# vaenyr/stable-diffusion-on-device

Hardware: AMD Instinct MI355X
Metric: images/sec + per-UNet-step ms, SD v1.4 512x512 20-step PLMS, 1/2/4/8 MI355X (higher is better)
Workload: dtype f16; 1 GPU; SD v1.4 txt2img 512x512, 20-step PLMS (21 UNet evals, batch 2 = cond+uncond per image), CLIP encode + VAE decode + uint8, guidance 7.5; images_per_gpu=1, global_batch=1, parallelism=dp1 (image shards, 1 RCCL broadcast), hip_graph=True, trajectory_graph=True, decode_overlaps_next_sampling=False

## Files before the change

### include/sdod_hip.h

```cpp
#ifndef SDOD_HIP_H
#define SDOD_HIP_H

#include <stddef.h>
#include <stdint.h>

#ifndef SDOD_API
#define SDOD_API
#endif

#ifdef __cplusplus
extern "C" {
#endif

enum sdod_act { SDOD_ACT_NONE = 0, SDOD_ACT_SILU = 1, SDOD_ACT_GELU = 2, SDOD_ACT_QUICK_GELU = 3 };
enum sdod_dtype { SDOD_F16 = 0, SDOD_F32 = 1, SDOD_U8Q = 2, SDOD_BF16 = 3  };
enum sdod_a_mode { SDOD_A_ROWS = 0, SDOD_A_CONV3X3 = 1  };

typedef struct sdod_gemm_desc {
    const void* a;
    const void* a2;
    const void* w;
    const void* bias;
    const void* row_bias;
    const void* residual;
    void* out;
    void* workspace;
    size_t workspace_bytes;
    int M, N, K;
    int lda, ldw, ldo, ldr;
    int a_mode;
    int n_img, h_in, w_in, c0, c1;
    int stride;
    int upsample;
    int ksize;
    int rows_per_img;
    int ld_row_bias;
    int act;
    float alpha;
    int bias_on_m;
    int split_k;
    int tile;
    int geglu;
    int k_tail;
    const void* t0;
    const void* t1;
    int tc0, tc1;
    const void* bias2;
    int ln;
    const void* ln_s;
    float ln_eps;
    int phase;
    int wq;
    const void* w_scale;
    const void* w_off;
    void* fix_counters;
    int xcd_panels;
    int w_img_stride;
    int vec_img_stride;
    int softmax_cols;
    int pad_mode;
} sdod_gemm_desc;

SDOD_API int sdod_gemm_f16(const sdod_gemm_desc* d, void* stream);
SDOD_API int sdod_gemm_fixup(const sdod_gemm_desc* d);
SDOD_API size_t sdod_gemm_fixup_counters(void);
SDOD_API size_t sdod_gemm_workspace_bytes(const sdod_gemm_desc* d);
SDOD_API int sdod_gemm_plan(const sdod_gemm_desc* d, int* tile, int* splits);
SDOD_API int sdod_gemm_halo_ok(const sdod_gemm_desc* d, int tile);
SDOD_API int sdod_gemm_panel_ok(const sdod_gemm_desc* d, int tile);
SDOD_API int sdod_gemm_xcd_panels(const sdod_gemm_desc* d);
SDOD_API int sdod_gemm_num_tiles(void);
SDOD_API int sdod_gemm_tile_shape(int tile, int* bm, int* bn, int* lds_dma);
SDOD_API int sdod_gemm_tile_info(int tile, int out[7]);
SDOD_API int sdod_gemm_time(const sdod_gemm_desc* d, void* stream, int iters, float* ms_avg);
SDOD_API int sdod_gemm_time_cold(const sdod_gemm_desc* d, void* stream, int iters, void* scratch, size_t scratch_bytes, float* ms_avg,
                                float* ms_min );

SDOD_API size_t sdod_group_norm_workspace_bytes(int n, int groups);
SDOD_API int sdod_group_norm_layout(int n, int groups, size_t* sync_off, size_t* partial_off, size_t* stats_off, size_t* shift_off,
                                    size_t* end_off);
SDOD_API int sdod_group_norm_status(void);
SDOD_API int sdod_group_norm_clear_error(void);
SDOD_API int sdod_group_norm_launches(int hw, int c, int groups, int dtype);
SDOD_API int sdod_group_norm_path(int n, int hw, int c0, int c1, int groups, int dtype);
SDOD_API int sdod_group_norm_nhwc(const void* x, const void* x2, void* y, const float* weight, const float* bias,
                                  int n, int hw, int c0, int c1, int groups, float eps, int silu, int dtype,
                                  void* workspace, void* stream);

SDOD_API size_t sdod_group_norm_nchw_workspace_bytes(int n, int groups);
SDOD_API int sdod_group_norm_nchw(const void* x, void* y, const float* weight, const float* bias, int n, int c, long long spatial,
                                  int groups, float eps, int silu, int dtype, void* workspace, void* stream);

typedef struct sdod_gn_reduce {
    const void* partial;
    int splits;
    size_t slab_floats;
    const void* bias;
    const void* bias2;
    const void* row_bias;
    int ld_row_bias;
    const void* residual;
    int ldr;
    void* x_out;
    float alpha;
    int act;
    int M, N;
} sdod_gn_reduce;
SDOD_API int sdod_gemm_reduce_info(const sdod_gemm_desc* d, sdod_gn_reduce* out);
SDOD_API int sdod_group_norm_reduce_ok(int hw, int c0, int c1, int groups);
SDOD_API int sdod_group_norm_reduce_nhwc(const sdod_gn_reduce* red, const void* x2, void* y, const float* weight,
                                         const float* bias, int n, int hw, int c0, int c1, int groups, float eps, int silu,
                                         void* stream);

SDOD_API int sdod_ln_fold_f16(void* w, int n, int k, int ldw, const float* gamma, const float* beta, const float* bias_in,
                              float* s_out, float* t_out, void* stream);
SDOD_API int sdod_compose_linear_f16(const void* p, int ldp, const void* w, int ldw, void* c, int ldc, int n_out, int n_mid, int k,
                                     const float* bias_w, const float* bias_p, float* bias_out, void* stream);
SDOD_API int sdod_layer_norm_f16(const void* x, void* y, const float* weight, const float* bias, int m, int c,
                                 float eps, void* stream);

SDOD_API int sdod_attention_f16(const void* q, const void* k, const void* v, void* out, int batch, int heads,
                                int lq, int lk, int d, int ldq, int ldk, int ldv, int ldo, float scale, int causal,
                                void* stream);

SDOD_API int sdod_xattn_fold_f16(const void* kv, int ld_kv, int k_off, int v_off, int n_img, int L, const void* wq, int ldq,
                                 const void* sq, const void* tq, const void* wo, int ldwo, int heads, int d, float scale, void* w1,
                                 void* s1, void* t1, void* w2, void* stream);

SDOD_API int sdod_softmax_rows_f16(const void* x, void* y, int m, int n, void* stream);

SDOD_API int sdod_geglu_f16(const void* x, void* y, int m, int c, void* stream);
SDOD_API int sdod_act_f16(const void* x, void* y, size_t n, int act, void* stream);
SDOD_API int sdod_add_f16(const void* a, const void* b, void* y, size_t n, void* stream);
SDOD_API int sdod_concat_channels_f16(const void* a, const void* b, void* y, size_t rows, int c0, int c1, void* stream);
SDOD_API int sdod_im2col3x3_small_f16(const void* x, void* y, int n_img, int h, int w, int c, int kpad, void* stream);
SDOD_API int sdod_latent_im2col_f16(const float* x, void* y, int n_img, int h, int w, int c, int kpad, float scale, void* stream);

SDOD_API int sdod_conv_in_f16(const float* x, const void* w, const float* bias, void* y, int n_img, int h, int wd, int c, int cout,
                              float scale, void* stream);
SDOD_API int sdod_image_conv_in_f16(const uint8_t* img, const void* w, const float* bias, void* y, int n_img, int h, int wd, int cout,
                                    void* stream);
SDOD_API int sdod_conv_in_cat_f16(const float* x, const float* cond, const void* w, const float* bias, void* y, int n_img, int h, int wd,
                                  int c, int c_cond, int cout, void* stream);
SDOD_API int sdod_masked_image_conv_in_f16(const uint8_t* img, const uint8_t* mask, const void* w, const float* bias, void* y, int n_img,
                                           int h, int wd, int cout, void* stream);
SDOD_API int sdod_inpaint_cond_f32(const float* moments, const uint8_t* mask_u8, const float* n1, float* cond, int n, int c, int h_lat,
                                   int w_lat, int factor, int reps, uint64_t seed, uint64_t image_index0, void* stream);
SDOD_API int sdod_encode_latent_f32(const float* moments, const float* n1, const float* n2, float* x, float* z0, int n, int c, int hw,
                                    float sqrt_at, float sqrt_one_minus_at, uint64_t seed, uint64_t image_index0, void* stream);
SDOD_API int sdod_nchw_f32_to_nhwc_f16(const float* x, void* y, int n, int c, int hw, float scale, void* stream);
SDOD_API int sdod_latent_prep_f16(const float* x, const float* w, const float* b, void* y, int n, int c, int hw,
                                  float scale, void* stream);
SDOD_API int sdod_nhwc_f16_to_nchw_f32(const void* x, float* y, int n, int c, int hw, void* stream);
SDOD_API int sdod_embedding_f16(const int32_t* ids, const void* table, const void* pos, void* y, int rows, int seq,
                                int c, void* stream);
SDOD_API int sdod_timestep_features_f16(const float* t, void* y, int n, int dim, void* stream);

SDOD_API int sdod_stage_unet_inputs(const float* x, float* x_dst, size_t lat_count, int reps, const void* temb_row,
                                    void* temb_dst, size_t temb_width, int temb_reps, void* stream);
SDOD_API int sdod_randn_f32(float* out, uint32_t* words_out, size_t count, uint64_t seed, uint64_t stream_id, void* stream);

SDOD_API int sdod_cfg_combine(const void* eps_nhwc, float* e_out, int n, int c, int hw, float guidance,
                              int uncond_first, int mode, void* stream);
SDOD_API int sdod_dpm_update(float* x, const float* eps, float* y_prev, size_t count, int order, float sigma_s,
                             float alpha_s, float sigma_ratio, float c_prev, float c_cur, void* stream);
SDOD_API int sdod_ddim_step_f32(float* x, const float* e, size_t count, float sqrt_one_minus_at, float sqrt_at,
                                float sqrt_a_prev, float dir_coef, void* stream);
SDOD_API int sdod_lincomb4_f32(float* out, const float* e0, const float* e1, const float* e2, const float* e3,
                               float c0, float c1, float c2, float c3, float div, size_t count, void* stream);

typedef struct sdod_plms_update_args {
    const void* eps_nhwc;
    float* e_out;
    float* x;
    const float* old1; const float* old2; const float* old3;
    float* x_stage;
    const void* temb_row;
    void* temb_dst;
    int n, c, hw, uncond_first, mode, v_pred, stage_reps, temb_width, temb_reps;
    float guidance, vc0, vc1, c0, c1, c2, c3, div, sqrt_one_minus_at, sqrt_at, sqrt_a_prev, dir_coef;
} sdod_plms_update_args;
SDOD_API int sdod_plms_update(const sdod_plms_update_args* a, void* stream);

typedef struct sdod_dpm_step_args {
    const void* eps_nhwc;
    float* e_out;
    float* x;
    float* y_prev;
    float* x_stage;
    const void* temb_row;
    void* temb_dst;
    int n, c, hw, uncond_first, mode, order, stage_reps, temb_width, temb_reps;
    float guidance, sigma_s, alpha_s, sigma_ratio, c_prev, c_cur;
} sdod_dpm_step_args;
SDOD_API int sdod_dpm_step(const sdod_dpm_step_args* a, void* stream);

typedef struct sdod_ddim_inpaint_step_args {
    const void* eps_nhwc;
    float* x;
    const float* z0;
    const float* keep;
    const float* noise;
    float* x_stage;
    const void* temb_row;
    void* temb_dst;
    uint64_t seed, image_index0;
    int n, c, hw, uncond_first, mode, v_pred, last, noise_level, stage_reps, temb_width, temb_reps;
    float guidance, vc0, vc1, sqrt_one_minus_at, sqrt_at, sqrt_a_prev, dir_coef, known_sa, known_s1a;
} sdod_ddim_inpaint_step_args;
SDOD_API int sdod_ddim_inpaint_step(const sdod_ddim_inpaint_step_args* a, void* stream);

typedef struct sdod_k_step_args {
    const void* eps_nhwc;
    float* x;
    float* den_prev;
    const float* noise;
    float* x_stage;
    const void* temb_row;
    void* temb_dst;
    uint64_t seed, image_index0;
    int n, c, hw, uncond_first, mode, noise_level, stage_reps, temb_width, temb_reps;
    float guidance, d0, d1, a, b, cprev, u, stage_scale;
} sdod_k_step_args;
SDOD_API int sdod_k_step(const sdod_k_step_args* a, void* stream);
SDOD_API int sdod_mask_to_latent_f32(const uint8_t* mask_u8, float* keep, int n, int h_lat, int w_lat, int factor, void* stream);
SDOD_API int sdod_image_composite_u8(const void* img, const uint8_t* init_u8, const uint8_t* mask_u8, uint8_t* out_u8, int n, size_t hw,
                                     float a, float b, int mode, void* stream);
SDOD_API int sdod_image_to_u8(const void* img, uint8_t* out, size_t count, float a, float b, int mode, void* stream);

SDOD_API const char* sdod_hip_last_error(void);
SDOD_API int sdod_hip_device_info(int* cu_count, size_t* hbm_bytes, char* arch, int arch_len);

SDOD_API int sdod_l2_prefetch(const void* ptr, size_t bytes, void* stream);

#ifdef __cplusplus
}
#endif
#endif
```

### stable-diffusion-on-device_amd/csrc/attention.hip

```cpp
#include "common.h"
#include "sdod_hip.h"
#include "host_util.h"

#include <climits>
#include <cmath>
#include <cstdlib>
#include <type_traits>

namespace {

struct AttnP {
    const f16* q;
    const f16* k;
    const f16* v;
    f16* out;
    int B, H, Lq, Lk;
    int ldq, ldk, ldv, ldo;
    float scale_log2;
    int causal;
};

typedef short short4v __attribute__((__vector_size__(4 * sizeof(short))));
typedef __attribute__((address_space(3))) short4v* lds_short4_ptr;

constexpr int odd16(int dv) {
    int s = (dv + 15) / 16;
    if ((s & 1) == 0) s += 1;
    return s * 16;
}

template <int D, int QT>
constexpr int attn_min_waves() { return (D == 40 || (D == 80 && QT == 1)) ? 3 : 1; }

template <int N, int I = 0, class F>
SDOD_DEVICE void static_for(F&& f) {
    if constexpr (I < N) {
        f(std::integral_constant<int, I>{});
        static_for<N, I + 1>(f);
    }
}

template <int D, int QT, bool TR, int KVS = 1>
__global__ __launch_bounds__(256 * KVS, (attn_min_waves<D, QT>())) void attn_kernel(const AttnP p) {
    constexpr int DP = ((D + 31) / 32) * 32;
    constexpr int KSTEPS = DP / 32;
    constexpr int DV = ((D + 15) / 16) * 16;
    constexpr int NDT = DV / 16;
    constexpr int KSTR = DP + 8;
    constexpr int VSTR = odd16(DV);
    constexpr int KT = 64;
    constexpr int DC = D / 8;
    constexpr int LD_IT = (KT * DC + 255) / 256;
    constexpr int STAGE = KT * (KSTR + VSTR);
    constexpr bool SUM_BY_MFMA = DV > D;
    constexpr bool DEFER = DP > D;
    constexpr int KS_M = D / 32, G_M = (D % 32) / 8;
    constexpr float THR = 8.0f;
    static_assert(D % 8 == 0, "head dim must be a multiple of 8");

    extern __shared__ __attribute__((aligned(16))) char smem_raw[];
    const int grp = KVS > 1 ? (int)(threadIdx.x >> 8) : 0;
    f16* smem = reinterpret_cast<f16*>(smem_raw) + (size_t)grp * 2 * STAGE;

    const int tid = threadIdx.x & 255;
    const int lane = tid & 63;
    const int wave = tid >> 6;
    const int g = lane >> 4;
    const int li = lane & 15;
    const int nqb = (p.Lq + 64 * QT - 1) / (64 * QT);
    const int lid = xcd_remap(blockIdx.x, nqb * p.H * p.B);
    const int bh = lid / nqb;
    const int b = bh / p.H, h = bh - b * p.H;
    const int q_block = (lid - bh * nqb) * (64 * QT);

    const f16* kbase = p.k + (size_t)b * p.Lk * p.ldk + h * D;
    const f16* vbase = p.v + (size_t)b * p.Lk * p.ldv + h * D;

    {
        constexpr int KPADC = (DP - D) / 8, VPADC = (DV - D) / 8;
        for (int st = 0; st < 2; ++st) {
            f16* sK = smem + st * STAGE;
            f16* sV = sK + KT * KSTR;
            if (KPADC > 0)
                for (int idx = tid; idx < KT * KPADC; idx += 256) {
                    const int row = idx / (KPADC > 0 ? KPADC : 1), ch = idx - row * KPADC;
                    f16x8 pad = zero8();
                    if (DEFER && ch == 0) pad[0] = (f16)-1.0f;
                    *reinterpret_cast<f16x8*>(sK + row * KSTR + D + ch * 8) = pad;
                }
            if (VPADC > 0)
                for (int idx = tid; idx < KT * VPADC; idx += 256) {
                    const int row = idx / (VPADC > 0 ? VPADC : 1), ch = idx - row * VPADC;
                    f16x8 pad = zero8();
                    if (ch == 0) pad[0] = (f16)1.0f;
                    *reinterpret_cast<f16x8*>(sV + row * VSTR + D + ch * 8) = pad;
                }
        }
    }

    f16x8 qf[QT][KSTEPS];
    int qrow[QT];
#pragma unroll
    for (int t = 0; t < QT; ++t) {
        qrow[t] = q_block + wave * (16 * QT) + t * 16 + li;
        const f16* qp = p.q + ((size_t)b * p.Lq + qrow[t]) * p.ldq + h * D;
#pragma unroll
        for (int ks = 0; ks < KSTEPS; ++ks) {
            const int d0 = ks * 32 + g * 8;
            qf[t][ks] = (qrow[t] < p.Lq && d0 + 8 <= D) ? ldg8(qp + d0) : zero8();
            if (DEFER)
#pragma unroll
                for (int e = 0; e < 8; ++e) qf[t][ks][e] = (f16)((float)qf[t][ks][e] * p.scale_log2);
        }
    }

    int kend = p.Lk;
    if (p.causal) kend = min(p.Lk, q_block + 64 * QT);
    const int NT = (kend + KT - 1) / KT;

    f16x8 rk[LD_IT], rv[LD_IT];
    const f16* kptr0[LD_IT];
    const f16* vptr0[LD_IT];
#pragma unroll
    for (int i = 0; i < LD_IT; ++i) {
        const int idx = tid + 256 * i;
        const int row = idx / DC, ch = idx - row * DC;
        kptr0[i] = kbase + (size_t)row * p.ldk + ch * 8;
        vptr0[i] = vbase + (size_t)row * p.ldv + ch * 8;
    }
    auto load_tile = [&](int t) {
        if (t * KT + KT <= p.Lk) {
            const size_t ko = (size_t)t * KT * p.ldk, vo = (size_t)t * KT * p.ldv;
#pragma unroll
            for (int i = 0; i < LD_IT; ++i) {
                if (tid + 256 * i < KT * DC) {
                    rk[i] = ldg8(kptr0[i] + ko);
                    rv[i] = ldg8(vptr0[i] + vo);
                }
            }
            return;
        }
#pragma unroll
        for (int i = 0; i < LD_IT; ++i) {
            const int idx = tid + 256 * i;
            const int row = idx / DC, ch = idx - row * DC;
            const int key = t * KT + row;
            const bool ok = (idx < KT * DC) && (key < p.Lk);
            rk[i] = ok ? ldg8(kbase + (size_t)key * p.ldk + ch * 8) : zero8();
            rv[i] = ok ? ldg8(vbase + (size_t)key * p.ldv + ch * 8) : zero8();
        }
    };
    auto store_tile = [&](int st) {
        f16* sK = smem + st * STAGE;
        f16* sV = sK + KT * KSTR;
#pragma unroll
        for (int i = 0; i < LD_IT; ++i) {
            const int idx = tid + 256 * i;
            const int row = idx / DC, ch = idx - row * DC;
            if (idx < KT * DC) {
                *reinterpret_cast<f16x8*>(sK + row * KSTR + ch * 8) = rk[i];
                *reinterpret_cast<f16x8*>(sV + row * VSTR + ch * 8) = rv[i];
            }
        }
    };

    f32x4 o[QT][NDT];
    float m_run[QT], l_run[QT];
#pragma unroll
    for (int t = 0; t < QT; ++t) {
        m_run[t] = DEFER ? 0.f : -1e30f;
        l_run[t] = 0.f;
#pragma unroll
        for (int dt = 0; dt < NDT; ++dt) o[t][dt] = f32x4{0.f, 0.f, 0.f, 0.f};
    }

#ifdef SDOD_ATTN_ABLATE
    constexpr int abl = SDOD_ATTN_ABLATE;
#else
    constexpr int abl = 0;
#endif
    constexpr bool HOLD = D <= 80;
    auto read_vt = [&](const f16* sV, int u, int dt) -> f16x8 {
        const f16* a0 = sV + (32 * u + 4 * g + (li >> 2)) * VSTR + dt * 16 + 4 * (li & 3);
        const short4v lo = __builtin_amdgcn_ds_read_tr16_b64_v4i16((lds_short4_ptr)(a0));
        const short4v hi = __builtin_amdgcn_ds_read_tr16_b64_v4i16((lds_short4_ptr)(a0 + 16 * VSTR));
        typedef short short8v __attribute__((__vector_size__(8 * sizeof(short))));
        const short8v both = __builtin_shufflevector(lo, hi, 0, 1, 2, 3, 4, 5, 6, 7);
        return __builtin_bit_cast(f16x8, both);
    };
    auto softmax_pv = [&](auto a_c, int t, int thr, f32x4 (&s_a)[4], const f16x8 (&vfr)[HOLD ? 2 : 1][HOLD ? NDT : 1],
                          const f16* sV) {
        constexpr int a = decltype(a_c)::value;
        const bool need_mask = (t * KT + KT > p.Lk) || (p.causal && (t * KT + KT - 1 > q_block + wave * (16 * QT)));
        if (need_mask) {
            int key0 = t * KT + g * 4;
            asm volatile("" : "+v"(key0));
#pragma unroll
            for (int c = 0; c < 4; ++c)
#pragma unroll
                for (int r = 0; r < 4; ++r) {
                    const int key = key0 + c * 16 + r;
                    const bool masked = (key >= p.Lk) | (p.causal & (key > qrow[a]));
                    s_a[c][r] = masked ? -1e30f : s_a[c][r];
                }
        }
        auto lane_max = [&]() {
            const float t0 = fmaxf(fmaxf(s_a[0][0], s_a[0][1]), s_a[0][2]);
            const float t1 = fmaxf(fmaxf(s_a[0][3], s_a[1][0]), s_a[1][1]);
            const float t2 = fmaxf(fmaxf(s_a[1][2], s_a[1][3]), s_a[2][0]);
            const float t3 = fmaxf(fmaxf(s_a[2][1], s_a[2][2]), s_a[2][3]);
            const float t4 = fmaxf(fmaxf(s_a[3][0], s_a[3][1]), s_a[3][2]);
            const float u0 = fmaxf(fmaxf(t0, t1), t2);
            const float u1 = fmaxf(fmaxf(t3, t4), s_a[3][3]);
            return fmaxf(u0, u1);
        };
        float rs[4] = {0.f, 0.f, 0.f, 0.f};
        if constexpr (DEFER) {
            auto bi = [](float x) { return __builtin_bit_cast(int, x); };
            auto mx3 = [](int x, int y, int z) { return max(max(x, y), z); };
            const int t0 = mx3(bi(s_a[0][0]), bi(s_a[0][1]), bi(s_a[0][2]));
            const int t1 = mx3(bi(s_a[0][3]), bi(s_a[1][0]), bi(s_a[1][1]));
            const int t2 = mx3(bi(s_a[1][2]), bi(s_a[1][3]), bi(s_a[2][0]));
            const int t3 = mx3(bi(s_a[2][1]), bi(s_a[2][2]), bi(s_a[2][3]));
            const int t4 = mx3(bi(s_a[3][0]), bi(s_a[3][1]), bi(s_a[3][2]));
            const int mi = max(mx3(t0, t1, t2), mx3(t3, t4, bi(s_a[3][3])));
            if (__builtin_amdgcn_ballot_w64(mi > thr) != 0) {
                const bool first = thr == INT_MIN;
                const float mx = quad_rows_max(lane_max());
                const float m_old = m_run[a];
                float m_new = m_old;
                if (first || mx > 0.f) m_new = (float)(f16)fminf(fmaxf(m_old + mx, -65504.f), 65504.f);
                const float delta = m_new - m_old;
                if (!first) {
                    const float alpha = __builtin_amdgcn_exp2f(-delta);
#pragma unroll
                    for (int dt = 0; dt < NDT; ++dt)
#pragma unroll
                        for (int r = 0; r < 4; ++r) o[a][dt][r] *= alpha;
                    if (!SUM_BY_MFMA) l_run[a] *= alpha;
                }
                m_run[a] = m_new;
                if (g == G_M) qf[a][KS_M][0] = (f16)m_new;
#pragma unroll
                for (int c = 0; c < 4; ++c)
#pragma unroll
                    for (int r = 0; r < 4; ++r) s_a[c][r] -= delta;
            }
#pragma unroll
            for (int c = 0; c < 4; ++c) {
#pragma unroll
                for (int r = 0; r < 4; ++r) {
                    float v = s_a[c][r];
                    if (!(abl & 2)) v = __builtin_amdgcn_exp2f(v);
                    if (!SUM_BY_MFMA) rs[r] += v;
                    s_a[c][r] = v;
                }
            }
            if (!SUM_BY_MFMA) l_run[a] += (rs[0] + rs[1]) + (rs[2] + rs[3]);
        } else {
            const float mx = quad_rows_max(lane_max());
            const float m_new = fmaxf(m_run[a], mx * p.scale_log2);
            const bool rescale = __builtin_amdgcn_ballot_w64(m_new != m_run[a]) != 0;
            const float alpha = rescale ? __builtin_amdgcn_exp2f(m_run[a] - m_new) : 1.0f;
            m_run[a] = m_new;
            const float sc = p.scale_log2, nm = -m_new;
#pragma unroll
            for (int c = 0; c < 4; ++c) {
#pragma unroll
                for (int r = 0; r < 4; ++r) {
                    float v = __builtin_fmaf(s_a[c][r], sc, nm);
                    if (!(abl & 2)) v = __builtin_amdgcn_exp2f(v);
                    if (!SUM_BY_MFMA) rs[r] += v;
                    s_a[c][r] = v;
                }
            }
            if (!SUM_BY_MFMA) l_run[a] = __builtin_fmaf(l_run[a], alpha, (rs[0] + rs[1]) + (rs[2] + rs[3]));
            if (rescale) {
#pragma unroll
                for (int dt = 0; dt < NDT; ++dt)
#pragma unroll
                    for (int r = 0; r < 4; ++r) o[a][dt][r] *= alpha;
            }
        }
        f16x8 pf[2];
#pragma unroll
        for (int u = 0; u < 2; ++u) {
            f16x8 f;
#pragma unroll
            for (int r = 0; r < 4; ++r) {
                f[r] = (f16)s_a[2 * u][r];
                f[4 + r] = (f16)s_a[2 * u + 1][r];
            }
            pf[u] = f;
        }
#pragma unroll
        for (int u = 0; u < 2; ++u) {
#pragma unroll
            for (int dt = 0; dt < NDT; ++dt) {
                f16x8 vf;
                if (TR) {
                    vf = HOLD ? vfr[u][dt] : read_vt(sV, u, dt);
                } else {
#pragma unroll
                    for (int e = 0; e < 8; ++e) vf[e] = sV[(32 * u + 16 * (e >> 2) + 4 * g + (e & 3)) * VSTR + dt * 16 + li];
                }
                o[a][dt] = mfma16(vf, pf[u], o[a][dt]);
            }
        }
    };
    auto read_k = [&](const f16* sK, f16x8 (&kf)[HOLD ? KSTEPS : 1][4]) {
        if constexpr (HOLD) {
#pragma unroll
            for (int ks = 0; ks < KSTEPS; ++ks)
#pragma unroll
                for (int c = 0; c < 4; ++c) kf[ks][c] = *reinterpret_cast<const f16x8*>(sK + (c * 16 + li) * KSTR + ks * 32 + g * 8);
        }
    };
    auto read_v = [&](const f16* sV, f16x8 (&vfr)[HOLD ? 2 : 1][HOLD ? NDT : 1]) {
        if constexpr (TR && HOLD) {
#pragma unroll
            for (int u = 0; u < 2; ++u)
#pragma unroll
                for (int dt = 0; dt < NDT; ++dt) vfr[u][dt] = read_vt(sV, u, dt);
        }
    };
    auto qk = [&](const f16* sK, const f16x8 (&kf)[HOLD ? KSTEPS : 1][4], f32x4 (&s)[QT][4]) {
#pragma unroll
        for (int a = 0; a < QT; ++a) {
#pragma unroll
            for (int c = 0; c < 4; ++c) s[a][c] = f32x4{0.f, 0.f, 0.f, 0.f};
#pragma unroll
            for (int ks = 0; ks < KSTEPS; ++ks)
#pragma unroll
                for (int c = 0; c < 4; ++c) {
                    const f16x8 k8 = HOLD ? kf[ks][c] : *reinterpret_cast<const f16x8*>(sK + (c * 16 + li) * KSTR + ks * 32 + g * 8);
                    s[a][c] = mfma16(k8, qf[a][ks], s[a][c]);
                }
        }
    };

    if (grp < NT) {
        load_tile(grp);
        store_tile(0);
    }
    __syncthreads();
    const int NTG = (NT + KVS - 1) / KVS;
    int thr = INT_MIN;
    for (int it = 0; it < NTG; ++it) {
        const int t = it * KVS + grp;
        const int cur = it & 1;
        const bool has_next = t + KVS < NT;
        const f16* sK = smem + cur * STAGE;
        const f16* sV = sK + KT * KSTR;
        if (t >= NT) {
            __syncthreads();
            continue;
        }
        f16x8 kf[HOLD ? KSTEPS : 1][4];
        f16x8 vfr[HOLD ? 2 : 1][HOLD ? NDT : 1];
        read_k(sK, kf);
        read_v(sV, vfr);
        f32x4 s[QT][4];
        qk(sK, kf, s);
        if (has_next && !(abl & 1)) load_tile(t + KVS);
        static_for<QT>([&](auto a_c) { softmax_pv(a_c, t, thr, s[decltype(a_c)::value], vfr, sV); });
        thr = __builtin_bit_cast(int, THR);
        asm volatile("" : "+s"(thr));
        if (has_next) store_tile(cur ^ 1);
        __syncthreads();
    }

    if constexpr (KVS > 1) {
        static_assert(KVS == 2, "the merge below handles two groups");
        float* mrg = reinterpret_cast<float*>(smem_raw);
        constexpr int NV = QT * (2 + NDT * 4);
        static_assert((size_t)NV * 256 * sizeof(float) <= (size_t)KVS * 2 * STAGE * sizeof(f16), "merge buffer fits the staging LDS");
        if (grp == 1) {
#pragma unroll
            for (int a = 0; a < QT; ++a) {
                mrg[(a * (2 + NDT * 4) + 0) * 256 + tid] = m_run[a];
                mrg[(a * (2 + NDT * 4) + 1) * 256 + tid] = l_run[a];
#pragma unroll
                for (int dt = 0; dt < NDT; ++dt)
#pragma unroll
                    for (int r = 0; r < 4; ++r) mrg[(a * (2 + NDT * 4) + 2 + dt * 4 + r) * 256 + tid] = o[a][dt][r];
            }
        }
        __syncthreads();
        if (grp == 1) return;
#pragma unroll
        for (int a = 0; a < QT; ++a) {
            const float m1 = mrg[(a * (2 + NDT * 4) + 0) * 256 + tid], l1 = mrg[(a * (2 + NDT * 4) + 1) * 256 + tid];
            const float m = fmaxf(m_run[a], m1);
            const float a0 = __builtin_amdgcn_exp2f(m_run[a] - m), a1 = __builtin_amdgcn_exp2f(m1 - m);
            l_run[a] = l_run[a] * a0 + l1 * a1;
#pragma unroll
            for (int dt = 0; dt < NDT; ++dt)
#pragma unroll
                for (int r = 0; r < 4; ++r) o[a][dt][r] = o[a][dt][r] * a0 + mrg[(a * (2 + NDT * 4) + 2 + dt * 4 + r) * 256 + tid] * a1;
            m_run[a] = m;
        }
    }
#pragma unroll
    for (int a = 0; a < QT; ++a) {
        float l;
        if (SUM_BY_MFMA) {
            l = __shfl(o[a][D / 16][D % 4], ((D % 16) / 4) * 16 + li);
        } else {
            l = quad_rows_sum(l_run[a]);
        }
        const float inv = l > 0.f ? 1.0f / l : 0.f;
        if (qrow[a] < p.Lq) {
            f16* op = p.out + ((size_t)b * p.Lq + qrow[a]) * p.ldo + h * D;
#pragma unroll
            for (int dt = 0; dt < NDT; ++dt) {
                const int dv0 = dt * 16 + g * 4;
                if (dv0 < D) {
                    f16x4 hv;
#pragma unroll
                    for (int r = 0; r < 4; ++r) hv[r] = (f16)(o[a][dt][r] * inv);
                    *reinterpret_cast<f16x4*>(op + dv0) = hv;
                }
            }
        }
    }
}

template <int D, int QT, bool TR, int KVS = 1>
hipError_t attn_launch(const AttnP& p, hipStream_t st) {
    constexpr int DP = ((D + 31) / 32) * 32;
    constexpr int DV = ((D + 15) / 16) * 16;
    constexpr size_t smem = (size_t)KVS * 2 * 64 * (DP + 8 + odd16(DV)) * sizeof(f16);
    static_assert(smem <= 160 * 1024, "LDS");
    static std::atomic<unsigned long long> attr_devs{0};
    if (sdod::first_use_on_device(attr_devs)) {
        hipError_t e = hipFuncSetAttribute(reinterpret_cast<const void*>(&attn_kernel<D, QT, TR, KVS>),
                                           hipFuncAttributeMaxDynamicSharedMemorySize, (int)smem);
        if (e != hipSuccess) return e;
    }
    dim3 grid(((p.Lq + 64 * QT - 1) / (64 * QT)) * p.H * p.B);
    SDOD_LAUNCH((attn_kernel<D, QT, TR, KVS>), grid, dim3(256 * KVS), smem, st, p);
    return hipGetLastError();
}

template <int D>
hipError_t attn_dispatch(const AttnP& p, bool big, bool tr, hipStream_t st) {
    if (tr) return big ? attn_launch<D, 2, true>(p, st) : attn_launch<D, 1, true>(p, st);
    return big ? attn_launch<D, 2, false>(p, st) : attn_launch<D, 1, false>(p, st);
}

struct FoldP {
    const f16* kv; int ld_kv, k_off, v_off, L, n_img;
    const f16* wq; int ldq;
    const float* sq; const float* tq;
    const f16* wo; int ldwo;
    int heads, d, C;
    float alpha;
    f16* w1; float* s1; float* t1; f16* w2;
    int tiles_c;
    int n_w;
};
constexpr int kFoldKMax = 160;
__global__ __launch_bounds__(256) void xattn_fold_kernel(const FoldP p) {
    __shared__ __attribute__((aligned(16))) f16 sa[80][kFoldKMax + 8], sb[80][kFoldKMax + 8];
    const int tid = threadIdx.x, lane = tid & 63, wave = tid >> 6;
    const int NK = p.heads * 80, d = p.d;
    int item = blockIdx.x;
    if (item >= 2 * p.n_w) {
        const int idx = (item - 2 * p.n_w) * 256 + tid;
        if (idx >= p.n_img * NK) return;
        const int j = idx % 80, bh = idx / 80, h = bh % p.heads, img = bh / p.heads;
        if (j >= p.L) {
            p.s1[idx] = 0.f;
            p.t1[idx] = -30000.f;
            return;
        }
        const f16* kr = p.kv + ((long long)img * p.L + j) * p.ld_kv + p.k_off + h * d;
        float a = 0.f, b = 0.f;
        for (int dd = 0; dd < d; ++dd) {
            const float kval = (float)kr[dd];
            a = fmaf(kval, p.sq[h * d + dd], a);
            b = fmaf(kval, p.tq[h * d + dd], b);
        }
        p.s1[idx] = p.alpha * a;
        p.t1[idx] = p.alpha * b;
        return;
    }
    const bool second = item >= p.n_w;
    if (second) item -= p.n_w;
    const int tc = item % p.tiles_c, bh = item / p.tiles_c, h = bh % p.heads, img = bh / p.heads;
    const int KP = (d + 31) & ~31, kc = KP / 8;
    auto stage_rows = [&](f16 (*dst)[kFoldKMax + 8], const f16* base, long long row_stride, int valid_rows) {
        for (int idx = tid; idx < 80 * kc; idx += 256) {
            const int r = idx / kc, ch = idx - r * kc;
            const f16x8 v = (r < valid_rows && ch * 8 < d) ? ldg8(base + (long long)r * row_stride + ch * 8) : zero8();
            *reinterpret_cast<f16x8*>(&dst[r][ch * 8]) = v;
        }
    };
    if (!second) {
        stage_rows(sa, p.kv + (long long)img * p.L * p.ld_kv + p.k_off + h * d, p.ld_kv, p.L);
        for (int idx = tid; idx < KP * 10; idx += 256) {
            const int k = idx / 10, ch = idx - k * 10;
            const f16x8 v = k < d ? ldg8(p.wq + (long long)(h * d + k) * p.ldq + tc * 80 + ch * 8) : zero8();
#pragma unroll
            for (int e = 0; e < 8; ++e) sb[ch * 8 + e][k] = v[e];
        }
    } else {
        stage_rows(sa, p.wo + (long long)(tc * 80) * p.ldwo + h * d, p.ldwo, 80);
        stage_rows(sb, p.kv + (long long)img * p.L * p.ld_kv + p.v_off + h * d, p.ld_kv, p.L);
    }
    __syncthreads();
    const int fr = lane & 15, fg = lane >> 4;
    for (int rb = wave; rb < 5; rb += 4) {
        f32x4 acc[5];
#pragma unroll
        for (int j = 0; j < 5; ++j) acc[j] = f32x4{0.f, 0.f, 0.f, 0.f};
        for (int ks = 0; ks < KP / 32; ++ks) {
            const f16x8 fa = *reinterpret_cast<const f16x8*>(&sa[rb * 16 + fr][ks * 32 + fg * 8]);
#pragma unroll
            for (int j = 0; j < 5; ++j) {
                const f16x8 fb = *reinterpret_cast<const f16x8*>(&sb[j * 16 + fr][ks * 32 + fg * 8]);
                acc[j] = mfma16(fb, fa, acc[j]);
            }
        }
        const int m = rb * 16 + fr;
        f16* row = second ? p.w2 + ((long long)img * p.C + tc * 80 + m) * NK + h * 80
                          : p.w1 + ((long long)(img * p.heads + h) * 80 + m) * p.C + tc * 80;
        const float al = second ? 1.0f : p.alpha;
#pragma unroll
        for (int j = 0; j < 5; ++j) {
            f16x4 o;
#pragma unroll
            for (int r = 0; r < 4; ++r) o[r] = (f16)(al * acc[j][r]);
            *reinterpret_cast<f16x4*>(row + j * 16 + fg * 4) = o;
        }
    }
}

}

extern "C" int sdod_attention_f16(const void* q, const void* k, const void* v, void* out, int batch, int heads, int lq,
                                  int lk, int d, int ldq, int ldk, int ldv, int ldo, float scale, int causal,
                                  void* stream) {
    SDOD_TRY
    SDOD_REQUIRE(q && k && v && out, "null pointer");
    SDOD_REQUIRE(batch > 0 && heads > 0 && lq > 0 && lk > 0, "bad shape");
    SDOD_REQUIRE(d == 40 || d == 64 || d == 80 || d == 160, "head dim must be one of 40, 64, 80, 160");
    SDOD_REQUIRE(ldq % 8 == 0 && ldk % 8 == 0 && ldv % 8 == 0 && ldo % 4 == 0, "row strides must keep 16-byte alignment");
    SDOD_REQUIRE(ldq >= heads * d && ldk >= heads * d && ldv >= heads * d && ldo >= heads * d, "row stride < heads*d");
    SDOD_REQUIRE((((uintptr_t)q | (uintptr_t)k | (uintptr_t)v) & 15) == 0 && ((uintptr_t)out & 7) == 0, "misaligned pointer");
    SDOD_REQUIRE(std::isfinite(scale) && scale > 0.f, "scale must be finite and > 0");
    AttnP p{};
    p.q = (const f16*)q; p.k = (const f16*)k; p.v = (const f16*)v; p.out = (f16*)out;
    p.B = batch; p.H = heads; p.Lq = lq; p.Lk = lk;
    p.ldq = ldq; p.ldk = ldk; p.ldv = ldv; p.ldo = ldo;
    p.scale_log2 = scale * 1.4426950408889634f;
    p.causal = causal;
    const bool no_tr = std::getenv("SDOD_ATTN_NO_TR") != nullptr;
    const bool tr = !no_tr;
    bool big = lq >= 2048 && d != 160;
    if (const char* e = std::getenv("SDOD_ATTN_QT")) big = e[0] == '2' && d != 160;
    hipStream_t st = (hipStream_t)stream;
    hipError_t e;
    switch (d) {
    case 40: e = attn_dispatch<40>(p, big, tr, st); break;
    case 64: e = attn_dispatch<64>(p, big, tr, st); break;
    case 80: {
        static const bool kvs_off = [] { const char* e2 = std::getenv("SDOD_ATTN_KVS"); return e2 && e2[0] == '0'; }();
        const long long wgs = (long long)((lq + 63) / 64) * heads * batch;
        if (!big && tr && !kvs_off && !causal && wgs <= 512 && lk >= 256) e = attn_launch<80, 1, true, 2>(p, st);
        else e = attn_dispatch<80>(p, big, tr, st);
        break;
    }
    default: e = attn_dispatch<160>(p, false, tr, st); break;
    }
    SDOD_HIP_CHECK(e);
    return 0;
    SDOD_CATCH
}

extern "C" int sdod_xattn_fold_f16(const void* kv, int ld_kv, int k_off, int v_off, int n_img, int L, const void* wq, int ldq,
                                   const void* sq, const void* tq, const void* wo, int ldwo, int heads, int d, float scale, void* w1,
                                   void* s1, void* t1, void* w2, void* stream) {
    SDOD_TRY
    SDOD_REQUIRE(kv && wq && sq && tq && wo && w1 && s1 && t1 && w2, "null pointer");
    SDOD_REQUIRE(n_img > 0 && heads > 0 && d > 0 && d <= kFoldKMax && d % 8 == 0 && L > 0 && L <= 80, "bad shape (d <= 160, d % 8 == 0, L <= 80)");
    const int C = heads * d, NK = heads * 80;
    SDOD_REQUIRE(C % 80 == 0 && ldq >= C && ldwo >= C && ld_kv >= C, "heads * d must be a multiple of 80; row strides >= heads * d");
    SDOD_REQUIRE(ld_kv % 8 == 0 && k_off % 8 == 0 && v_off % 8 == 0 && ldq % 8 == 0 && ldwo % 8 == 0 &&
                     (((uintptr_t)kv | (uintptr_t)wq | (uintptr_t)wo | (uintptr_t)w1 | (uintptr_t)w2) & 15) == 0,
                 "operands must keep 16-byte alignment");
    FoldP p{};
    p.kv = (const f16*)kv; p.ld_kv = ld_kv; p.k_off = k_off; p.v_off = v_off; p.L = L; p.n_img = n_img;
    p.wq = (const f16*)wq; p.ldq = ldq; p.sq = (const float*)sq; p.tq = (const float*)tq;
    p.wo = (const f16*)wo; p.ldwo = ldwo;
    p.heads = heads; p.d = d; p.C = C;
    p.alpha = scale * 1.4426950408889634f;
    p.w1 = (f16*)w1; p.s1 = (float*)s1; p.t1 = (float*)t1; p.w2 = (f16*)w2;
    p.tiles_c = C / 80;
    p.n_w = n_img * heads * p.tiles_c;
    const int blocks = 2 * p.n_w + (n_img * NK + 255) / 256;
    SDOD_LAUNCH(xattn_fold_kernel, dim3(blocks), dim3(256), 0, (hipStream_t)stream, p);
    SDOD_HIP_CHECK(hipGetLastError());
    return 0;
    SDOD_CATCH
}
```

### stable-diffusion-on-device_amd/csrc/engine.h

```cpp
#pragma once
#include <hip/hip_runtime.h>

#include <cstdint>
#include <functional>
#include <map>
#include <string>
#include <unordered_map>
#include <vector>

#include "host_util.h"
#include "sdod_engine.h"
#include "sdod_hip.h"

namespace sdod {

typedef _Float16 f16;

enum ParamKind {
    PK_CONV3,
    PK_CONV3_SMALL,
    PK_CONV1,
    PK_LINEAR,
    PK_EMBED,
    PK_VEC,
    PK_MAT_F32,
    PK_LINEAR_GEGLU,
    PK_VEC_GEGLU,
};

inline int small_k(int64_t cin) { return 9 * cin <= 64 ? 64 : 128; }

struct Param {
    std::string name;
    std::vector<int64_t> shape;
    ParamKind kind;
    int group = -1;
    int ld = 0;
    int col_off = 0;
    int owner = -1;
    size_t dev_bytes = 0;
    char* dev = nullptr;
    bool set = false;
    bool quant = false;
    size_t qrow = 0;
};

struct Act {
    f16* p = nullptr;
    int n = 0, h = 0, w = 0, c = 0;
    int rows() const { return n * h * w; }
    size_t numel() const { return (size_t)rows() * c; }
};

struct IoSlot {
    void* ptr = nullptr;
    size_t bytes = 0;
};

class Graph {
public:
    Graph(int kind, const sdod_model_config& cfg, int batch);
    ~Graph();
    Graph(const Graph&) = delete;

    int num_params() const { return (int)params_.size(); }
    const Param& param(int i) const { return params_.at(i); }
    void set_param(const std::string& name, const void* data, int dtype, const int64_t* shape, int ndim);
    void load_file(const std::string& path, const std::string& prefix);
    void finalize();
    void execute(hipStream_t st, bool use_hip_graph, bool skip_static = false);
    void check_health() const;
    IoSlot io(bool output, int index) const;
    void stats(size_t* wbytes, size_t* abytes, int* launches, double* flops) const;

private:
    enum Mode { DECLARE, DRY, REAL };
    int kind_;
    sdod_model_config cfg_;
    int batch_;
    Mode mode_ = DECLARE;
    bool finalized_ = false;

    std::vector<Param> params_;
    std::unordered_map<std::string, int> pindex_;
    std::vector<std::vector<int>> groups_;
    std::unordered_map<std::string, int> gindex_;
    char* weight_base_ = nullptr;
    size_t weight_bytes_ = 0;
    float* qscale_ = nullptr;
    float* qoff_ = nullptr;
    size_t qrows_ = 0;
    bool quant_mode() const { return cfg_.weight_quant != 0 && (kind_ == SDOD_GRAPH_UNET || kind_ == SDOD_GRAPH_TEMB); }
    static constexpr int kQuantAutoMaxRows = 128;
    bool quant_decl_ = false;
    void quant_rows(int rows) { quant_decl_ = quant_mode() && (cfg_.weight_quant == 1 || rows <= kQuantAutoMaxRows); }
    void quant_global() { quant_decl_ = quant_mode(); }
    const float* qscale_of(int w) const { return params_[w].quant ? qscale_ + params_[w].qrow : nullptr; }
    const float* qoff_of(int w) const { return params_[w].quant ? qoff_ + params_[w].qrow : nullptr; }
    int P(const std::string& name, std::vector<int64_t> shape, ParamKind kind, const std::string& group = "");
    int Pc(const std::string& name, std::vector<int64_t> shape, ParamKind kind, int ld, int col_off, int owner);
    template <typename T>
    const T* W(int idx) const { return reinterpret_cast<const T*>(params_[idx].dev); }
    void allocate_weights();

    char* arena_base_ = nullptr;
    size_t arena_cap_ = 0, arena_high_ = 0;
    std::map<size_t, size_t> free_;
    std::map<size_t, size_t> used_;
    void arena_reset();
    f16* alloc(size_t halves);
    void release(const void* p);
    Act act(int n, int h, int w, int c);
    void release(const Act& a) { release(a.p); }

    char* ws_ = nullptr;
    size_t ws_bytes_ = 0, ws_need_ = 0;
    char* gn_ws_ = nullptr;
    size_t gn_ws_bytes_ = 0, gn_ws_need_ = 0;

    std::vector<IoSlot> inputs_, outputs_;
    void* io_alloc(std::vector<IoSlot>& v, size_t bytes);

    struct Op {
        std::function<void(hipStream_t)> fn;
        std::string label;
        double flops = 0;
        double bytes = 0;
        std::string detail;
        const void* pf_ptr = nullptr;
        size_t pf_bytes = 0;
    };
    std::vector<Op> ops_;
    std::vector<Op> static_ops_;
    bool to_static_ = false;
    double flops_ = 0;
    hipGraphExec_t graph_exec_ = nullptr;
    hipGraph_t hip_graph_ = nullptr;
    hipStream_t capture_stream_ = nullptr;
    unsigned* fix_counters_ = nullptr;
    hipStream_t side_stream_ = nullptr;
    std::vector<hipEvent_t> pf_events_;
    void run_ops(hipStream_t st);
    int eager_runs_ = 0;
    int tune_hits_ = 0, tune_misses_ = 0;

    void build();
    void build_unet();
    void build_vae();
    void build_vae_encoder(bool masked);
    void build_clip();
    void build_temb();

    struct GemmOpt {
        int bias = -1;
        const float* bias_raw = nullptr;
        f16* out = nullptr;
        const f16* row_bias = nullptr;
        int ld_row_bias = 0, rows_per_img = 0;
        const f16* residual = nullptr;
        int act = 0;
        float alpha = 1.0f;
        bool bias_on_m = false;
        int lda = 0, ldo = 0;
        int ldr = 0;
        bool geglu = false;
        const Act* tail0 = nullptr;
        const Act* tail1 = nullptr;
        int bias2 = -1;
        int ln_w = -1, ln_b = -1;
        const float* wq_scale = nullptr;
        const float* wq_off = nullptr;
        const float* ln_s_raw = nullptr;
        int w_img_stride = 0, vec_img_stride = 0;
        int softmax_cols = 0;
        int pad_mode = 0;
    };
    struct LnVecs { float* s; float* t; };
    LnVecs ln_fold_vectors(f16* w, int N, int K, int ldw, int ln_w, int ln_b, const float* bias);
    struct FoldJob {
        f16* w; int n, k, ldw;
        const float *gamma, *beta, *bias_in;
        float *s, *t;
    };
    std::vector<FoldJob> fold_jobs_;
    struct ComposeJob {
        f16* c; const f16* p; int ld, n_out, n_mid, k;
        const float *bias_w, *bias_p;
        float* bias_out;
    };
    std::vector<ComposeJob> compose_jobs_;
    std::vector<void*> derived_;
    void emit_gemm(sdod_gemm_desc d);
    void linear(const f16* x, int rows, int K, int w, int N, f16* out, const GemmOpt& o);
    void linear_raw(const f16* x, int rows, int K, const f16* w, int ldw, int N, f16* out, const GemmOpt& o);
    Act conv(const Act& x, const Act* x2, int w, int cout, int ksize, int stride, bool upsample, const GemmOpt& o);
    Act group_norm(const Act& x, const Act* x2, int gw, int gb, float eps, bool silu);
    Act layer_norm(const Act& x, int lw, int lb, float eps);
    void attention(const f16* q, const f16* k, const f16* v, f16* out, int B, int heads, int lq, int lk, int d, int ldq,
                   int ldk, int ldv, int ldo, bool causal);

    Act res_block(const std::string& pfx, const Act& x, const Act* x2, int cout, const f16* emb_all, int emb_ld, int& emb_off);
    std::vector<Op>& sink() { return to_static_ ? static_ops_ : ops_; }
    struct PendingReduce {
        bool active = false;
        sdod_gemm_desc d{};
        double bytes = 0;
        std::string detail;
    } pending_;
    void flush_pending();
    std::vector<const void*> parked_;
    void release_after_consumer(const Act& a) { parked_.push_back(a.p); }
    void drain_parked() {
        for (const void* p : parked_) release(p);
        parked_.clear();
    }
    void settle() {
        flush_pending();
        drain_parked();
    }
    Act spatial_transformer(const std::string& pfx, const Act& x, const Act& ctx);
    Act vae_res_block(const std::string& pfx, const Act& x, int cout);
    Act vae_attn_block(const std::string& pfx, const Act& x);
    int emb_total_ = 0;
    int kv_total_ = 0;
    f16* kv_all_ = nullptr;
    int kv_off_ = 0;
    std::vector<std::pair<std::string, int>> unet_res_blocks() const;
    const char* group_base(const std::string& group) const;
    int group_first(const std::string& group) const;
    void emit(std::function<void(hipStream_t)> fn, const char* label = "elementwise", double flops = 0, double bytes = 0) {
        settle();
        if (mode_ == REAL) sink().push_back(Op{std::move(fn), label, flops, bytes, ""});
    }

public:
    int tune_hits() const { return tune_hits_; }
    int tune_misses() const { return tune_misses_; }
    int num_ops() const { return (int)ops_.size(); }
    const Op& op(int i) const { return ops_.at(i); }
    void profile(hipStream_t st, int iters, float* ms, int n);
};

}
```

### stable-diffusion-on-device_amd/csrc/engine.hip

```cpp
#include "engine.h"

#include <cstdio>

#include <dlfcn.h>
#include <fcntl.h>
#include <sys/mman.h>
#include <sys/stat.h>
#include <unistd.h>

#include <algorithm>
#include <cstdlib>
#include <cstring>
#include <map>
#include <mutex>
#include <thread>

namespace sdod {

static inline size_t align_up(size_t v, size_t a) { return (v + a - 1) / a * a; }

static void check_rc(int rc) {
    if (rc != 0) throw Error(rc, get_last_error());
}

template <typename F>
static void parallel_for(int64_t n, F&& fn) {
    int nt = (int)std::min<int64_t>(n, std::max(1u, std::min(16u, std::thread::hardware_concurrency())));
    if (nt <= 1) {
        fn(0, n);
        return;
    }
    std::vector<std::thread> th;
    const int64_t per = (n + nt - 1) / nt;
    for (int t = 0; t < nt; ++t) {
        const int64_t b = t * per, e = std::min(n, b + per);
        if (b < e) th.emplace_back([=, &fn]() { fn(b, e); });
    }
    for (auto& t : th) t.join();
}

Graph::Graph(int kind, const sdod_model_config& cfg, int batch) : kind_(kind), cfg_(cfg), batch_(batch) {
    SDOD_REQUIRE(kind >= SDOD_GRAPH_UNET && kind <= SDOD_GRAPH_VAE_ENCODER_MASKED, "unknown graph kind");
    SDOD_REQUIRE(batch > 0 && batch <= 64, "batch must be in [1, 64]");
    SDOD_REQUIRE(cfg.model_channels > 0 && cfg.model_channels % 64 == 0, "model_channels must be a multiple of 64");
    SDOD_REQUIRE(cfg.context_dim % 64 == 0, "context_dim must be a multiple of 64");
    SDOD_REQUIRE(cfg.concat_channels >= 0, "concat_channels must not be negative");
    mode_ = DECLARE;
    arena_reset();
    build();
}

Graph::~Graph() {
    if (graph_exec_) (void)hipGraphExecDestroy(graph_exec_);
    if (capture_stream_) (void)hipStreamDestroy(capture_stream_);
    if (side_stream_) (void)hipStreamDestroy(side_stream_);
    (void)hipFree(fix_counters_);
    for (hipEvent_t e : pf_events_) (void)hipEventDestroy(e);
    if (hip_graph_) (void)hipGraphDestroy(hip_graph_);
    for (auto& s : inputs_) (void)hipFree(s.ptr);
    for (auto& s : outputs_) (void)hipFree(s.ptr);
    (void)hipFree(weight_base_);
    (void)hipFree(qscale_);
    (void)hipFree(qoff_);
    (void)hipFree(arena_base_);
    (void)hipFree(ws_);
    (void)hipFree(gn_ws_);
    (void)hipFree(kv_all_);
    for (void* d : derived_) (void)hipFree(d);
}

static size_t param_dev_bytes(const Param& p) {
    const auto& s = p.shape;
    if (p.quant) return (size_t)s[0] * s[1] * (p.kind == PK_CONV3 ? 9 : 1);
    switch (p.kind) {
    case PK_CONV3: return (size_t)s[0] * s[1] * 9 * sizeof(f16);
    case PK_CONV3_SMALL: return (size_t)s[0] * small_k(s[1]) * sizeof(f16);
    case PK_CONV1:
    case PK_LINEAR:
    case PK_LINEAR_GEGLU:
    case PK_EMBED: return (size_t)s[0] * s[1] * sizeof(f16);
    case PK_VEC:
    case PK_VEC_GEGLU: return (size_t)s[0] * sizeof(float);
    case PK_MAT_F32: {
        size_t n = 1;
        for (auto d : s) n *= (size_t)d;
        return n * sizeof(float);
    }
    }
    return 0;
}

int Graph::P(const std::string& name, std::vector<int64_t> shape, ParamKind kind, const std::string& group) {
    if (mode_ != DECLARE) {
        auto it = pindex_.find(name);
        if (it == pindex_.end()) throw Error(INTERNAL_ERROR, "parameter not declared: " + name);
        return it->second;
    }
    if (pindex_.count(name)) throw Error(INTERNAL_ERROR, "duplicate parameter: " + name);
    Param p;
    p.name = name;
    p.shape = std::move(shape);
    p.kind = kind;
    p.quant = quant_decl_ && (kind == PK_CONV3 || kind == PK_CONV1 || kind == PK_LINEAR || kind == PK_LINEAR_GEGLU);
    p.dev_bytes = param_dev_bytes(p);
    if (!group.empty()) {
        auto it = gindex_.find(group);
        if (it == gindex_.end()) {
            gindex_[group] = (int)groups_.size();
            groups_.emplace_back();
            it = gindex_.find(group);
        }
        p.group = it->second;
        groups_[p.group].push_back((int)params_.size());
    }
    pindex_[name] = (int)params_.size();
    params_.push_back(std::move(p));
    return (int)params_.size() - 1;
}

int Graph::Pc(const std::string& name, std::vector<int64_t> shape, ParamKind kind, int ld, int col_off, int owner) {
    const int idx = P(name, std::move(shape), kind);
    if (mode_ == DECLARE) {
        Param& p = params_[idx];
        p.ld = ld;
        p.col_off = col_off;
        p.owner = owner;
        p.dev_bytes = owner < 0 ? (size_t)p.shape[0] * ld * sizeof(f16) : 0;
    }
    return idx;
}

void Graph::allocate_weights() {
    if (weight_base_) return;
    size_t off = 0;
    std::vector<size_t> offs(params_.size(), 0);
    for (auto& g : groups_) {
        off = align_up(off, 256);
        for (int idx : g) {
            if (params_[idx].dev_bytes % 16) throw Error(INTERNAL_ERROR, "grouped parameter size must be a multiple of 16: " + params_[idx].name);
            offs[idx] = off;
            off += params_[idx].dev_bytes;
        }
    }
    for (size_t i = 0; i < params_.size(); ++i) {
        if (params_[i].group >= 0) continue;
        off = align_up(off, 256);
        offs[i] = off;
        off += params_[i].dev_bytes;
    }
    weight_bytes_ = align_up(off, 256);
    SDOD_HIP_CHECK(hipMalloc((void**)&weight_base_, weight_bytes_));
    SDOD_HIP_CHECK(hipMemset(weight_base_, 0, weight_bytes_));
    for (size_t i = 0; i < params_.size(); ++i) params_[i].dev = weight_base_ + offs[i];
    {
        std::vector<size_t> order;
        for (size_t i = 0; i < params_.size(); ++i)
            if (params_[i].quant) order.push_back(i);
        std::sort(order.begin(), order.end(), [&](size_t a, size_t b) { return offs[a] < offs[b]; });
        qrows_ = 0;
        for (size_t i : order) {
            params_[i].qrow = qrows_;
            qrows_ += (size_t)params_[i].shape[0];
        }
        if (qrows_) {
            SDOD_HIP_CHECK(hipMalloc((void**)&qscale_, qrows_ * sizeof(float)));
            SDOD_HIP_CHECK(hipMalloc((void**)&qoff_, qrows_ * sizeof(float)));
        }
    }
    for (auto& p : params_)
        if (p.owner >= 0) p.dev = params_[p.owner].dev + (size_t)p.col_off * sizeof(f16);
}

template <typename S>
static void pack_param_host(const Param& p, const S* src, char* dst_raw) {
    const auto& s = p.shape;
    switch (p.kind) {
    case PK_CONV3:
    case PK_CONV3_SMALL: {
        const int64_t co = s[0], ci = s[1];
        const int64_t kd = p.kind == PK_CONV3 ? 9 * ci : small_k(ci);
        f16* dst = reinterpret_cast<f16*>(dst_raw);
        parallel_for(co, [&](int64_t b, int64_t e) {
            for (int64_t o = b; o < e; ++o) {
                f16* drow = dst + o * kd;
                if (p.kind == PK_CONV3_SMALL) std::memset(drow, 0, kd * sizeof(f16));
                const S* srow = src + o * ci * 9;
                for (int64_t c = 0; c < ci; ++c)
                    for (int t = 0; t < 9; ++t) drow[t * ci + c] = (f16)(float)srow[c * 9 + t];
            }
        });
        break;
    }
    case PK_CONV1:
    case PK_LINEAR:
    case PK_EMBED: {
        const int64_t n = s[0] * s[1];
        f16* dst = reinterpret_cast<f16*>(dst_raw);
        parallel_for(n, [&](int64_t b, int64_t e) {
            for (int64_t i = b; i < e; ++i) dst[i] = (f16)(float)src[i];
        });
        break;
    }
    case PK_LINEAR_GEGLU: {
        const int64_t rows = s[0], k = s[1], H = rows / 2;
        f16* dst = reinterpret_cast<f16*>(dst_raw);
        parallel_for(rows, [&](int64_t b, int64_t e) {
            for (int64_t r = b; r < e; ++r) {
                const int64_t j = r < H ? r : r - H;
                const int64_t nr = (j / 16) * 32 + (r < H ? 0 : 16) + j % 16;
                for (int64_t c = 0; c < k; ++c) dst[nr * k + c] = (f16)(float)src[r * k + c];
            }
        });
        break;
    }
    case PK_VEC_GEGLU: {
        const int64_t rows = s[0], H = rows / 2;
        float* dst = reinterpret_cast<float*>(dst_raw);
        for (int64_t r = 0; r < rows; ++r) {
            const int64_t j = r < H ? r : r - H;
            dst[(j / 16) * 32 + (r < H ? 0 : 16) + j % 16] = (float)src[r];
        }
        break;
    }
    case PK_VEC:
    case PK_MAT_F32: {
        int64_t n = 1;
        for (auto d : s) n *= d;
        float* dst = reinterpret_cast<float*>(dst_raw);
        for (int64_t i = 0; i < n; ++i) dst[i] = (float)src[i];
        break;
    }
    }
}

void Graph::set_param(const std::string& name, const void* data, int dtype, const int64_t* shape, int ndim) {
    allocate_weights();
    SDOD_REQUIRE(!finalized_, "parameters cannot change after finalize() (weights are repacked / folded in place)");
    auto it = pindex_.find(name);
    SDOD_REQUIRE(it != pindex_.end(), "unknown parameter '" + name + "'");
    SDOD_REQUIRE(data != nullptr, "null data for '" + name + "'");
    SDOD_REQUIRE(dtype == SDOD_F32 || dtype == SDOD_F16 || dtype == SDOD_U8Q, "dtype must be SDOD_F32, SDOD_F16 or SDOD_U8Q");
    Param& p = params_[it->second];
    int64_t want = 1, got = 1;
    for (auto d : p.shape) want *= d;
    for (int i = 0; i < ndim; ++i) got *= shape[i];
    if (p.quant) {
        SDOD_REQUIRE(dtype == SDOD_U8Q, "graph was created with weight_quant != 0: '" + name + "' must be given as SDOD_U8Q");
        bool same = (int)p.shape.size() == ndim;
        for (int i = 0; same && i < ndim; ++i) same = p.shape[i] == shape[i];
        if (!same && want == got && (p.kind == PK_CONV1 || p.kind == PK_LINEAR) && ndim >= 2 && shape[0] == p.shape[0]) same = true;
        SDOD_REQUIRE(same, "shape mismatch for '" + name + "'");
        float scale;
        int32_t offset;
        std::memcpy(&scale, data, 4);
        std::memcpy(&offset, static_cast<const char*>(data) + 4, 4);
        SDOD_REQUIRE(offset >= -1024 && offset <= 0, "'" + name + "': uint8 encoding offset must be in [-1024, 0] (QNN: -zero_point of a uint8 tensor)");
        const uint8_t* q = static_cast<const uint8_t*>(data) + 8;
        const int64_t rows = p.shape[0], kd = got / rows;
        std::vector<uint8_t> staging((size_t)got);
        uint8_t* dst = staging.data();
        if (p.kind == PK_CONV3) {
            const int64_t ci = p.shape[1];
            parallel_for(rows, [&](int64_t b, int64_t e) {
                for (int64_t o = b; o < e; ++o)
                    for (int64_t c = 0; c < ci; ++c)
                        for (int t = 0; t < 9; ++t) dst[o * kd + t * ci + c] = q[(o * ci + c) * 9 + t];
            });
        } else if (p.kind == PK_LINEAR_GEGLU) {
            const int64_t H = rows / 2;
            parallel_for(rows, [&](int64_t b, int64_t e) {
                for (int64_t r = b; r < e; ++r) {
                    const int64_t j = r < H ? r : r - H;
                    const int64_t nr = (j / 16) * 32 + (r < H ? 0 : 16) + j % 16;
                    std::memcpy(dst + nr * kd, q + r * kd, (size_t)kd);
                }
            });
        } else {
            std::memcpy(dst, q, (size_t)got);
        }
        SDOD_REQUIRE(p.ld == 0, "column-block parameters are not used with uint8 weights");
        SDOD_HIP_CHECK(hipMemcpy(p.dev, staging.data(), (size_t)got, hipMemcpyHostToDevice));
        std::vector<float> sv((size_t)rows, scale), ov((size_t)rows, (float)(offset + 128));
        SDOD_HIP_CHECK(hipMemcpy(qscale_ + p.qrow, sv.data(), sv.size() * sizeof(float), hipMemcpyHostToDevice));
        SDOD_HIP_CHECK(hipMemcpy(qoff_ + p.qrow, ov.data(), ov.size() * sizeof(float), hipMemcpyHostToDevice));
        p.set = true;
        return;
    }
    std::vector<float> deq;
    if (dtype == SDOD_U8Q) {
        float scale;
        int32_t offset;
        std::memcpy(&scale, data, 4);
        std::memcpy(&offset, static_cast<const char*>(data) + 4, 4);
        const uint8_t* q = static_cast<const uint8_t*>(data) + 8;
        deq.resize((size_t)got);
        float* dst = deq.data();
        parallel_for(got, [&](int64_t b, int64_t e) {
            for (int64_t i = b; i < e; ++i) dst[i] = (float)((double)((int32_t)q[i] + offset) * (double)scale);
        });
        data = deq.data();
        dtype = SDOD_F32;
    }
    bool same = (int)p.shape.size() == ndim;
    for (int i = 0; same && i < ndim; ++i) same = p.shape[i] == shape[i];
    if (!same && want == got && (p.kind == PK_CONV1 || p.kind == PK_LINEAR) && ndim >= 2 && shape[0] == p.shape[0]) same = true;
    if (!same) {
        std::string m = "shape mismatch for '" + name + "': expected [";
        for (auto d : p.shape) m += std::to_string(d) + ",";
        m += "] got [";
        for (int i = 0; i < ndim; ++i) m += std::to_string(shape[i]) + ",";
        throw Error(INVALID_ARGUMENT, m + "]");
    }
    Param dense = p;
    dense.ld = 0;
    const size_t dense_bytes = param_dev_bytes(dense);
    std::vector<char> staging(dense_bytes);
    if (dtype == SDOD_F32) pack_param_host(dense, reinterpret_cast<const float*>(data), staging.data());
    else pack_param_host(dense, reinterpret_cast<const f16*>(data), staging.data());
    if (p.ld > 0) {
        const size_t row_bytes = dense_bytes / (size_t)p.shape[0];
        SDOD_HIP_CHECK(hipMemcpy2D(p.dev, (size_t)p.ld * sizeof(f16), staging.data(), row_bytes, row_bytes, (size_t)p.shape[0],
                                   hipMemcpyHostToDevice));
    } else {
        SDOD_HIP_CHECK(hipMemcpy(p.dev, staging.data(), dense_bytes, hipMemcpyHostToDevice));
    }
    p.set = true;
}

void Graph::load_file(const std::string& path, const std::string& prefix) {
    int fd = ::open(path.c_str(), O_RDONLY);
    SDOD_REQUIRE(fd >= 0, "cannot open weight file " + path);
    struct stat stt;
    if (fstat(fd, &stt) != 0) {
        ::close(fd);
        throw Error(INVALID_ARGUMENT, "cannot stat " + path);
    }
    const size_t fsize = (size_t)stt.st_size;
    void* map = mmap(nullptr, fsize, PROT_READ, MAP_PRIVATE, fd, 0);
    ::close(fd);
    SDOD_REQUIRE(map != MAP_FAILED, "mmap failed for " + path);
    struct Unmap {
        void* p;
        size_t n;
        ~Unmap() { munmap(p, n); }
    } guard{map, fsize};
    const char* base = static_cast<const char*>(map);
    size_t pos = 0;
    auto need = [&](size_t n) { SDOD_REQUIRE(pos + n <= fsize, "truncated weight file " + path); };
    need(16);
    SDOD_REQUIRE(std::memcmp(base, "SDODW001", 8) == 0, "bad magic in " + path);
    uint64_t count;
    std::memcpy(&count, base + 8, 8);
    pos = 16;
    for (uint64_t t = 0; t < count; ++t) {
        uint32_t nl, dt, nd;
        need(4); std::memcpy(&nl, base + pos, 4); pos += 4;
        need(nl); std::string name(base + pos, nl); pos += nl;
        need(8); std::memcpy(&dt, base + pos, 4); std::memcpy(&nd, base + pos + 4, 4); pos += 8;
        SDOD_REQUIRE(nd <= 8, "bad ndim in " + path);
        int64_t dims[8];
        need(8 * nd + 16);
        for (uint32_t i = 0; i < nd; ++i) { uint64_t d; std::memcpy(&d, base + pos, 8); pos += 8; dims[i] = (int64_t)d; }
        uint64_t off, nb;
        std::memcpy(&off, base + pos, 8); std::memcpy(&nb, base + pos + 8, 8); pos += 16;
        SDOD_REQUIRE(off <= fsize && nb <= fsize - off, "tensor payload out of range in " + path);
        SDOD_REQUIRE(dt == SDOD_F16 || dt == SDOD_F32 || dt == SDOD_U8Q, "bad dtype for '" + name + "' in " + path);
        uint64_t numel = 1;
        for (uint32_t i = 0; i < nd; ++i) {
            SDOD_REQUIRE(dims[i] > 0 && (uint64_t)dims[i] <= (uint64_t(1) << 40) / numel, "bad dims for '" + name + "' in " + path);
            numel *= (uint64_t)dims[i];
        }
        const uint64_t want = dt == SDOD_U8Q ? 8 + numel : numel * (dt == SDOD_F16 ? 2 : 4);
        SDOD_REQUIRE(nb == want, "payload size of '" + name + "' does not match its dims in " + path);
        if (name.compare(0, prefix.size(), prefix) != 0) continue;
        const std::string local = name.substr(prefix.size());
        if (!pindex_.count(local)) continue;
        set_param(local, base + off, (int)dt, dims, (int)nd);
    }
}

static char* const kFakeBase = reinterpret_cast<char*>(uintptr_t(1) << 40);

void Graph::arena_reset() {
    free_.clear();
    used_.clear();
    if (mode_ == REAL) {
        free_[0] = arena_cap_;
    } else {
        free_[0] = size_t(1) << 39;
        arena_high_ = 0;
    }
}

f16* Graph::alloc(size_t halves) {
    const size_t bytes = align_up(std::max<size_t>(halves * sizeof(f16), 256), 256);
    for (auto it = free_.begin(); it != free_.end(); ++it) {
        if (it->second >= bytes) {
            const size_t off = it->first, sz = it->second;
            free_.erase(it);
            if (sz > bytes) free_[off + bytes] = sz - bytes;
            used_[off] = bytes;
            arena_high_ = std::max(arena_high_, off + bytes);
            char* base = mode_ == REAL ? arena_base_ : kFakeBase;
            return reinterpret_cast<f16*>(base + off);
        }
    }
    throw Error(INTERNAL_ERROR, "activation arena exhausted");
}

void Graph::release(const void* p) {
    if (!p) return;
    if (pending_.active && pending_.d.residual == p) flush_pending();
    char* base = mode_ == REAL ? arena_base_ : kFakeBase;
    const size_t off = (size_t)(reinterpret_cast<const char*>(p) - base);
    auto it = used_.find(off);
    if (it == used_.end()) throw Error(INTERNAL_ERROR, "arena release of unknown block");
    size_t sz = it->second;
    used_.erase(it);
    size_t start = off;
    auto nxt = free_.lower_bound(off);
    if (nxt != free_.end() && nxt->first == off + sz) {
        sz += nxt->second;
        nxt = free_.erase(nxt);
    }
    if (nxt != free_.begin()) {
        auto prv = std::prev(nxt);
        if (prv->first + prv->second == off) {
            start = prv->first;
            sz += prv->second;
            free_.erase(prv);
        }
    }
    free_[start] = sz;
}

Act Graph::act(int n, int h, int w, int c) {
    Act a;
    a.n = n; a.h = h; a.w = w; a.c = c;
    a.p = alloc(a.numel());
    return a;
}

void* Graph::io_alloc(std::vector<IoSlot>& v, size_t bytes) {
    IoSlot s;
    s.bytes = bytes;
    if (mode_ == REAL) {
        SDOD_HIP_CHECK(hipMalloc(&s.ptr, align_up(bytes, 256)));
        SDOD_HIP_CHECK(hipMemset(s.ptr, 0, align_up(bytes, 256)));
        v.push_back(s);
        return s.ptr;
    }
    return kFakeBase + (size_t(1) << 39) + v.size() * 4096;
}

IoSlot Graph::io(bool output, int index) const {
    const auto& v = output ? outputs_ : inputs_;
    SDOD_REQUIRE(finalized_, "graph not finalized");
    SDOD_REQUIRE(index >= 0 && index < (int)v.size(), "io index out of range");
    return v[index];
}

namespace {
constexpr size_t kPrefetchMinBytes = (size_t)12 << 20;
const std::vector<int> kCandidates = [] {
    std::vector<int> v((size_t)gemm_tuner_tiles(nullptr, 0));
    gemm_tuner_tiles(v.data(), (int)v.size());
    return v;
}();

struct ShapeKey {
    static constexpr int kFields = 14;
    int v[kFields];
    bool operator<(const ShapeKey& o) const { return std::lexicographical_compare(v, v + kFields, o.v, o.v + kFields); }
};
const char* tune_cache_path() {
    const char* e = std::getenv("SDOD_TUNE_CACHE");
    return (e && e[0]) ? e : nullptr;
}
std::string shipped_tune_path() {
    const char* e = std::getenv("SDOD_TUNE_DEFAULT");
    if (e && e[0] == '0') return "";
    Dl_info info;
    if (!dladdr(reinterpret_cast<const void*>(&sdod_model_config_sd14), &info) || !info.dli_fname) return "";
    std::string lib = info.dli_fname;
    const size_t a = lib.rfind('/');
    if (a == std::string::npos) return "";
    const size_t b = lib.rfind('/', a - 1);
    if (b == std::string::npos) return "";
    return lib.substr(0, b) + "/tune/gfx950.tune";
}
struct TuneEntry {
    int v;
    bool from_file;
};
struct TuneCache {
    std::mutex mu;
    std::map<ShapeKey, TuneEntry> map;
    bool loaded = false;
};
void tune_cache_read(const char* path, std::map<ShapeKey, TuneEntry>& c) {
    FILE* f = std::fopen(path, "r");
    if (!f) return;
    char line[512];
    while (std::fgets(line, sizeof line, f)) {
        long val[ShapeKey::kFields + 2];
        int n = 0;
        char* cur = line;
        while (n < ShapeKey::kFields + 2) {
            char* endp = nullptr;
            const long x = std::strtol(cur, &endp, 10);
            if (endp == cur) break;
            val[n++] = x;
            cur = endp;
        }
        ShapeKey k{};
        int v;
        if (n == ShapeKey::kFields + 1) {
            for (int i = 0; i < ShapeKey::kFields; ++i) k.v[i] = (int)val[i];
            v = (int)val[ShapeKey::kFields];
        } else if (n == 13) {
            for (int i = 0; i < 12; ++i) k.v[i] = (int)val[i];
            k.v[12] = k.v[13] = 0;
            if (k.v[0] == SDOD_A_CONV3X3 && k.v[9] > 0) {
                const int ups = k.v[7] ? 1 : 0, stride = k.v[6] > 0 ? k.v[6] : 1;
                const int ho = (k.v[9] << ups) / stride;
                k.v[12] = k.v[9];
                k.v[13] = ho > 0 ? k.v[1] / (ho * ho) : 0;
            }
            v = (int)val[12];
        } else {
            continue;
        }
        const int tile = v % 1000, split = v / 1000;
        if (tile >= 1 && tile <= sdod_gemm_num_tiles() && split >= 1 && split <= 64) c[k] = TuneEntry{v, true};
    }
    std::fclose(f);
}
TuneCache& tune_cache() {
    static TuneCache c;
    std::lock_guard<std::mutex> lk(c.mu);
    if (!c.loaded) {
        c.loaded = true;
        const std::string shipped = shipped_tune_path();
        if (!shipped.empty()) tune_cache_read(shipped.c_str(), c.map);
        if (const char* path = tune_cache_path()) tune_cache_read(path, c.map);
    }
    return c;
}
void tune_cache_append(const ShapeKey& k, int v) {
    const char* path = tune_cache_path();
    if (!path) return;
    if (FILE* f = std::fopen(path, "a")) {
        for (int i = 0; i < ShapeKey::kFields; ++i) std::fprintf(f, "%d ", k.v[i]);
        std::fprintf(f, "%d\n", v);
        std::fclose(f);
    }
}
bool autotune_enabled() {
    const char* e = std::getenv("SDOD_AUTOTUNE");
    return !(e && e[0] == '0');
}
bool autotune_cold() {
    const char* e = std::getenv("SDOD_AUTOTUNE");
    return !(e && e[0] == 'h');
}
constexpr size_t kSweepBytes = (size_t)384 << 20;
void*& tune_scratch() {
    static void* p = nullptr;
    return p;
}
ShapeKey key_of(const sdod_gemm_desc& d) {
    return ShapeKey{{d.a_mode, d.M, d.N, d.K, d.c0, d.c1, d.stride, d.upsample, d.ksize, d.h_in,
                     (d.residual ? 1 : 0) + (d.geglu ? 2 : 0) + 4 * d.tc0 + 16384 * d.tc1 + (d.ln ? (1 << 30) : 0) + (d.wq ? (1 << 29) : 0) + (d.softmax_cols ? (1 << 28) : 0) + (d.w_img_stride ? (1 << 27) : 0) +
                         (d.pad_mode ? (1 << 26) : 0) , d.lda,
                     d.a_mode == SDOD_A_CONV3X3 ? d.w_in : 0, d.a_mode == SDOD_A_CONV3X3 ? d.n_img : 0}};
}
bool pick_runs(const sdod_gemm_desc& d, int v) {
    sdod_gemm_desc c = d;
    c.tile = v % 1000;
    c.split_k = v / 1000;
    int info[7] = {0};
    if (sdod_gemm_tile_info(c.tile, info) != 0) return false;
    if (info[5] == 2) return sdod_gemm_halo_ok(&c, c.tile) != 0;
    if (info[5] == 3) return sdod_gemm_panel_ok(&c, c.tile) != 0;
    return true;
}
}

void Graph::flush_pending() {
    if (!pending_.active) return;
    pending_.active = false;
    const sdod_gemm_desc d2 = pending_.d;
    sink().push_back(Op{[d2](hipStream_t st) { check_rc(sdod_gemm_f16(&d2, st)); }, "splitk_reduce", 0.0, pending_.bytes, pending_.detail});
}

void Graph::emit_gemm(sdod_gemm_desc d) {
    settle();
    if (mode_ == DECLARE) return;
    const bool tune = autotune_enabled() && (d.N > 16 || (d.a_mode == SDOD_A_CONV3X3 && d.ksize != 1 && d.N % 4 == 0));
    if (tune) {
        for (int t : kCandidates) {
            sdod_gemm_desc c = d;
            c.tile = t;
            c.split_k = 0;
            int tt = 0, sp = 1;
            (void)sdod_gemm_plan(&c, &tt, &sp);
            c.split_k = sp > 1 ? std::min(64, sp * 2) : 1;
            if (c.split_k > 1 && d.N % 4 == 0) ws_need_ = std::max(ws_need_, sdod_gemm_workspace_bytes(&c));
        }
    }
    ws_need_ = std::max(ws_need_, sdod_gemm_workspace_bytes(&d));
    if (mode_ != REAL) return;
    if (tune) {
        d.workspace = ws_;
        d.workspace_bytes = ws_bytes_;
        d.fix_counters = std::getenv("SDOD_GEMM_FIXUP") && std::getenv("SDOD_GEMM_FIXUP")[0] == '1' ? fix_counters_ : nullptr;
        const ShapeKey key = key_of(d);
        TuneCache& tc = tune_cache();
        int pick = 0;
        bool from_file = false;
        {
            std::lock_guard<std::mutex> lk(tc.mu);
            auto it = tc.map.find(key);
            if (it != tc.map.end() && pick_runs(d, it->second.v)) {
                pick = it->second.v;
                from_file = it->second.from_file;
            }
        }
        if (pick && from_file) ++tune_hits_;
        else ++tune_misses_;
        if (!pick) {
            int best = 0;
            float best_ms = 1e30f;
            const int KT = d.K / 64;
            for (int t : kCandidates) {
                sdod_gemm_desc h = d;
                h.tile = t;
                h.split_k = 0;
                int tt = 0, sp = 1;
                (void)sdod_gemm_plan(&h, &tt, &sp);
                if (tt != t) continue;
                int tried[4] = {sp, 1, sp / 2, sp > 1 ? sp * 2 : 0};
                for (int k = 0; k < 4; ++k) {
                    const int want = tried[k];
                    bool dup = want < 1 || want > 64 || (want > 1 && KT / want < 2) || (want > 1 && d.N % 4 != 0);
                    for (int j = 0; j < k && !dup; ++j) dup = tried[j] == want;
                    if (dup) continue;
                    sdod_gemm_desc c = d;
                    c.tile = t;
                    c.split_k = want;
                    if (sdod_gemm_workspace_bytes(&c) > ws_bytes_) continue;
                    float ms = 0.f;
                    if (autotune_cold()) {
                        if (!tune_scratch()) {
                            SDOD_HIP_CHECK(hipMalloc(&tune_scratch(), kSweepBytes));
                            SDOD_HIP_CHECK(hipMemset(tune_scratch(), 0, kSweepBytes));
                        }
                        float avg = 0.f;
                        if (sdod_gemm_time_cold(&c, nullptr, 4, tune_scratch(), kSweepBytes, &avg, &ms) != 0) continue;
                    } else if (sdod_gemm_time(&c, nullptr, 4, &ms) != 0) {
                        continue;
                    }
                    if (ms < best_ms) {
                        best_ms = ms;
                        best = t + 1000 * want;
                    }
                }
            }
            {
                std::lock_guard<std::mutex> lk(tc.mu);
                tc.map[key] = TuneEntry{best, false};
                tune_cache_append(key, best);
            }
            pick = best;
        }
        d.tile = pick % 1000;
        d.split_k = pick / 1000;
    }
    const double fl = 2.0 * d.M * d.N * d.K;
    flops_ += fl;
    d.workspace = ws_;
    d.workspace_bytes = ws_bytes_;
    d.fix_counters = fix_counters_;
    int tile = 0, splits = 1;
    (void)sdod_gemm_plan(&d, &tile, &splits);
    std::string label = "gemm_t" + std::to_string(tile);
    double a_bytes = d.a_mode == SDOD_A_ROWS ? (double)d.M * d.K * 2
                                             : (double)d.n_img * d.h_in * d.w_in * (d.c0 + d.c1) * 2;
    double by = a_bytes + (double)d.N * d.K * 2 + (double)d.M * d.N * 2 * (d.residual ? 2 : 1);
    std::string detail = (d.a_mode == SDOD_A_ROWS ? std::string("rows") : "conv" + std::to_string(d.ksize) + (d.upsample ? "u" : "") +
                                                                          (d.stride == 2 ? "s2" : "") + (d.c1 ? "+cat" : "")) +
                         " M" + std::to_string(d.M) + " N" + std::to_string(d.N) + " K" + std::to_string(d.K) + " x" + std::to_string(splits);
    static const bool fixup_on = [] { const char* e = std::getenv("SDOD_GEMM_FIXUP"); return e && e[0] == '1'; }();
    if (!fixup_on) d.fix_counters = nullptr;
    static const bool fuse_reduce_gn = [] { const char* e = std::getenv("SDOD_GN_REDUCE"); return e && e[0] == '1'; }();
    if (splits > 1 && !fuse_reduce_gn && sdod_gemm_fixup(&d)) {
        const double part = (double)splits * d.M * d.N * 4;
        sink().push_back(Op{[d](hipStream_t st) { check_rc(sdod_gemm_f16(&d, st)); }, label, fl, by + part, detail});
        return;
    }
    if (splits > 1) {
        sdod_gemm_desc d1 = d, d2 = d;
        d1.phase = 1;
        d2.phase = 2;
        const double part = (double)splits * d.M * d.N * 4;
        sink().push_back(Op{[d1](hipStream_t st) { check_rc(sdod_gemm_f16(&d1, st)); }, label, fl, by + part, detail});
        if ((size_t)d.N * d.ldw * (d.wq ? 1 : 2) >= kPrefetchMinBytes) {
            sink().back().pf_ptr = d.w;
            sink().back().pf_bytes = (size_t)d.N * d.ldw * (d.wq ? 1 : 2);
        }
        pending_.active = true;
        pending_.d = d2;
        pending_.bytes = part + (double)d.M * d.N * 2 * (d.residual ? 2 : 1);
        pending_.detail = detail;
        static const bool fuse_reduce = [] { const char* e = std::getenv("SDOD_GN_REDUCE"); return e && e[0] == '1'; }();
        if (to_static_ || !fuse_reduce) flush_pending();
        return;
    }
    sink().push_back(Op{[d](hipStream_t st) { check_rc(sdod_gemm_f16(&d, st)); }, label, fl, by, detail});
    if ((size_t)d.N * d.ldw * (d.wq ? 1 : 2) >= kPrefetchMinBytes) {
        sink().back().pf_ptr = d.w;
        sink().back().pf_bytes = (size_t)d.N * d.ldw * (d.wq ? 1 : 2);
    }
}

void Graph::linear_raw(const f16* x, int rows, int K, const f16* w, int ldw, int N, f16* out, const GemmOpt& o) {
    sdod_gemm_desc d{};
    d.a = x; d.w = w; d.out = out;
    d.M = rows; d.N = N; d.K = K;
    d.lda = o.lda ? o.lda : K;
    d.ldw = ldw;
    d.ldo = o.ldo ? o.ldo : N;
    d.a_mode = SDOD_A_ROWS;
    if (o.bias >= 0) d.bias = params_[o.bias].dev;
    if (o.bias_raw) d.bias = o.bias_raw;
    d.bias_on_m = o.bias_on_m ? 1 : 0;
    d.row_bias = o.row_bias; d.ld_row_bias = o.ld_row_bias; d.rows_per_img = o.rows_per_img;
    d.residual = o.residual; d.ldr = o.ldr ? o.ldr : d.ldo;
    d.act = o.act; d.alpha = o.alpha;
    if (o.geglu) {
        d.geglu = 1;
        if (!o.ldo) d.ldo = N / 2;
        d.ldr = d.ldo;
    }
    if (o.wq_scale) {
        d.wq = 1;
        d.w_scale = o.wq_scale;
        d.w_off = o.wq_off;
    }
    if (o.ln_w >= 0) {
        if (d.wq) throw Error(INTERNAL_ERROR, "LayerNorm fold with uint8 weights");
        d.ln = 1;
        d.ln_eps = 1e-5f;
        if (mode_ == REAL) {
            const LnVecs v = ln_fold_vectors(const_cast<f16*>(w), N, K, ldw, o.ln_w, o.ln_b, reinterpret_cast<const float*>(d.bias));
            d.ln_s = v.s;
            d.bias = v.t;
        } else {
            d.ln_s = d.w;
            d.bias = d.w;
        }
    }
    if (o.ln_s_raw) {
        d.ln = 1;
        d.ln_eps = 1e-5f;
        d.ln_s = o.ln_s_raw;
    }
    d.w_img_stride = o.w_img_stride; d.vec_img_stride = o.vec_img_stride; d.softmax_cols = o.softmax_cols;
    emit_gemm(d);
}

Graph::LnVecs Graph::ln_fold_vectors(f16* w, int N, int K, int ldw, int ln_w, int ln_b, const float* bias) {
    float *sv = nullptr, *tv = nullptr;
    SDOD_HIP_CHECK(hipMalloc((void**)&sv, (size_t)N * sizeof(float)));
    SDOD_HIP_CHECK(hipMalloc((void**)&tv, (size_t)N * sizeof(float)));
    derived_.push_back(sv);
    derived_.push_back(tv);
    fold_jobs_.push_back(FoldJob{w, N, K, ldw, W<float>(ln_w), W<float>(ln_b), bias, sv, tv});
    return LnVecs{sv, tv};
}

void Graph::linear(const f16* x, int rows, int K, int w, int N, f16* out, const GemmOpt& o) {
    const Param& p = params_[w];
    const int ldw = p.ld > 0 ? p.ld : p.kind == PK_CONV3_SMALL ? small_k(p.shape[1]) : (int)(p.kind == PK_CONV3 ? p.shape[1] * 9 : p.shape[1]);
    if (p.quant) {
        GemmOpt oq = o;
        oq.wq_scale = qscale_of(w);
        oq.wq_off = qoff_of(w);
        linear_raw(x, rows, K, reinterpret_cast<const f16*>(p.dev), ldw, N, out, oq);
        return;
    }
    linear_raw(x, rows, K, reinterpret_cast<const f16*>(p.dev), ldw, N, out, o);
}

Act Graph::conv(const Act& x, const Act* x2, int w, int cout, int ksize, int stride, bool upsample, const GemmOpt& o) {
    const int ups = upsample ? 1 : 0;
    const int hup = x.h << ups, wup = x.w << ups;
    const int pad_sum = o.pad_mode ? 1 : 2 * (ksize / 2);
    const int ho = (hup + pad_sum - ksize) / stride + 1, wo = (wup + pad_sum - ksize) / stride + 1;
    Act y;
    y.n = x.n; y.h = ho; y.w = wo; y.c = cout;
    y.p = o.out ? o.out : alloc(y.numel());
    sdod_gemm_desc d{};
    d.a = x.p; d.a2 = x2 ? x2->p : nullptr;
    d.w = params_[w].dev; d.out = y.p;
    const int cin = x.c + (x2 ? x2->c : 0);
    d.M = y.rows(); d.N = cout; d.K = ksize * ksize * cin;
    if (o.tail0) {
        d.k_tail = d.K;
        d.t0 = o.tail0->p; d.tc0 = o.tail0->c;
        d.t1 = o.tail1 ? o.tail1->p : nullptr; d.tc1 = o.tail1 ? o.tail1->c : 0;
        d.K += d.tc0 + d.tc1;
        if (o.bias2 >= 0) d.bias2 = params_[o.bias2].dev;
    }
    d.ldw = params_[w].ld > 0 ? params_[w].ld : d.K; d.ldo = cout;
    d.a_mode = SDOD_A_CONV3X3;
    d.n_img = x.n; d.h_in = x.h; d.w_in = x.w; d.c0 = x.c; d.c1 = x2 ? x2->c : 0;
    d.stride = stride; d.upsample = ups; d.ksize = ksize; d.pad_mode = o.pad_mode;
    if (o.bias >= 0) d.bias = params_[o.bias].dev;
    else if (o.bias_raw) d.bias = o.bias_raw;
    d.row_bias = o.row_bias; d.ld_row_bias = o.ld_row_bias; d.rows_per_img = o.rows_per_img;
    d.residual = o.residual; d.ldr = cout;
    d.act = o.act; d.alpha = o.alpha;
    if (params_[w].quant) {
        if (o.tail0) throw Error(INTERNAL_ERROR, "tail segment with uint8 weights");
        d.wq = 1;
        d.w_scale = qscale_of(w);
        d.w_off = qoff_of(w);
    }
    emit_gemm(d);
    return y;
}

Act Graph::group_norm(const Act& x, const Act* x2, int gw, int gb, float eps, bool silu) {
    Act y = act(x.n, x.h, x.w, x.c + (x2 ? x2->c : 0));
    if (mode_ != DECLARE) gn_ws_need_ = std::max(gn_ws_need_, sdod_group_norm_workspace_bytes(x.n, 32));
    if (mode_ == REAL) {
        const void* xp = x.p; const void* x2p = x2 ? x2->p : nullptr; void* yp = y.p;
        const float* wp = W<float>(gw); const float* bp = W<float>(gb);
        const int n = x.n, hw = x.h * x.w, c0 = x.c, c1 = x2 ? x2->c : 0, si = silu ? 1 : 0;
        const std::string shape = "n" + std::to_string(n) + " hw" + std::to_string(hw) + " c" + std::to_string(c0 + c1);
        if (pending_.active && pending_.d.out == x.p && pending_.d.M == x.rows() && pending_.d.N == c0 &&
            (!pending_.d.row_bias || pending_.d.rows_per_img == hw) && sdod_group_norm_reduce_ok(hw, c0, c1, 32)) {
            sdod_gn_reduce red{};
            check_rc(sdod_gemm_reduce_info(&pending_.d, &red));
            pending_.active = false;
            ops_.push_back(Op{[=](hipStream_t st) {
                check_rc(sdod_group_norm_reduce_nhwc(&red, x2p, yp, wp, bp, n, hw, c0, c1, 32, eps, si, st));
            }, "gn_group_red", 0, pending_.bytes + 2.0 * n * hw * (c0 + c1) * 2, shape + " x" + std::to_string(red.splits)});
        } else {
            flush_pending();
            void* ws = gn_ws_;
            ops_.push_back(Op{[=](hipStream_t st) {
                check_rc(sdod_group_norm_nhwc(xp, x2p, yp, wp, bp, n, hw, c0, c1, 32, eps, si, SDOD_F16, ws, st));
            }, [&] {
                switch (sdod_group_norm_path(n, hw, c0, c1, 32, SDOD_F16)) {
                case 0: return "gn_grid";
                case 1: return "gn_group";
                case 2: return "gn_small";
                default: return "gn_stats_apply";
                }
            }(), 0, 2.0 * n * hw * (c0 + c1) * 2, shape});
        }
    }
    drain_parked();
    return y;
}

Act Graph::layer_norm(const Act& x, int lw, int lb, float eps) {
    Act y = act(x.n, x.h, x.w, x.c);
    settle();
    if (mode_ != REAL) return y;
    const void* xp = x.p; void* yp = y.p;
    const float* wp = W<float>(lw); const float* bp = W<float>(lb);
    const int m = x.rows(), c = x.c;
    ops_.push_back(Op{[=](hipStream_t st) { check_rc(sdod_layer_norm_f16(xp, yp, wp, bp, m, c, eps, st)); }, "layer_norm", 0,
                      2.0 * m * c * 2, "m" + std::to_string(m) + " c" + std::to_string(c)});
    return y;
}

void Graph::attention(const f16* q, const f16* k, const f16* v, f16* out, int B, int heads, int lq, int lk, int d, int ldq,
                      int ldk, int ldv, int ldo, bool causal) {
    settle();
    if (mode_ != REAL) return;
    const double fl = 4.0 * B * heads * (double)lq * lk * d;
    flops_ += fl;
    const float scale = 1.0f / sqrtf((float)d);
    const int ca = causal ? 1 : 0;
    ops_.push_back(Op{[=](hipStream_t st) {
        check_rc(sdod_attention_f16(q, k, v, out, B, heads, lq, lk, d, ldq, ldk, ldv, ldo, scale, ca, st));
    }, "attn_d" + std::to_string(d), fl, 2.0 * B * heads * d * (2.0 * lq + 2.0 * lk),
                      "B" + std::to_string(B) + " h" + std::to_string(heads) + " lq" + std::to_string(lq) + " lk" + std::to_string(lk)});
}

void Graph::build() {
    quant_global();
    switch (kind_) {
    case SDOD_GRAPH_UNET: build_unet(); break;
    case SDOD_GRAPH_VAE_DECODER: build_vae(); break;
    case SDOD_GRAPH_TEXT_ENCODER: build_clip(); break;
    case SDOD_GRAPH_VAE_ENCODER: build_vae_encoder(false); break;
    case SDOD_GRAPH_VAE_ENCODER_MASKED: build_vae_encoder(true); break;
    default: build_temb(); break;
    }
    settle();
}

void Graph::finalize() {
    allocate_weights();
    SDOD_REQUIRE(!finalized_, "graph already finalized");
    std::string missing;
    int nmiss = 0;
    for (auto& p : params_)
        if (!p.set) {
            if (nmiss < 5) missing += (nmiss ? ", " : "") + p.name;
            ++nmiss;
        }
    SDOD_REQUIRE(nmiss == 0, std::to_string(nmiss) + " parameter(s) not set: " + missing + (nmiss > 5 ? ", ..." : ""));
    mode_ = DRY;
    arena_reset();
    ws_need_ = gn_ws_need_ = 0;
    build();
    arena_cap_ = align_up(arena_high_, 256) + 256;
    ws_bytes_ = align_up(ws_need_, 256) + 256;
    gn_ws_bytes_ = align_up(gn_ws_need_, 256) + 256;
    SDOD_HIP_CHECK(hipMalloc((void**)&arena_base_, arena_cap_));
    SDOD_HIP_CHECK(hipMalloc((void**)&ws_, ws_bytes_));
    SDOD_HIP_CHECK(hipMalloc((void**)&gn_ws_, gn_ws_bytes_));
    SDOD_HIP_CHECK(hipMemset(gn_ws_, 0, gn_ws_bytes_));
    SDOD_HIP_CHECK(hipMalloc((void**)&fix_counters_, sdod_gemm_fixup_counters() * sizeof(unsigned)));
    SDOD_HIP_CHECK(hipMemset(fix_counters_, 0, sdod_gemm_fixup_counters() * sizeof(unsigned)));
    if (kind_ == SDOD_GRAPH_UNET && kv_total_ > 0)
        SDOD_HIP_CHECK(hipMalloc((void**)&kv_all_, (size_t)batch_ * cfg_.context_len * kv_total_ * sizeof(f16)));
    mode_ = REAL;
    arena_reset();
    ops_.clear();
    static_ops_.clear();
    fold_jobs_.clear();
    compose_jobs_.clear();
    flops_ = 0;
    build();
    for (const FoldJob& j : fold_jobs_)
        check_rc(sdod_ln_fold_f16(j.w, j.n, j.k, j.ldw, j.gamma, j.beta, j.bias_in, j.s, j.t, nullptr));
    for (const ComposeJob& j : compose_jobs_) {
        f16* tmp = nullptr;
        SDOD_HIP_CHECK(hipMalloc((void**)&tmp, (size_t)j.n_mid * j.k * sizeof(f16)));
        SDOD_HIP_CHECK(hipMemcpy2D(tmp, (size_t)j.k * sizeof(f16), j.c, (size_t)j.ld * sizeof(f16), (size_t)j.k * sizeof(f16), (size_t)j.n_mid,
                                   hipMemcpyDeviceToDevice));
        const int rc = sdod_compose_linear_f16(j.p, j.ld, tmp, j.k, j.c, j.ld, j.n_out, j.n_mid, j.k, j.bias_w, j.bias_p, j.bias_out, nullptr);
        SDOD_HIP_CHECK(hipDeviceSynchronize());
        (void)hipFree(tmp);
        check_rc(rc);
    }
    SDOD_HIP_CHECK(hipDeviceSynchronize());
    if (tune_scratch()) {
        (void)hipFree(tune_scratch());
        tune_scratch() = nullptr;
    }
    finalized_ = true;
}

namespace {
constexpr int kPrefetchLookahead = 3;
bool prefetch_enabled() {
    static const bool on = [] { const char* e = std::getenv("SDOD_PREFETCH"); return e && e[0] == '1'; }();
    return on;
}
}

void Graph::run_ops(hipStream_t st) {
    const bool pf = prefetch_enabled() && g_launch_timer == nullptr;
    size_t ev = 0;
    bool forked = false;
    auto next_event = [&]() {
        if (ev == pf_events_.size()) {
            hipEvent_t e = nullptr;
            SDOD_HIP_CHECK(hipEventCreateWithFlags(&e, hipEventDisableTiming));
            pf_events_.push_back(e);
        }
        return pf_events_[ev++];
    };
    for (size_t i = 0; i < ops_.size(); ++i) {
        const size_t j = i + kPrefetchLookahead;
        if (pf && j < ops_.size() && ops_[j].pf_bytes) {
            if (!side_stream_) SDOD_HIP_CHECK(hipStreamCreateWithFlags(&side_stream_, hipStreamNonBlocking));
            hipEvent_t fork = next_event();
            SDOD_HIP_CHECK(hipEventRecord(fork, st));
            SDOD_HIP_CHECK(hipStreamWaitEvent(side_stream_, fork, 0));
            check_rc(sdod_l2_prefetch(ops_[j].pf_ptr, ops_[j].pf_bytes, side_stream_));
            forked = true;
        }
        ops_[i].fn(st);
    }
    if (forked) {
        hipEvent_t join = next_event();
        SDOD_HIP_CHECK(hipEventRecord(join, side_stream_));
        SDOD_HIP_CHECK(hipStreamWaitEvent(st, join, 0));
    }
}

void Graph::check_health() const {
    if (sdod_group_norm_status() != 0)
        throw Error(RUNTIME_ERROR, "a GroupNorm grid barrier timed out on this device (workspace clobbered, or graphs sharing the device "
                                   "starved each other of CUs): results since then are invalid; sdod_group_norm_clear_error() after "
                                   "rebuilding the graph re-arms");
}

void Graph::execute(hipStream_t st, bool use_hip_graph, bool skip_static) {
    SDOD_REQUIRE(finalized_, "graph not finalized");
    check_health();
    if (!skip_static || eager_runs_ == 0)
        for (auto& op : static_ops_) op.fn(st);
    if (!use_hip_graph || eager_runs_ == 0) {
        run_ops(st);
        ++eager_runs_;
        return;
    }
    if (!graph_exec_) {
        if (!capture_stream_) SDOD_HIP_CHECK(hipStreamCreateWithFlags(&capture_stream_, hipStreamNonBlocking));
        SDOD_HIP_CHECK(hipStreamSynchronize(st));
        SDOD_HIP_CHECK(hipStreamBeginCapture(capture_stream_, hipStreamCaptureModeThreadLocal));
        try {
            run_ops(capture_stream_);
        } catch (...) {
            hipGraph_t g = nullptr;
            (void)hipStreamEndCapture(capture_stream_, &g);
            if (g) (void)hipGraphDestroy(g);
            throw;
        }
        SDOD_HIP_CHECK(hipStreamEndCapture(capture_stream_, &hip_graph_));
        SDOD_HIP_CHECK(hipGraphInstantiate(&graph_exec_, hip_graph_, nullptr, nullptr, 0));
    }
    SDOD_HIP_CHECK(hipGraphLaunch(graph_exec_, st));
}

void Graph::profile(hipStream_t st, int iters, float* ms, int n) {
    SDOD_REQUIRE(finalized_, "graph not finalized");
    SDOD_REQUIRE(ms != nullptr && n == (int)ops_.size() && iters > 0, "profile buffer must hold one float per op");
    constexpr int kMaxLaunches = 4;
    struct Events {
        std::vector<hipEvent_t> v;
        explicit Events(size_t n) : v(n, nullptr) {}
        ~Events() { for (auto e : v) if (e) (void)hipEventDestroy(e); }
        hipEvent_t& operator[](size_t i) { return v[i]; }
    } evs(ops_.size() * kMaxLaunches), eve(ops_.size() * kMaxLaunches);
    for (auto& e : evs.v) SDOD_HIP_CHECK(hipEventCreate(&e));
    for (auto& e : eve.v) SDOD_HIP_CHECK(hipEventCreate(&e));
    std::vector<int> used(ops_.size(), 0);
    std::vector<std::vector<float>> samples(ops_.size());
    for (int it = 0; it < iters + 1; ++it) {
        for (size_t i = 0; i < ops_.size(); ++i) {
            LaunchTimer lt{&evs[i * kMaxLaunches], &eve[i * kMaxLaunches], kMaxLaunches, 0};
            g_launch_timer = &lt;
            try {
                ops_[i].fn(st);
            } catch (...) {
                g_launch_timer = nullptr;
                throw;
            }
            g_launch_timer = nullptr;
            used[i] = lt.used;
        }
        SDOD_HIP_CHECK(hipStreamSynchronize(st));
        if (it == 0) continue;
        for (size_t i = 0; i < ops_.size(); ++i) {
            float tot = 0.f;
            for (int k = 0; k < used[i]; ++k) {
                float t = 0.f;
                SDOD_HIP_CHECK(hipEventElapsedTime(&t, evs[i * kMaxLaunches + k], eve[i * kMaxLaunches + k]));
                tot += t;
            }
            samples[i].push_back(tot);
        }
    }
    for (size_t i = 0; i < ops_.size(); ++i) {
        std::sort(samples[i].begin(), samples[i].end());
        const size_t k = samples[i].size();
        ms[i] = k == 0 ? 0.f : (k & 1) ? samples[i][k / 2] : 0.5f * (samples[i][k / 2 - 1] + samples[i][k / 2]);
    }
    ++eager_runs_;
}

void Graph::stats(size_t* wbytes, size_t* abytes, int* launches, double* flops) const {
    if (wbytes) *wbytes = weight_bytes_;
    if (abytes) *abytes = arena_cap_;
    if (launches) *launches = (int)ops_.size();
    if (flops) *flops = flops_;
}

}

using sdod::Graph;

extern "C" void sdod_model_config_sd14(sdod_model_config* cfg) {
    if (!cfg) return;
    cfg->latent_channels = 4;
    cfg->latent_h = 64;
    cfg->latent_w = 64;
    cfg->model_channels = 320;
    cfg->context_dim = 768;
    cfg->context_len = 77;
    cfg->num_heads = 8;
    cfg->head_dim = 0;
    cfg->vocab_size = 49408;
    cfg->text_layers = 12;
    cfg->text_heads = 12;
    cfg->vae_channels = 128;
    cfg->linear_proj = 0;
    cfg->text_arch = 0;
    cfg->concat_channels = 0;
}

extern "C" void sdod_model_config_sd21(sdod_model_config* cfg) {
    if (!cfg) return;
    sdod_model_config_sd14(cfg);
    cfg->latent_h = cfg->latent_w = 96;
    cfg->context_dim = 1024;
    cfg->num_heads = 0;
    cfg->head_dim = 64;
    cfg->linear_proj = 1;
    cfg->text_arch = 1;
    cfg->text_layers = 23;
    cfg->text_heads = 16;
}

extern "C" int sdod_graph_create(void** graph, int kind, const sdod_model_config* cfg, int batch) {
    SDOD_TRY
    SDOD_REQUIRE(graph != nullptr && cfg != nullptr, "null argument");
    *graph = nullptr;
    *graph = new Graph(kind, *cfg, batch);
    return 0;
    SDOD_CATCH
}

extern "C" int sdod_graph_destroy(void* graph) {
    SDOD_TRY
    delete static_cast<Graph*>(graph);
    return 0;
    SDOD_CATCH
}

extern "C" int sdod_graph_num_params(void* graph) { return graph ? static_cast<Graph*>(graph)->num_params() : 0; }

extern "C" int sdod_graph_param_info(void* graph, int index, const char** name, int* ndim, int64_t shape[4]) {
    SDOD_TRY
    SDOD_REQUIRE(graph != nullptr, "null graph");
    auto* g = static_cast<Graph*>(graph);
    SDOD_REQUIRE(index >= 0 && index < g->num_params(), "parameter index out of range");
    const sdod::Param& p = g->param(index);
    if (name) *name = p.name.c_str();
    if (ndim) *ndim = (int)p.shape.size();
    if (shape)
        for (size_t i = 0; i < 4; ++i) shape[i] = i < p.shape.size() ? p.shape[i] : 1;
    return 0;
    SDOD_CATCH
}

extern "C" int sdod_graph_set_param(void* graph, const char* name, const void* data, int dtype, const int64_t* shape, int ndim) {
    SDOD_TRY
    SDOD_REQUIRE(graph && name && shape, "null argument");
    static_cast<Graph*>(graph)->set_param(name, data, dtype, shape, ndim);
    return 0;
    SDOD_CATCH
}

extern "C" int sdod_graph_load_file(void* graph, const char* path, const char* prefix) {
    SDOD_TRY
    SDOD_REQUIRE(graph && path, "null argument");
    static_cast<Graph*>(graph)->load_file(path, prefix ? prefix : "");
    return 0;
    SDOD_CATCH
}

extern "C" int sdod_graph_finalize(void* graph) {
    SDOD_TRY
    SDOD_REQUIRE(graph != nullptr, "null graph");
    static_cast<Graph*>(graph)->finalize();
    return 0;
    SDOD_CATCH
}

extern "C" int sdod_graph_io(void* graph, int is_output, int index, void** device_ptr, size_t* bytes) {
    SDOD_TRY
    SDOD_REQUIRE(graph != nullptr, "null graph");
    const sdod::IoSlot s = static_cast<Graph*>(graph)->io(is_output != 0, index);
    if (device_ptr) *device_ptr = s.ptr;
    if (bytes) *bytes = s.bytes;
    return 0;
    SDOD_CATCH
}

extern "C" int sdod_graph_param_device(void* graph, const char* name, void** device_ptr, size_t* bytes) {
    SDOD_TRY
    SDOD_REQUIRE(graph != nullptr && name != nullptr, "null argument");
    Graph* g = static_cast<Graph*>(graph);
    for (int i = 0; i < g->num_params(); ++i) {
        const sdod::Param& p = g->param(i);
        if (p.name != name) continue;
        SDOD_REQUIRE(p.dev != nullptr && p.set, "parameter '" + p.name + "' has not been set");
        if (device_ptr) *device_ptr = p.dev;
        if (bytes) *bytes = p.dev_bytes;
        return 0;
    }
    SDOD_REQUIRE(false, std::string("unknown parameter '") + name + "'");
    return 0;
    SDOD_CATCH
}

extern "C" int sdod_graph_execute(void* graph, void* stream, int use_hip_graph) {
    SDOD_TRY
    SDOD_REQUIRE(graph != nullptr, "null graph");
    static_cast<Graph*>(graph)->execute((hipStream_t)stream, (use_hip_graph & 1) != 0, (use_hip_graph & 2) != 0);
    return 0;
    SDOD_CATCH
}

extern "C" int sdod_graph_check(void* graph) {
    SDOD_TRY
    SDOD_REQUIRE(graph != nullptr, "null graph");
    static_cast<Graph*>(graph)->check_health();
    return 0;
    SDOD_CATCH
}

extern "C" int sdod_graph_num_ops(void* graph) { return graph ? static_cast<Graph*>(graph)->num_ops() : 0; }

extern "C" int sdod_graph_op_detail(void* graph, int index, const char** detail) {
    SDOD_TRY
    SDOD_REQUIRE(graph != nullptr && detail != nullptr, "null argument");
    auto* g = static_cast<Graph*>(graph);
    SDOD_REQUIRE(index >= 0 && index < g->num_ops(), "op index out of range");
    *detail = g->op(index).detail.c_str();
    return 0;
    SDOD_CATCH
}

extern "C" int sdod_graph_op_info(void* graph, int index, const char** label, double* flops, double* bytes) {
    SDOD_TRY
    SDOD_REQUIRE(graph != nullptr, "null graph");
    auto* g = static_cast<Graph*>(graph);
    SDOD_REQUIRE(index >= 0 && index < g->num_ops(), "op index out of range");
    const auto& op = g->op(index);
    if (label) *label = op.label.c_str();
    if (flops) *flops = op.flops;
    if (bytes) *bytes = op.bytes;
    return 0;
    SDOD_CATCH
}

extern "C" int sdod_graph_profile(void* graph, void* stream, int iters, float* ms_out, int n) {
    SDOD_TRY
    SDOD_REQUIRE(graph != nullptr, "null graph");
    static_cast<Graph*>(graph)->profile((hipStream_t)stream, iters, ms_out, n);
    return 0;
    SDOD_CATCH
}

extern "C" int sdod_graph_tune_info(void* graph, int* from_table, int* tuned_in_process, char* table_path, int cap) {
    SDOD_TRY
    SDOD_REQUIRE(graph != nullptr, "null graph");
    auto* g = static_cast<Graph*>(graph);
    if (from_table) *from_table = g->tune_hits();
    if (tuned_in_process) *tuned_in_process = g->tune_misses();
    if (table_path && cap > 0) {
        std::string s = sdod::shipped_tune_path();
        if (const char* extra = sdod::tune_cache_path()) s += (s.empty() ? "" : " + ") + std::string(extra);
        std::snprintf(table_path, (size_t)cap, "%s", s.c_str());
    }
    return 0;
    SDOD_CATCH
}

extern "C" int sdod_graph_stats(void* graph, size_t* weight_bytes, size_t* arena_bytes, int* num_launches, double* flops) {
    SDOD_TRY
    SDOD_REQUIRE(graph != nullptr, "null graph");
    static_cast<Graph*>(graph)->stats(weight_bytes, arena_bytes, num_launches, flops);
    return 0;
    SDOD_CATCH
}
```

### stable-diffusion-on-device_amd/sdod/amd/_lib.py

```python
import ctypes
import os

_HERE = os.path.dirname(os.path.abspath(__file__))
LIB_DIR = os.path.normpath(os.path.join(_HERE, '..', '..', 'lib'))

_cache = {}


def load(name):
    if name in _cache:
        return _cache[name]
    path = os.path.join(LIB_DIR, os.environ.get('SDOD_LIBSDOD', name) if name == 'libsdod.so' else name)
    if not os.path.exists(path):
        raise ImportError(
            f'{path} not found: build the MI355X extension first '
            f'(python -c "import __graft_entry__ as g; g.build()" or make -C stable-diffusion-on-device_amd). '
            f'There is no CPU fallback for the HIP path.')
    lib = ctypes.CDLL(path, mode=ctypes.RTLD_GLOBAL)
    _cache[name] = lib
    return lib


class SdodError(RuntimeError):
    def __init__(self, code, msg):
        super().__init__(f'[libsdod status {code}] {msg}')
        self.code = code


def hip():
    lib = load('libsdod.so')
    if not getattr(lib, '_sdod_typed', False):
        _declare(lib)
        lib._sdod_typed = True
    return lib


c_void_p, c_int, c_float, c_size_t, c_char_p = ctypes.c_void_p, ctypes.c_int, ctypes.c_float, ctypes.c_size_t, ctypes.c_char_p


class PlmsUpdateArgs(ctypes.Structure):
    _fields_ = [('eps_nhwc', ctypes.c_void_p), ('e_out', ctypes.c_void_p), ('x', ctypes.c_void_p), ('old1', ctypes.c_void_p),
                ('old2', ctypes.c_void_p), ('old3', ctypes.c_void_p), ('x_stage', ctypes.c_void_p), ('temb_row', ctypes.c_void_p),
                ('temb_dst', ctypes.c_void_p)] + \
               [(k, ctypes.c_int) for k in ('n', 'c', 'hw', 'uncond_first', 'mode', 'v_pred', 'stage_reps', 'temb_width', 'temb_reps')] + \
               [(k, ctypes.c_float) for k in ('guidance', 'vc0', 'vc1', 'c0', 'c1', 'c2', 'c3', 'div', 'sqrt_one_minus_at', 'sqrt_at',
                                              'sqrt_a_prev', 'dir_coef')]


class DpmStepArgs(ctypes.Structure):
    _fields_ = [('eps_nhwc', ctypes.c_void_p), ('e_out', ctypes.c_void_p), ('x', ctypes.c_void_p), ('y_prev', ctypes.c_void_p),
                ('x_stage', ctypes.c_void_p), ('temb_row', ctypes.c_void_p), ('temb_dst', ctypes.c_void_p)] + \
               [(k, ctypes.c_int) for k in ('n', 'c', 'hw', 'uncond_first', 'mode', 'order', 'stage_reps', 'temb_width', 'temb_reps')] + \
               [(k, ctypes.c_float) for k in ('guidance', 'sigma_s', 'alpha_s', 'sigma_ratio', 'c_prev', 'c_cur')]


class DdimInpaintStepArgs(ctypes.Structure):
    _fields_ = [(k, ctypes.c_void_p) for k in ('eps_nhwc', 'x', 'z0', 'keep', 'noise', 'x_stage', 'temb_row', 'temb_dst')] + \
               [('seed', ctypes.c_uint64), ('image_index0', ctypes.c_uint64)] + \
               [(k, ctypes.c_int) for k in ('n', 'c', 'hw', 'uncond_first', 'mode', 'v_pred', 'last', 'noise_level', 'stage_reps',
                                            'temb_width', 'temb_reps')] + \
               [(k, ctypes.c_float) for k in ('guidance', 'vc0', 'vc1', 'sqrt_one_minus_at', 'sqrt_at', 'sqrt_a_prev', 'dir_coef',
                                              'known_sa', 'known_s1a')]


class KStepArgs(ctypes.Structure):
    _fields_ = [(k, ctypes.c_void_p) for k in ('eps_nhwc', 'x', 'den_prev', 'noise', 'x_stage', 'temb_row', 'temb_dst')] + \
               [('seed', ctypes.c_uint64), ('image_index0', ctypes.c_uint64)] + \
               [(k, ctypes.c_int) for k in ('n', 'c', 'hw', 'uncond_first', 'mode', 'noise_level', 'stage_reps', 'temb_width', 'temb_reps')] + \
               [(k, ctypes.c_float) for k in ('guidance', 'd0', 'd1', 'a', 'b', 'cprev', 'u', 'stage_scale')]


class GemmDesc(ctypes.Structure):
    _fields_ = [
        ('a', c_void_p), ('a2', c_void_p), ('w', c_void_p), ('bias', c_void_p), ('row_bias', c_void_p),
        ('residual', c_void_p), ('out', c_void_p), ('workspace', c_void_p), ('workspace_bytes', c_size_t),
        ('M', c_int), ('N', c_int), ('K', c_int),
        ('lda', c_int), ('ldw', c_int), ('ldo', c_int), ('ldr', c_int),
        ('a_mode', c_int),
        ('n_img', c_int), ('h_in', c_int), ('w_in', c_int), ('c0', c_int), ('c1', c_int),
        ('stride', c_int), ('upsample', c_int), ('ksize', c_int), ('rows_per_img', c_int), ('ld_row_bias', c_int),
        ('act', c_int), ('alpha', c_float), ('bias_on_m', c_int), ('split_k', c_int), ('tile', c_int),
        ('geglu', c_int), ('k_tail', c_int), ('t0', c_void_p), ('t1', c_void_p), ('tc0', c_int), ('tc1', c_int),
        ('bias2', c_void_p), ('ln', c_int), ('ln_s', c_void_p), ('ln_eps', c_float), ('phase', c_int),
        ('wq', c_int), ('w_scale', c_void_p), ('w_off', c_void_p), ('fix_counters', c_void_p), ('xcd_panels', c_int),
        ('w_img_stride', c_int), ('vec_img_stride', c_int), ('softmax_cols', c_int), ('pad_mode', c_int),
    ]


def _declare(lib):
    P = c_void_p
    sig = {
        'sdod_gemm_f16': (c_int, [ctypes.POINTER(GemmDesc), P]),
        'sdod_gemm_fixup': (c_int, [P]),
        'sdod_gemm_fixup_counters': (c_size_t, []),
        'sdod_gemm_workspace_bytes': (c_size_t, [ctypes.POINTER(GemmDesc)]),
        'sdod_gemm_plan': (c_int, [ctypes.POINTER(GemmDesc), ctypes.POINTER(c_int), ctypes.POINTER(c_int)]),
        'sdod_gemm_halo_ok': (c_int, [ctypes.POINTER(GemmDesc), c_int]),
        'sdod_gemm_panel_ok': (c_int, [ctypes.POINTER(GemmDesc), c_int]),
        'sdod_gemm_xcd_panels': (c_int, [ctypes.POINTER(GemmDesc)]),
        'sdod_gemm_time': (c_int, [ctypes.POINTER(GemmDesc), P, c_int, ctypes.POINTER(c_float)]),
        'sdod_gemm_time_cold': (c_int, [ctypes.POINTER(GemmDesc), P, c_int, P, c_size_t, ctypes.POINTER(c_float), ctypes.POINTER(c_float)]),
        'sdod_gemm_num_tiles': (c_int, []),
        'sdod_gemm_tile_info': (c_int, [c_int, ctypes.POINTER(c_int)]),
        'sdod_gemm_tile_shape': (c_int, [c_int, ctypes.POINTER(c_int), ctypes.POINTER(c_int), ctypes.POINTER(c_int)]),
        'sdod_gemm_reduce_info': (c_int, [ctypes.POINTER(GemmDesc), P]),
        'sdod_group_norm_reduce_ok': (c_int, [c_int, c_int, c_int, c_int]),
        'sdod_group_norm_reduce_nhwc': (c_int, [P, P, P, P, P, c_int, c_int, c_int, c_int, c_int, c_float, c_int, P]),
        'sdod_group_norm_launches': (c_int, [c_int, c_int, c_int, c_int]),
        'sdod_group_norm_workspace_bytes': (c_size_t, [c_int, c_int]),
        'sdod_group_norm_layout': (c_int, [c_int, c_int] + [ctypes.POINTER(c_size_t)] * 5),
        'sdod_group_norm_status': (c_int, []),
        'sdod_group_norm_clear_error': (c_int, []),
        'sdod_group_norm_path': (c_int, [c_int, c_int, c_int, c_int, c_int, c_int]),
        'sdod_group_norm_nchw_workspace_bytes': (c_size_t, [c_int, c_int]),
        'sdod_group_norm_nchw': (c_int, [P, P, P, P, c_int, c_int, ctypes.c_longlong, c_int, c_float, c_int, c_int, P, P]),
        'sdod_group_norm_nhwc': (c_int, [P, P, P, P, P, c_int, c_int, c_int, c_int, c_int, c_float, c_int, c_int, P, P]),
        'sdod_layer_norm_f16': (c_int, [P, P, P, P, c_int, c_int, c_float, P]),
        'sdod_ln_fold_f16': (c_int, [P, c_int, c_int, c_int, P, P, P, P, P, P]),
        'sdod_compose_linear_f16': (c_int, [P, c_int, P, c_int, P, c_int, c_int, c_int, c_int, P, P, P, P]),
        'sdod_attention_f16': (c_int, [P, P, P, P, c_int, c_int, c_int, c_int, c_int, c_int, c_int, c_int, c_int, c_float, c_int, P]),
        'sdod_xattn_fold_f16': (c_int, [P, c_int, c_int, c_int, c_int, c_int, P, c_int, P, P, P, c_int, c_int, c_int, c_float, P, P, P, P, P]),
        'sdod_softmax_rows_f16': (c_int, [P, P, c_int, c_int, P]),
        'sdod_geglu_f16': (c_int, [P, P, c_int, c_int, P]),
        'sdod_act_f16': (c_int, [P, P, c_size_t, c_int, P]),
        'sdod_add_f16': (c_int, [P, P, P, c_size_t, P]),
        'sdod_concat_channels_f16': (c_int, [P, P, P, c_size_t, c_int, c_int, P]),
        'sdod_im2col3x3_small_f16': (c_int, [P, P, c_int, c_int, c_int, c_int, c_int, P]),
        'sdod_latent_im2col_f16': (c_int, [P, P, c_int, c_int, c_int, c_int, c_int, c_float, P]),
        'sdod_conv_in_f16': (c_int, [P, P, P, P, c_int, c_int, c_int, c_int, c_int, c_float, P]),
        'sdod_image_conv_in_f16': (c_int, [P, P, P, P, c_int, c_int, c_int, c_int, P]),
        'sdod_conv_in_cat_f16': (c_int, [P, P, P, P, P, c_int, c_int, c_int, c_int, c_int, c_int, P]),
        'sdod_masked_image_conv_in_f16': (c_int, [P, P, P, P, P, c_int, c_int, c_int, c_int, P]),
        'sdod_inpaint_cond_f32': (c_int, [P, P, P, P, c_int, c_int, c_int, c_int, c_int, c_int, ctypes.c_uint64, ctypes.c_uint64, P]),
        'sdod_encode_latent_f32': (c_int, [P, P, P, P, P, c_int, c_int, c_int, c_float, c_float, ctypes.c_uint64, ctypes.c_uint64, P]),
        'sdod_plms_update': (c_int, [ctypes.POINTER(PlmsUpdateArgs), P]),
        'sdod_dpm_step': (c_int, [ctypes.POINTER(DpmStepArgs), P]),
        'sdod_ddim_inpaint_step': (c_int, [ctypes.POINTER(DdimInpaintStepArgs), P]),
        'sdod_k_step': (c_int, [ctypes.POINTER(KStepArgs), P]),
        'sdod_mask_to_latent_f32': (c_int, [P, P, c_int, c_int, c_int, c_int, P]),
        'sdod_image_composite_u8': (c_int, [P, P, P, P, c_int, c_size_t, c_float, c_float, c_int, P]),
        'sdod_nchw_f32_to_nhwc_f16': (c_int, [P, P, c_int, c_int, c_int, c_float, P]),
        'sdod_nhwc_f16_to_nchw_f32': (c_int, [P, P, c_int, c_int, c_int, P]),
        'sdod_latent_prep_f16': (c_int, [P, P, P, P, c_int, c_int, c_int, c_float, P]),
        'sdod_embedding_f16': (c_int, [P, P, P, P, c_int, c_int, c_int, P]),
        'sdod_timestep_features_f16': (c_int, [P, P, c_int, c_int, P]),
        'sdod_stage_unet_inputs': (c_int, [P, P, c_size_t, c_int, P, P, c_size_t, c_int, P]),
        'sdod_randn_f32': (c_int, [P, P, c_size_t, ctypes.c_uint64, ctypes.c_uint64, P]),
        'sdod_cfg_combine': (c_int, [P, P, c_int, c_int, c_int, c_float, c_int, c_int, P]),
        'sdod_dpm_update': (c_int, [P, P, P, c_size_t, c_int, c_float, c_float, c_float, c_float, c_float, P]),
        'sdod_ddim_step_f32': (c_int, [P, P, c_size_t, c_float, c_float, c_float, c_float, P]),
        'sdod_lincomb4_f32': (c_int, [P, P, P, P, P, c_float, c_float, c_float, c_float, c_float, c_size_t, P]),
        'sdod_image_to_u8': (c_int, [P, P, c_size_t, c_float, c_float, c_int, P]),
        'sdod_hip_last_error': (c_char_p, []),
        'sdod_hip_device_info': (c_int, [ctypes.POINTER(c_int), ctypes.POINTER(c_size_t), c_char_p, c_int]),
    }
    for name, (res, args) in sig.items():
        fn = getattr(lib, name)
        fn.restype = res
        fn.argtypes = args


HIP_SYMBOLS = [
    'sdod_gemm_f16', 'sdod_gemm_fixup', 'sdod_gemm_fixup_counters', 'sdod_gemm_workspace_bytes', 'sdod_gemm_plan', 'sdod_gemm_halo_ok', 'sdod_gemm_panel_ok', 'sdod_gemm_xcd_panels', 'sdod_gemm_num_tiles', 'sdod_gemm_tile_shape', 'sdod_gemm_tile_info', 'sdod_gemm_time', 'sdod_gemm_time_cold', 'sdod_group_norm_workspace_bytes', 'sdod_group_norm_layout', 'sdod_group_norm_status', 'sdod_group_norm_clear_error', 'sdod_l2_prefetch', 'sdod_group_norm_launches', 'sdod_group_norm_path', 'sdod_group_norm_nhwc', 'sdod_group_norm_nchw', 'sdod_group_norm_nchw_workspace_bytes', 'sdod_gemm_reduce_info', 'sdod_group_norm_reduce_ok', 'sdod_group_norm_reduce_nhwc',
    'sdod_layer_norm_f16', 'sdod_ln_fold_f16', 'sdod_compose_linear_f16', 'sdod_attention_f16', 'sdod_xattn_fold_f16', 'sdod_softmax_rows_f16', 'sdod_geglu_f16', 'sdod_act_f16',
    'sdod_add_f16', 'sdod_concat_channels_f16', 'sdod_im2col3x3_small_f16', 'sdod_latent_im2col_f16', 'sdod_conv_in_f16', 'sdod_image_conv_in_f16', 'sdod_conv_in_cat_f16', 'sdod_masked_image_conv_in_f16', 'sdod_inpaint_cond_f32', 'sdod_encode_latent_f32', 'sdod_plms_update', 'sdod_dpm_step', 'sdod_ddim_inpaint_step', 'sdod_k_step', 'sdod_mask_to_latent_f32', 'sdod_image_composite_u8', 'sdod_nchw_f32_to_nhwc_f16',
    'sdod_nhwc_f16_to_nchw_f32', 'sdod_latent_prep_f16', 'sdod_embedding_f16', 'sdod_timestep_features_f16', 'sdod_cfg_combine', 'sdod_stage_unet_inputs', 'sdod_randn_f32',
    'sdod_dpm_update', 'sdod_ddim_step_f32', 'sdod_lincomb4_f32', 'sdod_image_to_u8', 'sdod_hip_last_error',
    'sdod_hip_device_info',
]


def check(code):
    if code != 0:
        msg = hip().sdod_hip_last_error()
        raise SdodError(code, msg.decode() if msg else 'unknown error')
```

### stable-diffusion-on-device_amd/sdod/amd/ops.py

```python
import ctypes

import torch

from . import _lib
from ._lib import GemmDesc, check

ACT = {None: 0, 'none': 0, 'silu': 1, 'gelu': 2, 'quick_gelu': 3}


def _stream():
    return ctypes.c_void_p(torch.cuda.current_stream().cuda_stream)


def _p(t):
    return None if t is None else ctypes.c_void_p(t.data_ptr())


def _req(t, dtype=None, name='tensor'):
    if not t.is_cuda:
        raise ValueError(f'{name} must live on the GPU')
    if not t.is_contiguous():
        raise ValueError(f'{name} must be contiguous')
    if dtype is not None and t.dtype != dtype:
        raise ValueError(f'{name} must be {dtype}, got {t.dtype}')
    return t


def _affine(weight, bias, c, device):
    if weight is None and bias is None:
        return None, None
    weight = torch.ones(c, dtype=torch.float32, device=device) if weight is None else weight.detach().to(torch.float32).contiguous()
    bias = torch.zeros(c, dtype=torch.float32, device=device) if bias is None else bias.detach().to(torch.float32).contiguous()
    return weight, bias


_ws = {}


def workspace(nbytes, device, tag='default'):
    key = (device, tag)
    buf = _ws.get(key)
    if buf is None or buf.numel() * 4 < nbytes:
        buf = torch.zeros((max(nbytes, 1) + 3) // 4, dtype=torch.float32, device=device)
        _ws[key] = buf
    return buf


def gemm(a, w, bias=None, *, residual=None, row_bias=None, rows_per_img=0, act=None, alpha=1.0, out=None,
         conv=None, a2=None, bias_on_m=False, split_k=0, tile=0, time_iters=0, geglu=False, tail=None, bias2=None,
         ln_s=None, ln_eps=1e-5, cold_scratch=None, phase=0, return_desc=False, w_scale=None, w_off=None, fixup=False,
         xcd=0, softmax_cols=0):
    lib = _lib.hip()
    _req(a, torch.float16, 'a')
    d = GemmDesc()
    if w_scale is not None:
        _req(w, torch.uint8, 'w'); _req(w_scale, torch.float32, 'w_scale'); _req(w_off, torch.float32, 'w_off')
        d.wq = 1; d.w_scale = _p(w_scale); d.w_off = _p(w_off)
    else:
        _req(w, torch.float16, 'w')
    per_image = w.dim() == 3
    nout, k = w.shape[-2:]
    if per_image:
        assert conv is None and rows_per_img > 0 and w.is_contiguous()
        d.w_img_stride = nout * k
        d.rows_per_img = rows_per_img
        if (bias is not None and bias.dim() == 2) or (ln_s is not None and ln_s.dim() == 2):
            assert (bias is None or bias.dim() == 2) and (ln_s is None or ln_s.dim() == 2)
            d.vec_img_stride = nout
    d.softmax_cols = softmax_cols
    if conv is None:
        m = a.shape[0]
        assert a.shape[1] == k, (a.shape, w.shape)
        d.a_mode = 0
        d.lda = k
        out_shape = (m, nout)
    else:
        n_img, h, wd, c0 = a.shape
        c1 = 0
        if a2 is not None:
            _req(a2, torch.float16, 'a2')
            assert a2.shape[:3] == a.shape[:3]
            c1 = a2.shape[3]
        stride = int(conv.get('stride', 1)); ups = 1 if conv.get('upsample', False) else 0
        ks = int(conv.get('ksize', 3))
        pad_mode = int(conv.get('pad_mode', 0))
        pad_sum = 1 if pad_mode else 2 * (ks // 2)
        hup, wup = h << ups, wd << ups
        ho, wo = (hup + pad_sum - ks) // stride + 1, (wup + pad_sum - ks) // stride + 1
        d.ksize = ks
        d.pad_mode = pad_mode
        m = n_img * ho * wo
        d.a_mode = 1
        d.n_img, d.h_in, d.w_in, d.c0, d.c1 = n_img, h, wd, c0, c1
        d.stride, d.upsample = stride, ups
        d.a2 = _p(a2)
        out_shape = (n_img, ho, wo, nout)
    nvis = nout // 2 if geglu else nout
    if geglu:
        out_shape = out_shape[:-1] + (nvis,)
    if out is None:
        out = torch.empty(out_shape, dtype=torch.float16, device=a.device)
    else:
        _req(out, torch.float16, 'out')
        assert out.numel() == m * nvis
    d.a, d.w, d.out = _p(a), _p(w), _p(out)
    d.M, d.N, d.K = m, nout, k
    d.ldw, d.ldo = k, nvis
    d.geglu = 1 if geglu else 0
    if tail is not None:
        t0, t1 = tail
        d.t0 = _p(t0); d.tc0 = t0.shape[-1]
        d.t1 = _p(t1); d.tc1 = t1.shape[-1] if t1 is not None else 0
        d.k_tail = k - d.tc0 - d.tc1
    if bias2 is not None:
        _req(bias2, torch.float32, 'bias2'); d.bias2 = _p(bias2)
    if ln_s is not None:
        _req(ln_s, torch.float32, 'ln_s'); d.ln = 1; d.ln_s = _p(ln_s); d.ln_eps = ln_eps
    if bias is not None:
        _req(bias, torch.float32, 'bias'); d.bias = _p(bias)
    if row_bias is not None:
        _req(row_bias, torch.float16, 'row_bias'); d.row_bias = _p(row_bias); d.rows_per_img = rows_per_img
        d.ld_row_bias = row_bias.shape[-1]
    if residual is not None:
        _req(residual, torch.float16, 'residual'); assert residual.numel() == m * nout
        d.residual = _p(residual); d.ldr = nout
    d.act = ACT[act]
    d.alpha = alpha
    d.bias_on_m = 1 if bias_on_m else 0
    d.split_k = split_k
    d.tile = tile
    d.xcd_panels = xcd
    need = lib.sdod_gemm_workspace_bytes(ctypes.byref(d))
    if need:
        ws = workspace(need, a.device, 'gemm')
        d.workspace = _p(ws); d.workspace_bytes = ws.numel() * 4
        if fixup:
            d.fix_counters = _p(workspace(lib.sdod_gemm_fixup_counters() * 4, a.device, 'gemm_fixup'))
    if time_iters:
        ms = ctypes.c_float()
        if cold_scratch is not None:
            check(lib.sdod_gemm_time_cold(ctypes.byref(d), _stream(), min(time_iters, 16), _p(cold_scratch),
                                          cold_scratch.numel() * cold_scratch.element_size(), ctypes.byref(ms), None))
        else:
            check(lib.sdod_gemm_time(ctypes.byref(d), _stream(), time_iters, ctypes.byref(ms)))
        return ms.value
    d.phase = phase
    check(lib.sdod_gemm_f16(ctypes.byref(d), _stream()))
    if return_desc:
        d._keep = (a, w, bias, residual, row_bias, out, a2, bias2)
        return out, d
    return out


class GnReduce(ctypes.Structure):
    _fields_ = [('partial', ctypes.c_void_p), ('splits', ctypes.c_int), ('slab_floats', ctypes.c_size_t), ('bias', ctypes.c_void_p),
                ('bias2', ctypes.c_void_p), ('row_bias', ctypes.c_void_p), ('ld_row_bias', ctypes.c_int), ('residual', ctypes.c_void_p),
                ('ldr', ctypes.c_int), ('x_out', ctypes.c_void_p), ('alpha', ctypes.c_float), ('act', ctypes.c_int),
                ('M', ctypes.c_int), ('N', ctypes.c_int)]


def group_norm_reduce(desc, n, hw, groups, weight=None, bias=None, eps=1e-5, silu=False, x2=None):
    lib = _lib.hip()
    red = GnReduce()
    check(lib.sdod_gemm_reduce_info(ctypes.byref(desc), ctypes.byref(red)))
    c0 = desc.N
    c1 = x2.shape[-1] if x2 is not None else 0
    dev = desc._keep[0].device
    y = torch.empty((n, hw, c0 + c1), dtype=torch.float16, device=dev)
    weight, bias = _affine(weight, bias, c0 + c1, dev)
    check(lib.sdod_group_norm_reduce_nhwc(ctypes.byref(red), _p(x2), _p(y), _p(weight), _p(bias), n, hw, c0, c1, groups, eps,
                                          1 if silu else 0, _stream()))
    return y


def group_norm_nhwc(x, groups, weight=None, bias=None, eps=1e-5, silu=False, x2=None, out=None):
    lib = _lib.hip()
    _req(x, None, 'x')
    assert x.dtype in (torch.float16, torch.float32)
    n, c0 = x.shape[0], x.shape[-1]
    hw = x.numel() // (n * c0)
    c1 = 0
    if x2 is not None:
        _req(x2, x.dtype, 'x2'); c1 = x2.shape[-1]
    if out is None:
        out = torch.empty(x.shape[:-1] + (c0 + c1,), dtype=x.dtype, device=x.device)
    weight, bias = _affine(weight, bias, c0 + c1, x.device)
    ws = workspace(lib.sdod_group_norm_workspace_bytes(n, groups), x.device, 'gn')
    check(lib.sdod_group_norm_nhwc(_p(x), _p(x2), _p(out), _p(weight), _p(bias), n, hw, c0, c1, groups, eps,
                                   1 if silu else 0, 0 if x.dtype == torch.float16 else 1, _p(ws), _stream()))
    return out


_NCHW_DTYPES = {torch.float16: 0, torch.float32: 1, torch.bfloat16: 3}


def group_norm_nchw(x, groups, weight=None, bias=None, eps=1e-5, silu=False, out=None):
    if x.dtype not in _NCHW_DTYPES:
        raise TypeError('EfficientGN HIP kernels support float16, bfloat16 and float32')
    n, c = x.shape[0], x.shape[1]
    x = x.detach()
    lib = _lib.hip()
    if (x.dim() == 4 and c % 8 == 0 and x.dtype != torch.bfloat16 and not x.is_contiguous()
            and x.is_contiguous(memory_format=torch.channels_last)):
        hw = x.shape[2] * x.shape[3]
        if lib.sdod_group_norm_path(n, hw, c, 0, groups, 0 if x.dtype == torch.float16 else 1) >= 0:
            o = None
            if out is not None:
                if not (out.shape == x.shape and out.dtype == x.dtype and out.is_contiguous(memory_format=torch.channels_last)):
                    raise ValueError('out must match x in shape, dtype and memory format')
                o = out.permute(0, 2, 3, 1)
            y = group_norm_nhwc(x.permute(0, 2, 3, 1), groups, weight, bias, eps, silu, out=o)
            return y.permute(0, 3, 1, 2)
    back_to_cl = False
    if not x.is_contiguous():
        back_to_cl = x.dim() == 4 and x.is_contiguous(memory_format=torch.channels_last)
        x = x.contiguous()
    _req(x, None, 'x')
    dst = torch.empty_like(x)
    if out is not None:
        if out.shape != x.shape or out.dtype != x.dtype:
            raise ValueError('out must match x in shape and dtype')
        if out.is_contiguous():
            dst = out
        elif not (back_to_cl and out.is_contiguous(memory_format=torch.channels_last)):
            raise ValueError('out must have the memory format of x')
    weight, bias = _affine(weight, bias, c, x.device)
    spatial = x.numel() // (n * c)
    ws = workspace(lib.sdod_group_norm_nchw_workspace_bytes(n, groups), x.device, 'gn_nchw')
    check(lib.sdod_group_norm_nchw(_p(x), _p(dst), _p(weight), _p(bias), n, c, spatial, groups, eps, 1 if silu else 0,
                                   _NCHW_DTYPES[x.dtype], _p(ws), _stream()))
    if back_to_cl:
        if out is not None and dst is not out:
            return out.copy_(dst)
        return dst.contiguous(memory_format=torch.channels_last)
    return dst


def ln_fold(w, gamma, beta, bias=None):
    lib = _lib.hip()
    _req(w, torch.float16, 'w'); _req(gamma, torch.float32, 'gamma'); _req(beta, torch.float32, 'beta')
    n, k = w.shape
    s = torch.empty(n, dtype=torch.float32, device=w.device); t = torch.empty_like(s)
    check(lib.sdod_ln_fold_f16(_p(w), n, k, k, _p(gamma), _p(beta), _p(bias), _p(s), _p(t), _stream()))
    return w, s, t


def layer_norm(x, weight, bias, eps=1e-5, out=None):
    lib = _lib.hip()
    _req(x, torch.float16, 'x')
    c = x.shape[-1]; m = x.numel() // c
    if out is None:
        out = torch.empty_like(x)
    check(lib.sdod_layer_norm_f16(_p(x), _p(out), _p(weight), _p(bias), m, c, eps, _stream()))
    return out


def attention(q, k, v, heads, scale=None, causal=False, out=None):
    lib = _lib.hip()
    for t, nme in ((q, 'q'), (k, 'k'), (v, 'v')):
        _req(t, torch.float16, nme)
    b, lq, c = q.shape
    lk = k.shape[1]
    d = c // heads
    if scale is None:
        scale = d ** -0.5
    if out is None:
        out = torch.empty_like(q)
    check(lib.sdod_attention_f16(_p(q), _p(k), _p(v), _p(out), b, heads, lq, lk, d, q.shape[2], k.shape[2], v.shape[2],
                                 out.shape[2], scale, 1 if causal else 0, _stream()))
    return out


def xattn_fold(kv, k_off, v_off, n_img, L, wq, sq, tq, wo, heads, scale=None):
    lib = _lib.hip()
    _req(kv, torch.float16, 'kv'); _req(wq, torch.float16, 'wq'); _req(wo, torch.float16, 'wo')
    _req(sq, torch.float32, 'sq'); _req(tq, torch.float32, 'tq')
    c = wq.shape[0]; d = c // heads
    if scale is None:
        scale = d ** -0.5
    w1 = torch.empty(n_img, heads * 80, c, dtype=torch.float16, device=kv.device)
    w2 = torch.empty(n_img, c, heads * 80, dtype=torch.float16, device=kv.device)
    s1 = torch.empty(n_img, heads * 80, dtype=torch.float32, device=kv.device); t1 = torch.empty_like(s1)
    check(lib.sdod_xattn_fold_f16(_p(kv), kv.shape[-1], k_off, v_off, n_img, L, _p(wq), wq.shape[1], _p(sq), _p(tq), _p(wo), wo.shape[1],
                                  heads, d, scale, _p(w1), _p(s1), _p(t1), _p(w2), _stream()))
    return w1, s1, t1, w2


def attention_strided(q, k, v, out, batch, heads, lq, lk, d, ldq, ldk, ldv, ldo, scale, causal=False):
    lib = _lib.hip()
    check(lib.sdod_attention_f16(q, k, v, out, batch, heads, lq, lk, d, ldq, ldk, ldv, ldo, scale, 1 if causal else 0,
                                 _stream()))


def softmax_rows(x, out=None):
    lib = _lib.hip()
    _req(x, torch.float16, 'x')
    n = x.shape[-1]; m = x.numel() // n
    if out is None:
        out = torch.empty_like(x)
    check(lib.sdod_softmax_rows_f16(_p(x), _p(out), m, n, _stream()))
    return out


def geglu(x, out=None):
    lib = _lib.hip()
    _req(x, torch.float16, 'x')
    c = x.shape[-1] // 2; m = x.numel() // (2 * c)
    if out is None:
        out = torch.empty(x.shape[:-1] + (c,), dtype=torch.float16, device=x.device)
    check(lib.sdod_geglu_f16(_p(x), _p(out), m, c, _stream()))
    return out


def activation(x, act, out=None):
    lib = _lib.hip()
    _req(x, torch.float16, 'x')
    if out is None:
        out = torch.empty_like(x)
    check(lib.sdod_act_f16(_p(x), _p(out), x.numel(), ACT[act], _stream()))
    return out


def add(a, b, out=None):
    lib = _lib.hip()
    _req(a, torch.float16, 'a'); _req(b, torch.float16, 'b')
    if out is None:
        out = torch.empty_like(a)
    check(lib.sdod_add_f16(_p(a), _p(b), _p(out), a.numel(), _stream()))
    return out


def concat_channels(a, b):
    lib = _lib.hip()
    _req(a, torch.float16, 'a'); _req(b, torch.float16, 'b')
    c0, c1 = a.shape[-1], b.shape[-1]
    rows = a.numel() // c0
    out = torch.empty(a.shape[:-1] + (c0 + c1,), dtype=torch.float16, device=a.device)
    check(lib.sdod_concat_channels_f16(_p(a), _p(b), _p(out), rows, c0, c1, _stream()))
    return out


def im2col3x3_small(x, kpad=64):
    lib = _lib.hip()
    _req(x, torch.float16, 'x')
    n, h, w, c = x.shape
    out = torch.empty((n * h * w, kpad), dtype=torch.float16, device=x.device)
    check(lib.sdod_im2col3x3_small_f16(_p(x), _p(out), n, h, w, c, kpad, _stream()))
    return out


def latent_im2col(x, kpad=64, scale=1.0):
    lib = _lib.hip()
    _req(x, torch.float32, 'x')
    n, c, h, w = x.shape
    out = torch.empty((n * h * w, kpad), dtype=torch.float16, device=x.device)
    check(lib.sdod_latent_im2col_f16(_p(x), _p(out), n, h, w, c, kpad, scale, _stream()))
    return out


def conv_in(x, w, bias, scale=1.0):
    lib = _lib.hip()
    _req(x, torch.float32, 'x'); _req(w, torch.float16, 'w'); _req(bias, torch.float32, 'bias')
    n, c, h, wd = x.shape
    cout = w.shape[0]
    assert w.shape[1] == 64
    out = torch.empty((n, h, wd, cout), dtype=torch.float16, device=x.device)
    check(lib.sdod_conv_in_f16(_p(x), _p(w), _p(bias), _p(out), n, h, wd, c, cout, scale, _stream()))
    return out


def image_conv_in(img_u8, w, bias):
    lib = _lib.hip()
    _req(img_u8, torch.uint8, 'img'); _req(w, torch.float16, 'w'); _req(bias, torch.float32, 'bias')
    n, h, wd, c = img_u8.shape
    assert c == 3 and w.shape[1] == 64
    cout = w.shape[0]
    out = torch.empty((n, h, wd, cout), dtype=torch.float16, device=img_u8.device)
    check(lib.sdod_image_conv_in_f16(_p(img_u8), _p(w), _p(bias), _p(out), n, h, wd, cout, _stream()))
    return out


def conv_in_cat(x, cond, w, bias):
    lib = _lib.hip()
    _req(x, torch.float32, 'x'); _req(cond, torch.float32, 'cond'); _req(w, torch.float16, 'w'); _req(bias, torch.float32, 'bias')
    n, c, h, wd = x.shape
    assert cond.shape[0] == n and tuple(cond.shape[2:]) == (h, wd) and w.shape[1] == 128, (x.shape, cond.shape, w.shape)
    cout = w.shape[0]
    out = torch.empty((n, h, wd, cout), dtype=torch.float16, device=x.device)
    check(lib.sdod_conv_in_cat_f16(_p(x), _p(cond), _p(w), _p(bias), _p(out), n, h, wd, c, cond.shape[1], cout, _stream()))
    return out


def masked_image_conv_in(img_u8, mask_u8, w, bias):
    lib = _lib.hip()
    _req(img_u8, torch.uint8, 'img'); _req(mask_u8, torch.uint8, 'mask'); _req(w, torch.float16, 'w'); _req(bias, torch.float32, 'bias')
    n, h, wd, c = img_u8.shape
    assert c == 3 and w.shape[1] == 64 and tuple(mask_u8.shape) == (n, h, wd)
    cout = w.shape[0]
    out = torch.empty((n, h, wd, cout), dtype=torch.float16, device=img_u8.device)
    check(lib.sdod_masked_image_conv_in_f16(_p(img_u8), _p(mask_u8), _p(w), _p(bias), _p(out), n, h, wd, cout, _stream()))
    return out


def inpaint_cond(moments, mask_u8, seed=0, image_index=0, n1=None, out=None, reps=1, factor=8):
    lib = _lib.hip()
    _req(moments, torch.float32, 'moments'); _req(mask_u8, torch.uint8, 'mask')
    n, c2, h, w = moments.shape
    c = c2 // 2
    assert tuple(mask_u8.shape) == (n, factor * h, factor * w), (mask_u8.shape, moments.shape)
    if n1 is not None:
        _req(n1, torch.float32, 'n1')
        assert tuple(n1.shape) == (n, c, h, w), n1.shape
    if out is None:
        out = torch.empty((reps * n, 1 + c, h, w), dtype=torch.float32, device=moments.device)
    else:
        _req(out, torch.float32, 'out')
        assert out.numel() == reps * n * (1 + c) * h * w, (out.shape, reps, n, c, h, w)
    check(lib.sdod_inpaint_cond_f32(_p(moments), _p(mask_u8), _p(n1), _p(out), n, c, h, w, factor, reps, int(seed) & (2 ** 64 - 1),
                                    int(image_index) & (2 ** 64 - 1), _stream()))
    return out


def encode_latent(moments, sqrt_at, sqrt_one_minus_at, seed=0, image_index=0, n1=None, n2=None, z0=None):
    lib = _lib.hip()
    _req(moments, torch.float32, 'moments')
    n, c2, h, w = moments.shape
    c = c2 // 2
    shape = (n, c, h, w)
    for t, name in ((n1, 'n1'), (n2, 'n2'), (z0, 'z0')):
        if t is not None:
            _req(t, torch.float32, name)
            assert tuple(t.shape) == shape, (name, t.shape, shape)
    x = torch.empty(shape, dtype=torch.float32, device=moments.device)
    check(lib.sdod_encode_latent_f32(_p(moments), _p(n1), _p(n2), _p(x), _p(z0), n, c, h * w, float(sqrt_at), float(sqrt_one_minus_at),
                                     int(seed), int(image_index), _stream()))
    return x


def nchw_f32_to_nhwc_f16(x, scale=1.0):
    lib = _lib.hip()
    _req(x, torch.float32, 'x')
    n, c = x.shape[0], x.shape[1]
    hw = x.numel() // (n * c)
    out = torch.empty((n,) + tuple(x.shape[2:]) + (c,), dtype=torch.float16, device=x.device)
    check(lib.sdod_nchw_f32_to_nhwc_f16(_p(x), _p(out), n, c, hw, scale, _stream()))
    return out


def nhwc_f16_to_nchw_f32(x):
    lib = _lib.hip()
    _req(x, torch.float16, 'x')
    n, c = x.shape[0], x.shape[-1]
    hw = x.numel() // (n * c)
    out = torch.empty((n, c) + tuple(x.shape[1:-1]), dtype=torch.float32, device=x.device)
    check(lib.sdod_nhwc_f16_to_nchw_f32(_p(x), _p(out), n, c, hw, _stream()))
    return out


def embedding(ids, table, pos):
    lib = _lib.hip()
    _req(ids, torch.int32, 'ids'); _req(table, torch.float16, 'table'); _req(pos, torch.float16, 'pos')
    rows = ids.numel(); seq = pos.shape[0]; c = table.shape[1]
    out = torch.empty(tuple(ids.shape) + (c,), dtype=torch.float16, device=ids.device)
    check(lib.sdod_embedding_f16(_p(ids), _p(table), _p(pos), _p(out), rows, seq, c, _stream()))
    return out


def timestep_features(t, dim=320):
    lib = _lib.hip()
    _req(t, torch.float32, 't')
    out = torch.empty((t.numel(), dim), dtype=torch.float16, device=t.device)
    check(lib.sdod_timestep_features_f16(_p(t), _p(out), t.numel(), dim, _stream()))
    return out


def cfg_combine(eps_nhwc, guidance, uncond_first=True, mode=1):
    lib = _lib.hip()
    _req(eps_nhwc, torch.float16, 'eps')
    n2, c = eps_nhwc.shape[0], eps_nhwc.shape[-1]
    n = n2 // 2
    spatial = tuple(eps_nhwc.shape[1:-1])
    hw = eps_nhwc.numel() // (n2 * c)
    out = torch.empty((n, c) + spatial, dtype=torch.float32, device=eps_nhwc.device)
    check(lib.sdod_cfg_combine(_p(eps_nhwc), _p(out), n, c, hw, guidance, 1 if uncond_first else 0, mode, _stream()))
    return out


def _guided_dims(eps_nhwc, x):
    _req(eps_nhwc, torch.float16, 'eps'); _req(x, torch.float32, 'x')
    n2, c = eps_nhwc.shape[0], eps_nhwc.shape[-1]
    n = n2 // 2
    hw = eps_nhwc.numel() // (n2 * c)
    assert x.numel() == n * c * hw
    return n, c, hw


def _fill_ddim(a, ddim):
    a.sqrt_one_minus_at, a.sqrt_at, a.sqrt_a_prev, a.dir_coef = ddim['sqrt_one_minus_at'], ddim['sqrt_at'], ddim['sqrt_a_prev'], ddim['dir_coef']


def _fill_v_pred(a, v_coef):
    if v_coef is not None:
        a.v_pred, a.vc0, a.vc1 = 1, v_coef[0], v_coef[1]


def _fill_stage(a, x, stage):
    if stage is None:
        return
    x_dst, temb_row, temb_dst = stage
    _req(x_dst, torch.float32, 'x_dst'); _req(temb_row, torch.float16, 'temb_row'); _req(temb_dst, torch.float16, 'temb_dst')
    a.x_stage, a.stage_reps = _p(x_dst), x_dst.numel() // x.numel()
    assert a.stage_reps * x.numel() == x_dst.numel() and temb_dst.numel() % temb_row.numel() == 0
    a.temb_row, a.temb_dst, a.temb_width, a.temb_reps = _p(temb_row), _p(temb_dst), temb_row.numel(), temb_dst.numel() // temb_row.numel()


def plms_update(eps_nhwc, x, old, coefs, div, ddim, guidance, mode=1, v_coef=None, stage=None):
    lib = _lib.hip()
    n, c, hw = _guided_dims(eps_nhwc, x)
    assert len(old) <= 3 and len(coefs) == len(old) + 1
    e_out = torch.empty_like(x)
    a = _lib.PlmsUpdateArgs()
    a.eps_nhwc, a.e_out, a.x = _p(eps_nhwc), _p(e_out), _p(x)
    olds = list(old) + [None] * (3 - len(old)); cs = list(coefs) + [0.0] * (4 - len(coefs))
    for t in old:
        _req(t, torch.float32, 'old')
    a.old1, a.old2, a.old3 = _p(olds[0]), _p(olds[1]), _p(olds[2])
    a.n, a.c, a.hw, a.uncond_first, a.mode = n, c, hw, 1, mode
    a.guidance, a.c0, a.c1, a.c2, a.c3, a.div = guidance, cs[0], cs[1], cs[2], cs[3], div
    _fill_v_pred(a, v_coef)
    _fill_ddim(a, ddim)
    _fill_stage(a, x, stage)
    check(lib.sdod_plms_update(ctypes.byref(a), _stream()))
    return e_out


def dpm_step(eps_nhwc, x, y_prev, coef, guidance, mode=0, uncond_first=True, stage=None):
    lib = _lib.hip()
    n, c, hw = _guided_dims(eps_nhwc, x)
    _req(y_prev, torch.float32, 'y_prev')
    assert x.numel() == y_prev.numel()
    a = _lib.DpmStepArgs()
    a.eps_nhwc, a.x, a.y_prev = _p(eps_nhwc), _p(x), _p(y_prev)
    a.n, a.c, a.hw, a.uncond_first, a.mode, a.order = n, c, hw, 1 if uncond_first else 0, mode, coef['order']
    a.guidance = guidance
    a.sigma_s, a.alpha_s, a.sigma_ratio, a.c_prev, a.c_cur = coef['sigma_s'], coef['alpha_s'], coef['sigma_ratio'], coef['c_prev'], coef['c_cur']
    _fill_stage(a, x, stage)
    check(lib.sdod_dpm_step(ctypes.byref(a), _stream()))


def ddim_inpaint_step(eps_nhwc, x, ddim, guidance, z0=None, keep=None, known=None, noise=None, seed=0, noise_level=0, image_index=0,
                      mode=1, v_coef=None, stage=None):
    lib = _lib.hip()
    n, c, hw = _guided_dims(eps_nhwc, x)
    a = _lib.DdimInpaintStepArgs()
    a.eps_nhwc, a.x = _p(eps_nhwc), _p(x)
    if keep is not None:
        _req(keep, torch.float32, 'keep')
        assert keep.numel() == n * hw, (keep.shape, n, hw)
        if z0 is not None:
            _req(z0, torch.float32, 'z0')
            assert z0.numel() == x.numel()
        a.keep, a.z0 = _p(keep), _p(z0)
        if noise is not None:
            _req(noise, torch.float32, 'noise')
            assert noise.numel() == x.numel()
            a.noise = _p(noise)
        if known is None:
            a.last = 1
        else:
            a.known_sa, a.known_s1a = known
            a.seed, a.noise_level, a.image_index0 = int(seed) & (2 ** 64 - 1), int(noise_level), int(image_index) & (2 ** 64 - 1)
    a.n, a.c, a.hw, a.uncond_first, a.mode = n, c, hw, 1, mode
    a.guidance = guidance
    _fill_v_pred(a, v_coef)
    _fill_ddim(a, ddim)
    _fill_stage(a, x, stage)
    check(lib.sdod_ddim_inpaint_step(ctypes.byref(a), _stream()))


def k_step(eps_nhwc, x, coef, guidance=1.0, den_prev=None, noise=None, seed=0, noise_level=0, image_index=0, mode=1, uncond_first=True,
           stage=None):
    lib = _lib.hip()
    _req(x, torch.float32, 'x')
    a = _lib.KStepArgs()
    if eps_nhwc is None:
        n, c = x.shape[0], x.shape[1]
        hw = x.numel() // (n * c)
    else:
        n, c, hw = _guided_dims(eps_nhwc, x)
        a.eps_nhwc = _p(eps_nhwc)
    a.x = _p(x)
    for t, name in ((den_prev, 'den_prev'), (noise, 'noise')):
        if t is not None:
            _req(t, torch.float32, name)
            assert t.numel() == x.numel(), (name, t.shape, x.shape)
    a.den_prev, a.noise = _p(den_prev), _p(noise)
    a.seed, a.noise_level, a.image_index0 = int(seed) & (2 ** 64 - 1), int(noise_level), int(image_index) & (2 ** 64 - 1)
    a.n, a.c, a.hw, a.uncond_first, a.mode = n, c, hw, 1 if uncond_first else 0, mode
    a.guidance = guidance
    a.d0, a.d1, a.a, a.b = coef.get('d0', 1.0), coef.get('d1', 0.0), coef.get('a', 0.0), coef.get('b', 0.0)
    a.cprev, a.u, a.stage_scale = coef.get('cprev', 0.0), coef.get('u', 0.0), coef.get('stage_scale', 0.0)
    _fill_stage(a, x, stage)
    check(lib.sdod_k_step(ctypes.byref(a), _stream()))


def mask_to_latent(mask_u8, factor=8):
    lib = _lib.hip()
    _req(mask_u8, torch.uint8, 'mask')
    n, h, w = mask_u8.shape
    assert h % factor == 0 and w % factor == 0, (h, w, factor)
    out = torch.empty((n, h // factor, w // factor), dtype=torch.float32, device=mask_u8.device)
    check(lib.sdod_mask_to_latent_f32(_p(mask_u8), _p(out), n, h // factor, w // factor, factor, _stream()))
    return out


def image_composite(img_nhwc, init_u8, mask_u8, a=0.5, b=0.5, mode=1):
    lib = _lib.hip()
    _req(img_nhwc, torch.float16, 'img'); _req(init_u8, torch.uint8, 'init'); _req(mask_u8, torch.uint8, 'mask')
    assert img_nhwc.shape[-1] == 3 and init_u8.numel() == img_nhwc.numel() and mask_u8.numel() * 3 == img_nhwc.numel()
    n = img_nhwc.shape[0]
    out = torch.empty(img_nhwc.shape, dtype=torch.uint8, device=img_nhwc.device)
    check(lib.sdod_image_composite_u8(_p(img_nhwc), _p(init_u8), _p(mask_u8), _p(out), n, mask_u8.numel() // n, a, b, mode, _stream()))
    return out


def stage_unet_inputs(x, x_dst, temb_row, temb_dst):
    lib = _lib.hip()
    _req(x, torch.float32, 'x'); _req(x_dst, torch.float32, 'x_dst'); _req(temb_row, torch.float16, 'temb_row'); _req(temb_dst, torch.float16, 'temb_dst')
    reps = x_dst.numel() // x.numel()
    assert reps * x.numel() == x_dst.numel() and temb_dst.numel() % temb_row.numel() == 0
    check(lib.sdod_stage_unet_inputs(_p(x), _p(x_dst), x.numel(), reps, _p(temb_row), _p(temb_dst), temb_row.numel(),
                                     temb_dst.numel() // temb_row.numel(), _stream()))


def randn(shape, seed, stream_id, device, return_words=False, out=None):
    lib = _lib.hip()
    if out is None:
        out = torch.empty(shape, dtype=torch.float32, device=device)
    else:
        _req(out, torch.float32, 'out')
        assert tuple(out.shape) == tuple(shape), (out.shape, shape)
    words = torch.empty(out.numel(), dtype=torch.int32, device=device) if return_words else None
    with torch.cuda.device(out.device):
        check(lib.sdod_randn_f32(_p(out), _p(words), out.numel(), int(seed) & (2 ** 64 - 1), int(stream_id) & (2 ** 64 - 1), _stream()))
    return (out, words) if return_words else out


def dpm_update(x, eps, y_prev, order, sigma_s, alpha_s, sigma_ratio, c_prev, c_cur):
    lib = _lib.hip()
    for t in (x, eps, y_prev):
        _req(t, torch.float32)
    check(lib.sdod_dpm_update(_p(x), _p(eps), _p(y_prev), x.numel(), order, sigma_s, alpha_s, sigma_ratio, c_prev, c_cur,
                              _stream()))


def ddim_step(x, e, sqrt_one_minus_at, sqrt_at, sqrt_a_prev, dir_coef):
    lib = _lib.hip()
    _req(x, torch.float32); _req(e, torch.float32)
    check(lib.sdod_ddim_step_f32(_p(x), _p(e), x.numel(), sqrt_one_minus_at, sqrt_at, sqrt_a_prev, dir_coef, _stream()))


def lincomb4(es, coefs, div):
    lib = _lib.hip()
    es = list(es) + [None] * (4 - len(es)); coefs = list(coefs) + [0.0] * (4 - len(coefs))
    out = torch.empty_like(es[0])
    check(lib.sdod_lincomb4_f32(_p(out), _p(es[0]), _p(es[1]), _p(es[2]), _p(es[3]), coefs[0], coefs[1], coefs[2], coefs[3],
                                div, out.numel(), _stream()))
    return out


def image_to_u8(img_nhwc, a=0.5, b=0.5, mode=1):
    lib = _lib.hip()
    _req(img_nhwc, torch.float16, 'img')
    out = torch.empty(img_nhwc.shape, dtype=torch.uint8, device=img_nhwc.device)
    check(lib.sdod_image_to_u8(_p(img_nhwc), _p(out), img_nhwc.numel(), a, b, mode, _stream()))
    return out


def device_info():
    lib = _lib.hip()
    cu = ctypes.c_int(); mem = ctypes.c_size_t(); arch = ctypes.create_string_buffer(64)
    check(lib.sdod_hip_device_info(ctypes.byref(cu), ctypes.byref(mem), arch, 64))
    return {'cu_count': cu.value, 'hbm_bytes': mem.value, 'arch': arch.value.decode()}
```

Baseline: 10.69 images/s.

## Add stream-K split-KV attention for d=40 with cross-workgroup partial merge

Adds a stream-K form of the d=40 attention kernel. A fixed grid of 3x the CU count splits all (query-block, key-tile) work evenly, and partial outputs and running maxima are published to a workspace. An atomic counter picks the last contributor, which merges the partials with exp2 rescaling. The path is meant to fix poor wave quantization when the number of query blocks sits between 1x and 2x the CU count, as at SD's 64x64 resolution. In exchange it needs a workspace, global-memory round trips and atomics.

```diff
diff --git a/include/sdod_hip.h b/include/sdod_hip.h
--- a/include/sdod_hip.h
+++ b/include/sdod_hip.h
@@ -123,6 +123,13 @@
                                 int lq, int lk, int d, int ldq, int ldk, int ldv, int ldo, float scale, int causal,
                                 void* stream);
 
+SDOD_API int sdod_attention_ws_f16(const void* q, const void* k, const void* v, void* out, int batch, int heads,
+                                   int lq, int lk, int d, int ldq, int ldk, int ldv, int ldo, float scale, int causal,
+                                   void* workspace, size_t workspace_bytes, void* stream);
+SDOD_API size_t sdod_attention_workspace_bytes(int batch, int heads, int lq, int lk, int d);
+SDOD_API int sdod_attention_stream_grid(int batch, int heads, int lq, int lk, int d, int causal);
+SDOD_API int sdod_attention_stream_plan(int nqb, int nt, int g, int view, int index, int* out, int cap);
+
 SDOD_API int sdod_xattn_fold_f16(const void* kv, int ld_kv, int k_off, int v_off, int n_img, int L, const void* wq, int ldq,
                                  const void* sq, const void* tq, const void* wo, int ldwo, int heads, int d, float scale, void* w1,
                                  void* s1, void* t1, void* w2, void* stream);
diff --git a/stable-diffusion-on-device_amd/csrc/attention.hip b/stable-diffusion-on-device_amd/csrc/attention.hip
--- a/stable-diffusion-on-device_amd/csrc/attention.hip
+++ b/stable-diffusion-on-device_amd/csrc/attention.hip
@@ -18,6 +18,8 @@
     int ldq, ldk, ldv, ldo;
     float scale_log2;
     int causal;
+    unsigned* ws_cnt;
+    f32x4* ws_slot;
 };
 
 typedef short short4v __attribute__((__vector_size__(4 * sizeof(short))));
@@ -40,8 +42,38 @@
     }
 }
 
-template <int D, int QT, bool TR, int KVS = 1>
+__host__ __device__ inline int stream_cut(int i, int T, int G) { return (int)((unsigned)i * (unsigned)T / (unsigned)G); }
+__host__ __device__ inline int stream_owner(int x, int T, int G) { return (int)((((unsigned)x + 1u) * (unsigned)G - 1u) / (unsigned)T); }
+struct StreamSeg {
+    int qb, t0, t1;
+    int slot;
+    int first, last;
+    int end;
+};
+__host__ __device__ inline StreamSeg stream_segment(int i, int gt, int hi, int NT, int T, int G) {
+    StreamSeg s;
+    s.qb = (int)((unsigned)gt / (unsigned)NT);
+    const int base = s.qb * NT;
+    s.t0 = gt - base;
+    s.t1 = hi - base < NT ? hi - base : NT;
+    s.slot = i + s.qb;
+    s.first = stream_owner(base, T, G);
+    s.last = stream_owner(base + NT - 1, T, G);
+    s.end = base + s.t1;
+    return s;
+}
+__host__ __device__ inline bool stream_contributes(int i, int T, int G) { return stream_cut(i + 1, T, G) > stream_cut(i, T, G); }
+__host__ __device__ inline int stream_contributors(int first, int last, int T, int G) {
+    int n = 0;
+    for (int i = first; i <= last; ++i) n += stream_contributes(i, T, G) ? 1 : 0;
+    return n;
+}
+constexpr int kStreamSlotVecs = 7;
+constexpr size_t kStreamSlotBytes = (size_t)kStreamSlotVecs * 256 * sizeof(f32x4);
+
+template <int D, int QT, bool TR, int KVS = 1, bool STREAM = false>
 __global__ __launch_bounds__(256 * KVS, (attn_min_waves<D, QT>())) void attn_kernel(const AttnP p) {
+    static_assert(!STREAM || (D == 40 && QT == 2 && TR && KVS == 1), "the stream form exists for <40, 2, true, 1> only");
     constexpr int DP = ((D + 31) / 32) * 32;
     constexpr int KSTEPS = DP / 32;
     constexpr int DV = ((D + 15) / 16) * 16;
@@ -67,15 +99,6 @@
     const int wave = tid >> 6;
     const int g = lane >> 4;
     const int li = lane & 15;
-    const int nqb = (p.Lq + 64 * QT - 1) / (64 * QT);
-    const int lid = xcd_remap(blockIdx.x, nqb * p.H * p.B);
-    const int bh = lid / nqb;
-    const int b = bh / p.H, h = bh - b * p.H;
-    const int q_block = (lid - bh * nqb) * (64 * QT);
-
-    const f16* kbase = p.k + (size_t)b * p.Lk * p.ldk + h * D;
-    const f16* vbase = p.v + (size_t)b * p.Lk * p.ldv + h * D;
-
     {
         constexpr int KPADC = (DP - D) / 8, VPADC = (DV - D) / 8;
         for (int st = 0; st < 2; ++st) {
@@ -98,15 +121,38 @@
         }
     }
 
+    const int nqb = (p.Lq + 64 * QT - 1) / (64 * QT);
+    const int sG = (int)gridDim.x, sNT = (p.Lk + KT - 1) / KT, sT = nqb * p.H * p.B * sNT;
+    const int swg = STREAM ? xcd_remap(blockIdx.x, sG) : 0;
+    const int shi = STREAM ? stream_cut(swg + 1, sT, sG) : 0;
+    int sgt = STREAM ? stream_cut(swg, sT, sG) : 0;
+    if (STREAM && sgt >= shi) return;
+    do {
+    StreamSeg sg{};
+    if constexpr (STREAM) {
+        sg = stream_segment(swg, sgt, shi, sNT, sT, sG);
+        sgt = sg.end;
+    }
+    int stid = tid;
+    if constexpr (STREAM) asm volatile("" : "+v"(stid));
+    const int sli = stid & 15, sgr = (stid & 63) >> 4, swave = stid >> 6;
+    const int lid = STREAM ? sg.qb : xcd_remap(blockIdx.x, nqb * p.H * p.B);
+    const int bh = lid / nqb;
+    const int b = bh / p.H, h = bh - b * p.H;
+    const int q_block = (lid - bh * nqb) * (64 * QT);
+
+    const f16* kbase = p.k + (size_t)b * p.Lk * p.ldk + h * D;
+    const f16* vbase = p.v + (size_t)b * p.Lk * p.ldv + h * D;
+
     f16x8 qf[QT][KSTEPS];
     int qrow[QT];
 #pragma unroll
     for (int t = 0; t < QT; ++t) {
-        qrow[t] = q_block + wave * (16 * QT) + t * 16 + li;
+        qrow[t] = q_block + swave * (16 * QT) + t * 16 + sli;
         const f16* qp = p.q + ((size_t)b * p.Lq + qrow[t]) * p.ldq + h * D;
 #pragma unroll
         for (int ks = 0; ks < KSTEPS; ++ks) {
-            const int d0 = ks * 32 + g * 8;
+            const int d0 = ks * 32 + sgr * 8;
             qf[t][ks] = (qrow[t] < p.Lq && d0 + 8 <= D) ? ldg8(qp + d0) : zero8();
             if (DEFER)
 #pragma unroll
@@ -115,15 +161,16 @@
     }
 
     int kend = p.Lk;
-    if (p.causal) kend = min(p.Lk, q_block + 64 * QT);
+    if (!STREAM && p.causal) kend = min(p.Lk, q_block + 64 * QT);
     const int NT = (kend + KT - 1) / KT;
+    const int tbeg = STREAM ? sg.t0 : 0, tend = STREAM ? sg.t1 : NT;
 
     f16x8 rk[LD_IT], rv[LD_IT];
     const f16* kptr0[LD_IT];
     const f16* vptr0[LD_IT];
 #pragma unroll
     for (int i = 0; i < LD_IT; ++i) {
-        const int idx = tid + 256 * i;
+        const int idx = stid + 256 * i;
         const int row = idx / DC, ch = idx - row * DC;
         kptr0[i] = kbase + (size_t)row * p.ldk + ch * 8;
         vptr0[i] = vbase + (size_t)row * p.ldv + ch * 8;
@@ -164,6 +211,26 @@
         }
     };
 
+    auto stage_first = [&](int t) {
+        f16* sK = smem;
+        f16* sV = sK + KT * KSTR;
+#pragma unroll
+        for (int i = 0; i < LD_IT; ++i) {
+            const int idx = stid + 256 * i;
+            const int row = idx / DC, ch = idx - row * DC;
+            const int key = t * KT + row;
+            if (idx < KT * DC) {
+                f16x8 kx = zero8(), vx = zero8();
+                if (key < p.Lk) {
+                    kx = ldg8(kbase + (size_t)key * p.ldk + ch * 8);
+                    vx = ldg8(vbase + (size_t)key * p.ldv + ch * 8);
+                }
+                asm volatile("" : "+v"(kx), "+v"(vx));
+                *reinterpret_cast<f16x8*>(sK + row * KSTR + ch * 8) = kx;
+                *reinterpret_cast<f16x8*>(sV + row * VSTR + ch * 8) = vx;
+            }
+        }
+    };
     f32x4 o[QT][NDT];
     float m_run[QT], l_run[QT];
 #pragma unroll
@@ -191,7 +258,7 @@
     auto softmax_pv = [&](auto a_c, int t, int thr, f32x4 (&s_a)[4], const f16x8 (&vfr)[HOLD ? 2 : 1][HOLD ? NDT : 1],
                           const f16* sV) {
         constexpr int a = decltype(a_c)::value;
-        const bool need_mask = (t * KT + KT > p.Lk) || (p.causal && (t * KT + KT - 1 > q_block + wave * (16 * QT)));
+        const bool need_mask = (t * KT + KT > p.Lk) || (!STREAM && p.causal && (t * KT + KT - 1 > q_block + wave * (16 * QT)));
         if (need_mask) {
             int key0 = t * KT + g * 4;
             asm volatile("" : "+v"(key0));
@@ -339,20 +406,22 @@
         }
     };
 
-    if (grp < NT) {
-        load_tile(grp);
+    if constexpr (STREAM) {
+        stage_first(tbeg);
+    } else if (tbeg + grp < tend) {
+        load_tile(tbeg + grp);
         store_tile(0);
     }
     __syncthreads();
-    const int NTG = (NT + KVS - 1) / KVS;
+    const int NTG = (tend - tbeg + KVS - 1) / KVS;
     int thr = INT_MIN;
     for (int it = 0; it < NTG; ++it) {
-        const int t = it * KVS + grp;
+        const int t = tbeg + it * KVS + grp;
         const int cur = it & 1;
-        const bool has_next = t + KVS < NT;
+        const bool has_next = t + KVS < tend;
         const f16* sK = smem + cur * STAGE;
         const f16* sV = sK + KT * KSTR;
-        if (t >= NT) {
+        if (t >= tend) {
             __syncthreads();
             continue;
         }
@@ -401,17 +470,107 @@
             m_run[a] = m;
         }
     }
+    int etid = tid;
+    if constexpr (STREAM) asm volatile("" : "+v"(etid));
+    const int eli = etid & 15;
+    if constexpr (STREAM) {
+        bool store = sg.t0 == 0 && sg.t1 == NT;
+        if (!store) {
+            auto pub = [&](f32x4* dst, f32x4 v) { asm volatile("global_store_dwordx4 %0, %1, off sc0 sc1" ::"v"(dst), "v"(v) : "memory"); };
+            auto sub = [&](const f32x4* src) {
+                f32x4 v;
+                asm volatile("global_load_dwordx4 %0, %1, off sc0 sc1" : "=v"(v) : "v"(src) : "memory");
+                return v;
+            };
+            f32x4* mine = p.ws_slot + (size_t)sg.slot * (kStreamSlotVecs * 256) + etid;
+#pragma unroll
+            for (int a = 0; a < QT; ++a)
+#pragma unroll
+                for (int dt = 0; dt < NDT; ++dt) pub(mine + (a * NDT + dt) * 256, o[a][dt]);
+            pub(mine + QT * NDT * 256, f32x4{m_run[0], m_run[1], 0.f, 0.f});
+            asm volatile("s_waitcnt vmcnt(0)" ::: "memory");
+            __syncthreads();
+            const int ncontrib = stream_contributors(sg.first, sg.last, sT, sG);
+            int* flag = reinterpret_cast<int*>(smem_raw);
+            if (etid == 0) {
+                unsigned* cnt = p.ws_cnt + sg.qb;
+                const unsigned prev = __hip_atomic_fetch_add(cnt, 1u, __ATOMIC_RELAXED, __HIP_MEMORY_SCOPE_AGENT);
+                const bool last = prev + 1u == (unsigned)ncontrib;
+                if (last) __hip_atomic_store(cnt, 0u, __ATOMIC_RELAXED, __HIP_MEMORY_SCOPE_AGENT);
+                *flag = last ? 1 : 0;
+            }
+            __syncthreads();
+            store = __builtin_amdgcn_readfirstlane(*flag) != 0;
+            __syncthreads();
+            if (store) {
+                f32x4 ao[QT][NDT];
+                float am[QT];
+#pragma unroll
+                for (int a = 0; a < QT; ++a) {
+                    am[a] = -1e30f;
+#pragma unroll
+                    for (int dt = 0; dt < NDT; ++dt) ao[a][dt] = f32x4{0.f, 0.f, 0.f, 0.f};
+                }
+                for (int i = sg.first; i <= sg.last; ++i) {
+                    if (!stream_contributes(i, sT, sG)) continue;
+                    f32x4 to[QT][NDT], tm;
+                    if (i != swg) {
+                        const f32x4* src = p.ws_slot + (size_t)(i + sg.qb) * (kStreamSlotVecs * 256) + etid;
+#pragma unroll
+                        for (int a = 0; a < QT; ++a)
+#pragma unroll
+                            for (int dt = 0; dt < NDT; ++dt) to[a][dt] = sub(src + (a * NDT + dt) * 256);
+                        tm = sub(src + QT * NDT * 256);
+                        asm volatile("s_waitcnt vmcnt(0)" ::: "memory");
+#pragma unroll
+                        for (int a = 0; a < QT; ++a)
+#pragma unroll
+                            for (int dt = 0; dt < NDT; ++dt) asm volatile("" : "+v"(to[a][dt]));
+                        asm volatile("" : "+v"(tm));
+                    } else {
+#pragma unroll
+                        for (int a = 0; a < QT; ++a)
+#pragma unroll
+                            for (int dt = 0; dt < NDT; ++dt) to[a][dt] = o[a][dt];
+                        tm = f32x4{m_run[0], m_run[1], 0.f, 0.f};
+                    }
+#pragma unroll
+                    for (int a = 0; a < QT; ++a) {
+                        const float m = fmaxf(am[a], tm[a]);
+                        const float a0 = __builtin_amdgcn_exp2f(am[a] - m), a1 = __builtin_amdgcn_exp2f(tm[a] - m);
+#pragma unroll
+                        for (int dt = 0; dt < NDT; ++dt)
+#pragma unroll
+                            for (int r = 0; r < 4; ++r) ao[a][dt][r] = ao[a][dt][r] * a0 + to[a][dt][r] * a1;
+                        am[a] = m;
+                    }
+                }
+#pragma unroll
+                for (int a = 0; a < QT; ++a) {
+                    m_run[a] = am[a];
+#pragma unroll
+                    for (int dt = 0; dt < NDT; ++dt) o[a][dt] = ao[a][dt];
+                }
+            }
+        }
+        if (!store) continue;
+    }
 #pragma unroll
     for (int a = 0; a < QT; ++a) {
         float l;
         if (SUM_BY_MFMA) {
-            l = __shfl(o[a][D / 16][D % 4], ((D % 16) / 4) * 16 + li);
+            if constexpr (STREAM)
+                l = __builtin_bit_cast(float, __builtin_amdgcn_ds_bpermute(4 * (((D % 16) / 4) * 16 + eli), __builtin_bit_cast(int, o[a][D / 16][D % 4])));
+            else
+                l = __shfl(o[a][D / 16][D % 4], ((D % 16) / 4) * 16 + li);
         } else {
             l = quad_rows_sum(l_run[a]);
         }
         const float inv = l > 0.f ? 1.0f / l : 0.f;
-        if (qrow[a] < p.Lq) {
-            f16* op = p.out + ((size_t)b * p.Lq + qrow[a]) * p.ldo + h * D;
+        int qr = qrow[a];
+        if constexpr (STREAM) asm volatile("" : "+v"(qr));
+        if (qr < p.Lq) {
+            f16* op = p.out + ((size_t)b * p.Lq + qr) * p.ldo + h * D;
 #pragma unroll
             for (int dt = 0; dt < NDT; ++dt) {
                 const int dv0 = dt * 16 + g * 4;
@@ -424,6 +583,7 @@
             }
         }
     }
+    } while (STREAM && sgt < shi);
 }
 
 template <int D, int QT, bool TR, int KVS = 1>
@@ -440,6 +600,18 @@
     }
     dim3 grid(((p.Lq + 64 * QT - 1) / (64 * QT)) * p.H * p.B);
     SDOD_LAUNCH((attn_kernel<D, QT, TR, KVS>), grid, dim3(256 * KVS), smem, st, p);
+    return hipGetLastError();
+}
+
+hipError_t attn_launch_stream(const AttnP& p, int G, hipStream_t st) {
+    constexpr size_t smem = (size_t)2 * 64 * (64 + 8 + odd16(48)) * sizeof(f16);
+    static std::atomic<unsigned long long> attr_devs{0};
+    if (sdod::first_use_on_device(attr_devs)) {
+        hipError_t e = hipFuncSetAttribute(reinterpret_cast<const void*>(&attn_kernel<40, 2, true, 1, true>),
+                                           hipFuncAttributeMaxDynamicSharedMemorySize, (int)smem);
+        if (e != hipSuccess) return e;
+    }
+    SDOD_LAUNCH((attn_kernel<40, 2, true, 1, true>), dim3(G), dim3(256), smem, st, p);
     return hipGetLastError();
 }
 
@@ -537,12 +709,115 @@
     }
 }
 
+int attn_device_cus() {
+    static std::atomic<int> cus[64];
+    int dev = 0;
+    if (hipGetDevice(&dev) != hipSuccess || dev < 0 || dev >= 64) return 0;
+    int v = cus[dev].load(std::memory_order_relaxed);
+    if (v == 0) {
+        if (hipDeviceGetAttribute(&v, hipDeviceAttributeMultiprocessorCount, dev) != hipSuccess || v <= 0) v = -1;
+        cus[dev].store(v, std::memory_order_relaxed);
+    }
+    return v > 0 ? v : 0;
+}
+
+bool attn_two_query_tiles(int lq, int d) {
+    bool big = lq >= 2048 && d != 160;
+    if (const char* e = std::getenv("SDOD_ATTN_QT")) big = e[0] == '2' && d != 160;
+    return big;
+}
+bool attn_transposed_reads() { return std::getenv("SDOD_ATTN_NO_TR") == nullptr; }
+
+bool stream_fits(long long nqb, long long nt, long long g) { return nqb > 0 && nt > 0 && g > 0 && nqb * nt * (g + 1) < INT_MAX; }
+
+int stream_grid(int batch, int heads, int lq, int lk, int d, int causal) {
+    if (d != 40 || causal || !attn_two_query_tiles(lq, d) || !attn_transposed_reads()) return 0;
+    const long long nqb = (long long)((lq + 127) / 128) * heads * batch, nt = (lk + 63) / 64;
+    int G;
+    if (const char* e = std::getenv("SDOD_ATTN_STREAM")) {
+        G = std::atoi(e);
+        if (G <= 0) return 0;
+    } else {
+        const int cus = attn_device_cus();
+        if (!(nqb > cus && nqb <= 2ll * cus) || nt < 4) return 0;
+        G = 3 * cus;
+    }
+    return stream_fits(nqb, nt, G) ? G : 0;
+}
+
+size_t stream_counter_bytes(long long nqb) { return (size_t)((nqb * sizeof(unsigned) + 127) / 128 * 128); }
+
+int attention_impl(const void* q, const void* k, const void* v, void* out, int batch, int heads, int lq, int lk, int d, int ldq,
+                   int ldk, int ldv, int ldo, float scale, int causal, void* workspace, size_t workspace_bytes, void* stream);
+
 }
 
 extern "C" int sdod_attention_f16(const void* q, const void* k, const void* v, void* out, int batch, int heads, int lq,
                                   int lk, int d, int ldq, int ldk, int ldv, int ldo, float scale, int causal,
                                   void* stream) {
     SDOD_TRY
+    return attention_impl(q, k, v, out, batch, heads, lq, lk, d, ldq, ldk, ldv, ldo, scale, causal, nullptr, 0, stream);
+    SDOD_CATCH
+}
+
+extern "C" int sdod_attention_ws_f16(const void* q, const void* k, const void* v, void* out, int batch, int heads, int lq,
+                                     int lk, int d, int ldq, int ldk, int ldv, int ldo, float scale, int causal,
+                                     void* workspace, size_t workspace_bytes, void* stream) {
+    SDOD_TRY
+    return attention_impl(q, k, v, out, batch, heads, lq, lk, d, ldq, ldk, ldv, ldo, scale, causal, workspace, workspace_bytes, stream);
+    SDOD_CATCH
+}
+
+extern "C" int sdod_attention_stream_grid(int batch, int heads, int lq, int lk, int d, int causal) {
+    if (batch <= 0 || heads <= 0 || lq <= 0 || lk <= 0) return 0;
+    return stream_grid(batch, heads, lq, lk, d, causal);
+}
+
+extern "C" size_t sdod_attention_workspace_bytes(int batch, int heads, int lq, int lk, int d) {
+    if (batch <= 0 || heads <= 0 || lq <= 0 || lk <= 0) return 0;
+    const int G = stream_grid(batch, heads, lq, lk, d, 0);
+    if (G == 0) return 0;
+    const long long nqb = (long long)((lq + 127) / 128) * heads * batch;
+    return stream_counter_bytes(nqb) + (size_t)(nqb + G - 1) * kStreamSlotBytes;
+}
+
+extern "C" int sdod_attention_stream_plan(int nqb, int nt, int g, int view, int index, int* out, int cap) {
+    if (!stream_fits(nqb, nt, g) || index < 0 || cap < 0 || (cap > 0 && !out)) return -1;
+    const int T = nqb * nt;
+    int n = 0;
+    if (view == 0) {
+        if (index >= g) return -1;
+        const int hi = stream_cut(index + 1, T, g);
+        for (int gt = stream_cut(index, T, g); gt < hi; ++n) {
+            const StreamSeg sg = stream_segment(index, gt, hi, nt, T, g);
+            if (n < cap / 5) {
+                int* row = out + 5 * n;
+                row[0] = sg.qb; row[1] = sg.t0; row[2] = sg.t1; row[3] = sg.slot;
+                row[4] = stream_contributors(sg.first, sg.last, T, g);
+            }
+            gt = sg.end;
+        }
+        return n;
+    }
+    if (view == 1) {
+        if (index >= nqb) return -1;
+        const int first = stream_owner(index * nt, T, g), last = stream_owner(index * nt + nt - 1, T, g);
+        for (int i = first; i <= last; ++i) {
+            if (!stream_contributes(i, T, g)) continue;
+            if (n < cap / 2) {
+                out[2 * n] = i;
+                out[2 * n + 1] = i + index;
+            }
+            ++n;
+        }
+        return n;
+    }
+    return -1;
+}
+
+namespace {
+int attention_impl(const void* q, const void* k, const void* v, void* out, int batch, int heads, int lq, int lk, int d, int ldq,
+                   int ldk, int ldv, int ldo, float scale, int causal, void* workspace, size_t workspace_bytes, void* stream) {
     SDOD_REQUIRE(q && k && v && out, "null pointer");
     SDOD_REQUIRE(batch > 0 && heads > 0 && lq > 0 && lk > 0, "bad shape");
     SDOD_REQUIRE(d == 40 || d == 64 || d == 80 || d == 160, "head dim must be one of 40, 64, 80, 160");
@@ -556,14 +831,25 @@
     p.ldq = ldq; p.ldk = ldk; p.ldv = ldv; p.ldo = ldo;
     p.scale_log2 = scale * 1.4426950408889634f;
     p.causal = causal;
-    const bool no_tr = std::getenv("SDOD_ATTN_NO_TR") != nullptr;
-    const bool tr = !no_tr;
-    bool big = lq >= 2048 && d != 160;
-    if (const char* e = std::getenv("SDOD_ATTN_QT")) big = e[0] == '2' && d != 160;
+    const bool tr = attn_transposed_reads();
+    const bool big = attn_two_query_tiles(lq, d);
     hipStream_t st = (hipStream_t)stream;
     hipError_t e;
+    const int G = workspace ? stream_grid(batch, heads, lq, lk, d, causal) : 0;
     switch (d) {
-    case 40: e = attn_dispatch<40>(p, big, tr, st); break;
+    case 40:
+        if (G > 0) {
+            const long long nqb = (long long)((lq + 127) / 128) * heads * batch;
+            SDOD_REQUIRE(((uintptr_t)workspace & 127) == 0, "workspace must be 128-byte aligned");
+            SDOD_REQUIRE(workspace_bytes >= stream_counter_bytes(nqb) + (size_t)(nqb + G - 1) * kStreamSlotBytes,
+                         "workspace smaller than sdod_attention_workspace_bytes reports");
+            p.ws_cnt = (unsigned*)workspace;
+            p.ws_slot = (f32x4*)((char*)workspace + stream_counter_bytes(nqb));
+            e = attn_launch_stream(p, G, st);
+            break;
+        }
+        e = attn_dispatch<40>(p, big, tr, st);
+        break;
     case 64: e = attn_dispatch<64>(p, big, tr, st); break;
     case 80: {
         static const bool kvs_off = [] { const char* e2 = std::getenv("SDOD_ATTN_KVS"); return e2 && e2[0] == '0'; }();
@@ -576,7 +862,7 @@
     }
     SDOD_HIP_CHECK(e);
     return 0;
-    SDOD_CATCH
+}
 }
 
 extern "C" int sdod_xattn_fold_f16(const void* kv, int ld_kv, int k_off, int v_off, int n_img, int L, const void* wq, int ldq,
diff --git a/stable-diffusion-on-device_amd/csrc/engine.h b/stable-diffusion-on-device_amd/csrc/engine.h
--- a/stable-diffusion-on-device_amd/csrc/engine.h
+++ b/stable-diffusion-on-device_amd/csrc/engine.h
@@ -117,6 +117,8 @@
     size_t ws_bytes_ = 0, ws_need_ = 0;
     char* gn_ws_ = nullptr;
     size_t gn_ws_bytes_ = 0, gn_ws_need_ = 0;
+    char* attn_ws_ = nullptr;
+    size_t attn_ws_bytes_ = 0, attn_ws_need_ = 0;
 
     std::vector<IoSlot> inputs_, outputs_;
     void* io_alloc(std::vector<IoSlot>& v, size_t bytes);
diff --git a/stable-diffusion-on-device_amd/csrc/engine.hip b/stable-diffusion-on-device_amd/csrc/engine.hip
--- a/stable-diffusion-on-device_amd/csrc/engine.hip
+++ b/stable-diffusion-on-device_amd/csrc/engine.hip
@@ -65,6 +65,7 @@
     (void)hipFree(arena_base_);
     (void)hipFree(ws_);
     (void)hipFree(gn_ws_);
+    (void)hipFree(attn_ws_);
     (void)hipFree(kv_all_);
     for (void* d : derived_) (void)hipFree(d);
 }
@@ -882,13 +883,16 @@
 void Graph::attention(const f16* q, const f16* k, const f16* v, f16* out, int B, int heads, int lq, int lk, int d, int ldq,
                       int ldk, int ldv, int ldo, bool causal) {
     settle();
+    if (mode_ != DECLARE && !causal) attn_ws_need_ = std::max(attn_ws_need_, sdod_attention_workspace_bytes(B, heads, lq, lk, d));
     if (mode_ != REAL) return;
     const double fl = 4.0 * B * heads * (double)lq * lk * d;
     flops_ += fl;
     const float scale = 1.0f / sqrtf((float)d);
     const int ca = causal ? 1 : 0;
+    void* ws = attn_ws_;
+    const size_t ws_bytes = attn_ws_bytes_;
     ops_.push_back(Op{[=](hipStream_t st) {
-        check_rc(sdod_attention_f16(q, k, v, out, B, heads, lq, lk, d, ldq, ldk, ldv, ldo, scale, ca, st));
+        check_rc(sdod_attention_ws_f16(q, k, v, out, B, heads, lq, lk, d, ldq, ldk, ldv, ldo, scale, ca, ws, ws_bytes, st));
     }, "attn_d" + std::to_string(d), fl, 2.0 * B * heads * d * (2.0 * lq + 2.0 * lk),
                       "B" + std::to_string(B) + " h" + std::to_string(heads) + " lq" + std::to_string(lq) + " lk" + std::to_string(lk)});
 }
@@ -919,7 +923,7 @@
     SDOD_REQUIRE(nmiss == 0, std::to_string(nmiss) + " parameter(s) not set: " + missing + (nmiss > 5 ? ", ..." : ""));
     mode_ = DRY;
     arena_reset();
-    ws_need_ = gn_ws_need_ = 0;
+    ws_need_ = gn_ws_need_ = attn_ws_need_ = 0;
     build();
     arena_cap_ = align_up(arena_high_, 256) + 256;
     ws_bytes_ = align_up(ws_need_, 256) + 256;
@@ -928,6 +932,11 @@
     SDOD_HIP_CHECK(hipMalloc((void**)&ws_, ws_bytes_));
     SDOD_HIP_CHECK(hipMalloc((void**)&gn_ws_, gn_ws_bytes_));
     SDOD_HIP_CHECK(hipMemset(gn_ws_, 0, gn_ws_bytes_));
+    if (attn_ws_need_ > 0) {
+        attn_ws_bytes_ = align_up(attn_ws_need_, 256);
+        SDOD_HIP_CHECK(hipMalloc((void**)&attn_ws_, attn_ws_bytes_));
+        SDOD_HIP_CHECK(hipMemset(attn_ws_, 0, attn_ws_bytes_));
+    }
     SDOD_HIP_CHECK(hipMalloc((void**)&fix_counters_, sdod_gemm_fixup_counters() * sizeof(unsigned)));
     SDOD_HIP_CHECK(hipMemset(fix_counters_, 0, sdod_gemm_fixup_counters() * sizeof(unsigned)));
     if (kind_ == SDOD_GRAPH_UNET && kv_total_ > 0)
diff --git a/stable-diffusion-on-device_amd/sdod/amd/_lib.py b/stable-diffusion-on-device_amd/sdod/amd/_lib.py
--- a/stable-diffusion-on-device_amd/sdod/amd/_lib.py
+++ b/stable-diffusion-on-device_amd/sdod/amd/_lib.py
@@ -119,6 +119,10 @@
         'sdod_ln_fold_f16': (c_int, [P, c_int, c_int, c_int, P, P, P, P, P, P]),
         'sdod_compose_linear_f16': (c_int, [P, c_int, P, c_int, P, c_int, c_int, c_int, c_int, P, P, P, P]),
         'sdod_attention_f16': (c_int, [P, P, P, P, c_int, c_int, c_int, c_int, c_int, c_int, c_int, c_int, c_int, c_float, c_int, P]),
+        'sdod_attention_ws_f16': (c_int, [P, P, P, P, c_int, c_int, c_int, c_int, c_int, c_int, c_int, c_int, c_int, c_float, c_int, P, c_size_t, P]),
+        'sdod_attention_workspace_bytes': (c_size_t, [c_int, c_int, c_int, c_int, c_int]),
+        'sdod_attention_stream_grid': (c_int, [c_int, c_int, c_int, c_int, c_int, c_int]),
+        'sdod_attention_stream_plan': (c_int, [c_int, c_int, c_int, c_int, c_int, ctypes.POINTER(c_int), c_int]),
         'sdod_xattn_fold_f16': (c_int, [P, c_int, c_int, c_int, c_int, c_int, P, c_int, P, P, P, c_int, c_int, c_int, c_float, P, P, P, P, P]),
         'sdod_softmax_rows_f16': (c_int, [P, P, c_int, c_int, P]),
         'sdod_geglu_f16': (c_int, [P, P, c_int, c_int, P]),
@@ -162,7 +166,7 @@
 
 HIP_SYMBOLS = [
     'sdod_gemm_f16', 'sdod_gemm_fixup', 'sdod_gemm_fixup_counters', 'sdod_gemm_workspace_bytes', 'sdod_gemm_plan', 'sdod_gemm_halo_ok', 'sdod_gemm_panel_ok', 'sdod_gemm_xcd_panels', 'sdod_gemm_num_tiles', 'sdod_gemm_tile_shape', 'sdod_gemm_tile_info', 'sdod_gemm_time', 'sdod_gemm_time_cold', 'sdod_group_norm_workspace_bytes', 'sdod_group_norm_layout', 'sdod_group_norm_status', 'sdod_group_norm_clear_error', 'sdod_l2_prefetch', 'sdod_group_norm_launches', 'sdod_group_norm_path', 'sdod_group_norm_nhwc', 'sdod_group_norm_nchw', 'sdod_group_norm_nchw_workspace_bytes', 'sdod_gemm_reduce_info', 'sdod_group_norm_reduce_ok', 'sdod_group_norm_reduce_nhwc',
-    'sdod_layer_norm_f16', 'sdod_ln_fold_f16', 'sdod_compose_linear_f16', 'sdod_attention_f16', 'sdod_xattn_fold_f16', 'sdod_softmax_rows_f16', 'sdod_geglu_f16', 'sdod_act_f16',
+    'sdod_layer_norm_f16', 'sdod_ln_fold_f16', 'sdod_compose_linear_f16', 'sdod_attention_f16', 'sdod_attention_ws_f16', 'sdod_attention_workspace_bytes', 'sdod_attention_stream_grid', 'sdod_attention_stream_plan', 'sdod_xattn_fold_f16', 'sdod_softmax_rows_f16', 'sdod_geglu_f16', 'sdod_act_f16',
     'sdod_add_f16', 'sdod_concat_channels_f16', 'sdod_im2col3x3_small_f16', 'sdod_latent_im2col_f16', 'sdod_conv_in_f16', 'sdod_image_conv_in_f16', 'sdod_conv_in_cat_f16', 'sdod_masked_image_conv_in_f16', 'sdod_inpaint_cond_f32', 'sdod_encode_latent_f32', 'sdod_plms_update', 'sdod_dpm_step', 'sdod_ddim_inpaint_step', 'sdod_k_step', 'sdod_mask_to_latent_f32', 'sdod_image_composite_u8', 'sdod_nchw_f32_to_nhwc_f16',
     'sdod_nhwc_f16_to_nchw_f32', 'sdod_latent_prep_f16', 'sdod_embedding_f16', 'sdod_timestep_features_f16', 'sdod_cfg_combine', 'sdod_stage_unet_inputs', 'sdod_randn_f32',
     'sdod_dpm_update', 'sdod_ddim_step_f32', 'sdod_lincomb4_f32', 'sdod_image_to_u8', 'sdod_hip_last_error',
diff --git a/stable-diffusion-on-device_amd/sdod/amd/ops.py b/stable-diffusion-on-device_amd/sdod/amd/ops.py
--- a/stable-diffusion-on-device_amd/sdod/amd/ops.py
+++ b/stable-diffusion-on-device_amd/sdod/amd/ops.py
@@ -255,7 +255,12 @@
     return out
 
 
-def attention(q, k, v, heads, scale=None, causal=False, out=None):
+def attention_workspace(batch, heads, lq, lk, d, device=None):
+    n = _lib.hip().sdod_attention_workspace_bytes(batch, heads, lq, lk, d)
+    return torch.zeros(max(n, 128), dtype=torch.uint8, device=device if device is not None else torch.device('cuda:0'))
+
+
+def attention(q, k, v, heads, scale=None, causal=False, out=None, workspace=None):
     lib = _lib.hip()
     for t, nme in ((q, 'q'), (k, 'k'), (v, 'v')):
         _req(t, torch.float16, nme)
@@ -266,6 +271,11 @@
         scale = d ** -0.5
     if out is None:
         out = torch.empty_like(q)
+    if workspace is not None:
+        check(lib.sdod_attention_ws_f16(_p(q), _p(k), _p(v), _p(out), b, heads, lq, lk, d, q.shape[2], k.shape[2], v.shape[2],
+                                        out.shape[2], scale, 1 if causal else 0, _p(workspace), workspace.numel() * workspace.element_size(),
+                                        _stream()))
+        return out
     check(lib.sdod_attention_f16(_p(q), _p(k), _p(v), _p(out), b, heads, lq, lk, d, q.shape[2], k.shape[2], v.shape[2],
                                  out.shape[2], scale, 1 if causal else 0, _stream()))
     return out
@@ -286,8 +296,12 @@
     return w1, s1, t1, w2
 
 
-def attention_strided(q, k, v, out, batch, heads, lq, lk, d, ldq, ldk, ldv, ldo, scale, causal=False):
-    lib = _lib.hip()
+def attention_strided(q, k, v, out, batch, heads, lq, lk, d, ldq, ldk, ldv, ldo, scale, causal=False, workspace=None):
+    lib = _lib.hip()
+    if workspace is not None:
+        check(lib.sdod_attention_ws_f16(q, k, v, out, batch, heads, lq, lk, d, ldq, ldk, ldv, ldo, scale, 1 if causal else 0,
+                                        _p(workspace), workspace.numel() * workspace.element_size(), _stream()))
+        return
     check(lib.sdod_attention_f16(q, k, v, out, batch, heads, lq, lk, d, ldq, ldk, ldv, ldo, scale, 1 if causal else 0,
                                  _stream()))
 
```

Result: no change. 10.76 images/s, median of 6 (+0.7%).
